# MLCogUP/nspeech

Hardware: AMD Instinct MI355X
Metric: mel-frames/sec Tacotron-2 LJSpeech bs32 train step (higher is better)
Workload: dtype bf16; 1 GPU; Tacotron-2 train step (fwd+bwd+clip+Adam), batch 32/GPU, T_in 160, T_out 1000, r=5; targets = spectrogram features of synthetic speech (SURVEY 8d); global_batch=32, parallelism=dp1, deterministic_gradients=True

## Files before the change

### include/nspeech_hip.h

```cpp
#ifndef NSPEECH_HIP_H
#define NSPEECH_HIP_H
#include <stddef.h>
#include <stdint.h>

#ifdef __cplusplus
extern "C" {
#endif

typedef void* ns_stream_t;

enum { NS_OK = 0, NS_ERR_BAD_ARG = -1, NS_ERR_UNSUPPORTED_SHAPE = -2, NS_ERR_LAUNCH = -3,
       NS_ERR_SHORT_BUFFER = -4  };
enum { NS_F32 = 0, NS_BF16 = 1, NS_F64 = 2  };
enum { NS_ACT_NONE = 0, NS_ACT_RELU = 1, NS_ACT_TANH = 2, NS_ACT_SIGMOID = 3,
       NS_ACT_SOFTSIGN = 4  };

int ns_version(void);
const char* ns_device_arch(void);
const char* ns_last_error(void);

int ns_occupy(int blocks, int threads, int lds_bytes, int heavy, double usec, int* started, ns_stream_t stream);
int ns_wait_counter(const int* counter, int target, double timeout_usec, ns_stream_t stream);

typedef struct {
  int dtype;
  int M, N, K;
  const void* A; int64_t lda; int a_mode;
  const void* B; int64_t ldb; int b_mode;
  int b_seg_len; int64_t b_seg_stride;
  void* C; int64_t ldc; int c_dtype;
  int accumulate;
  const float* bias;
  int act;
  float alpha;
  int row_period, row_lo, row_hi, row_shift;
  float* col_sum; float* col_sumsq;
  int split_k;
  const void* addend; int64_t ld_add;
  const void* gate; int64_t ld_gate;
  int f32_passes;
  int addend_dtype;
  const void* A_lo; const void* B_lo;
  int batch; int64_t batch_stride_a, batch_stride_b, batch_stride_c;
  float* stat_part;
  int stat_slots;
  const void* stat_z; int64_t ld_stat_z; int stat_z_dtype;
  const float* stat_mean; const float* stat_istd;
  float* splitk_work; int* splitk_count;
} ns_gemm_params;
int ns_gemm(const ns_gemm_params* p, ns_stream_t stream);
size_t ns_gemm_stat_part_floats(int M, int N);
size_t ns_gemm_splitk_work_bytes(int M, int N, int split_k);
size_t ns_gemm_splitk_counters(int M, int N);
const char* ns_gemm_last_kernel(void);



typedef struct {
  const void* src; int src_dtype; int64_t src_si, src_sj;
  void* dst; int dst_dtype; int64_t dst_si, dst_sj;
  int I, J, Cc;
  int accumulate;
} ns_copy3d_params;
int ns_copy3d(const ns_copy3d_params* p, ns_stream_t stream);

typedef struct {
  const int* ids;
  const float* table;
  void* out; int out_dtype;
  int N, T, P, padl, D, V;
} ns_embedding_params;
int ns_embedding_fwd(const ns_embedding_params* p, ns_stream_t stream);
typedef struct {
  const int* ids;
  const float* dout;
  float* dtable;
  int N, T, P, padl, D, V;
  float* work;
} ns_embedding_bwd_params;
int ns_embedding_bwd(const ns_embedding_bwd_params* p, ns_stream_t stream);
size_t ns_embedding_bwd_work_floats(int N, int D, int V);

typedef struct {
  const void* z; void* y; int dtype;
  int rows, C;
  const float* col_sum; const float* col_sumsq; float count;
  const float* gamma; const float* beta;
  float* moving_mean; float* moving_var;
  float* mean_out; float* istd_out;
  float eps, momentum;
  int training;
  int row_period, row_lo, row_hi;
  void* y_hi; void* y_lo;
  int64_t ld_y;
} ns_bn_fwd_params;
int ns_bn_fwd(const ns_bn_fwd_params* p, ns_stream_t stream);

typedef struct {
  const float* dy; const void* z; void* dpre; int dtype;
  int rows, C;
  const float* mean; const float* istd; const float* gamma;
  float* dgamma; float* dbeta; float* dbias;
  float* work;
  float count;
  int act;
  int row_period, row_lo, row_hi;
  int dpre_dtype;
  const float* sum_dy; const float* sum_dyxh;
  int64_t ld_dy;
} ns_bn_bwd_params;
int ns_bn_bwd(const ns_bn_bwd_params* p, ns_stream_t stream);

typedef struct {
  const void* x; int dtype; int64_t ld;
  int rows, C;
  float* out;
  float* work;
} ns_colsum_params;
int ns_colsum(const ns_colsum_params* p, ns_stream_t stream);
size_t ns_colsum_work_floats(int C);

typedef struct {
  const float* pred; int64_t ldp;
  const float* target;
  void* dpred; int dpred_dtype; int64_t ldd;
  int N, T, P, padl, F;
  int n_prio; float w_all, w_prio;
  float* loss_acc;
  int vec4;
} ns_l1_loss_params;
int ns_l1_loss(const ns_l1_loss_params* p, ns_stream_t stream);

typedef struct { const float* x; int64_t n; float* out; float* work; } ns_sumsq_params;
int ns_sumsq(const ns_sumsq_params* p, ns_stream_t stream);
typedef struct {
  float* p; const float* g; float* m; float* v; int64_t n;
  const float* gnorm_sq; float clip; float grad_scale;
  float lr_t, beta1, beta2, eps;
  void* shadow_bf16;
  const int* status[12];
  float* skipped;
} ns_adam_params;
int ns_adam(const ns_adam_params* p, ns_stream_t stream);

typedef struct { const float* x; const int64_t* offsets; int nseg; float* out; } ns_segment_stats_params;
int ns_segment_stats(const ns_segment_stats_params* p, ns_stream_t stream);

int ns_zero(void* p, size_t bytes, ns_stream_t stream);
#define NS_ZERO_MANY_MAX 24
int ns_zero_many(void* const* ptrs, const size_t* bytes, int n, ns_stream_t stream);
int ns_streams_concurrent(ns_stream_t a, ns_stream_t b, void* work);

typedef struct { const float* src; void* hi; void* lo; int64_t n; } ns_split_params;
int ns_split_hi_lo(const ns_split_params* p, ns_stream_t stream);

typedef struct {
  const float* src; int rows, cols; int64_t ld_src;
  void* dst; int dst_dtype; int64_t ld_dst;
  int transpose;
  void* dst_hi; void* dst_lo;
} ns_cast2d_params;
int ns_cast2d(const ns_cast2d_params* p, ns_stream_t stream);
int ns_cast2d_batchable(const ns_cast2d_params* p);
int ns_cast2d_batch(const ns_cast2d_params* table_dev, const int* tile_end_dev, int n, int total_tiles, ns_stream_t stream);

typedef struct {
  int dtype;
  int N, T, H, P, padl;
  const float* xg; int64_t ld_xg;
  const void* whT;
  const void* wh;
  const int* lengths;
  int reverse;
  float forget_bias;
  void* h; int64_t ld_h;
  float* c;
  void* gates;
  const float* dh; int64_t ld_dh;
  void* dgates;
  float* work;
  int f32_passes;
  const void* whT_hi; const void* whT_lo; const void* wh_bf16;
  void* dgates_bf16;
  void* h_bf16; int64_t ld_h_bf16;
  uint32_t zoneout_thr_cell, zoneout_thr_output;
  uint32_t zoneout_seed_cell, zoneout_seed_output;
  float cell_clip;
} ns_lstm_seq_params;
int ns_lstm_seq_fwd(const ns_lstm_seq_params* p, ns_stream_t stream);
int ns_lstm_seq_bwd(const ns_lstm_seq_params* p, ns_stream_t stream);
size_t ns_lstm_seq_work_bytes(const ns_lstm_seq_params* p);
int ns_lstm_seq2_fwd(const ns_lstm_seq_params* p0, const ns_lstm_seq_params* p1, ns_stream_t stream);
int ns_lstm_seq2_bwd(const ns_lstm_seq_params* p0, const ns_lstm_seq_params* p1, ns_stream_t stream);


int ns_lstm_cluster_supported(const ns_lstm_seq_params* fw, const ns_lstm_seq_params* bw, int backward);
size_t ns_lstm_cluster_work_bytes(const ns_lstm_seq_params* p);
int ns_lstm_cluster_fwd(const ns_lstm_seq_params* fw, const ns_lstm_seq_params* bw, void* work, ns_stream_t stream);
int ns_lstm_cluster_bwd(const ns_lstm_seq_params* fw, const ns_lstm_seq_params* bw, void* work, ns_stream_t stream);

int ns_lstm_wide_supported(const ns_lstm_seq_params* p, int backward);
size_t ns_lstm_wide_work_bytes(const ns_lstm_seq_params* p);
int ns_lstm_wide_fwd(const ns_lstm_seq_params* p, void* work, ns_stream_t stream);
int ns_lstm_wide_bwd(const ns_lstm_seq_params* p, void* work, ns_stream_t stream);

typedef struct {
  int dtype, N, H, K;
  const void* a; int64_t a_sn;
  const void* wT;
  const float* xg; int64_t xg_sn;
  const float* bias;
  const float* c_prev; int64_t c_sn;
  void* h_out; int64_t h_sn;
  void* h_out2; int64_t h2_sn;
  float* c_out; int64_t co_sn;
  float forget_bias;
  int f32_passes;
  const void* wT_hi; const void* wT_lo;
  float zoneout_cell, zoneout_output;
  const void* h_prev; int64_t hp_sn;
  float cell_clip;
} ns_lstm_step_params;
int ns_lstm_step(const ns_lstm_step_params* p, ns_stream_t stream);

size_t ns_rows32_packed_bytes(int K, int C);
int ns_rows32_pack(const float* w, int64_t ldw, int K, int C, int cell_units, void* packed, ns_stream_t stream);
size_t ns_rows32_rows_bytes(int K);
int ns_rows32_pack_rows(const float* a, int64_t a_sn, int N, int K, void* rows, int rows_K, int col0, ns_stream_t stream);
typedef struct {
  int N, K, C;
  const float* a; int64_t a_sn;
  const void* a_rows; int a_rows_K, a_rows_col;
  const void* packed;
  int f32_passes;
  const float* bias;
  const float* add; int64_t add_sn;
  int act;
  float* out; int64_t out_sn;
  float* out2; int64_t out2_sn;
  void* rows_out; int rows_out_K, rows_out_col;
  void* rows_out2; int rows_out2_K, rows_out2_col;
  int cell_units;
  const float* c_prev; int64_t c_sn;
  float* c_out; int64_t co_sn;
  float forget_bias;
  float zoneout_cell, zoneout_output;
  const float* h_prev; int64_t hp_sn;
  float cell_clip;
} ns_rows32_params;
int ns_rows32(const ns_rows32_params* p, ns_stream_t stream);

typedef struct {
  int dtype, N, Ti, Pi, padl_i, Tia, A, E, kw;
  const int* lengths;
  const float* keys_t;
  const void* values;
  const float* q; int64_t q_sn;
  const float* aprev; float* aout; int64_t al_sn;
  void* ctx_out; int64_t ctx_sn;
  void* ctx_out2; int64_t ctx2_sn;
  const float* wcl; const float* v;
  float* e_raw;
  const void* pv; int E2;
  void* pv_out; int64_t pv_out_sn;
// ... 298 lines not shown
```

### nspeech_amd/csrc/common.h

```cpp
#pragma once
#include <hip/hip_runtime.h>
#include <stdint.h>
#include <stdio.h>
#include <string.h>
#include "../../include/nspeech_hip.h"

typedef __bf16 bf16_t;
typedef __attribute__((ext_vector_type(8))) __bf16 bf16x8;
typedef __attribute__((ext_vector_type(4))) __bf16 bf16x4;
typedef __attribute__((ext_vector_type(4))) float f32x4;
typedef __attribute__((ext_vector_type(16))) float f32x16;

void ns_set_error(const char* fmt, ...);
int ns_zero_async(void* p, size_t bytes, hipStream_t s);
int ns_device_cus();
int ns_stats_finalize(const float* part, int slots, int N, float* s1, float* s2, hipStream_t s);

#define NS_CHECK_ARG(cond, ...)                                   \
  do {                                                            \
    if (!(cond)) {                                                \
      ns_set_error(__VA_ARGS__);                                  \
      return NS_ERR_BAD_ARG;                                      \
    }                                                             \
  } while (0)

#define NS_CHECK_LAUNCH(name)                                     \
  do {                                                            \
    hipError_t e__ = hipGetLastError();                           \
    if (e__ != hipSuccess) {                                      \
      ns_set_error("%s: launch failed: %s", name,                 \
                   hipGetErrorString(e__));                       \
      return NS_ERR_LAUNCH;                                       \
    }                                                             \
  } while (0)

template <typename T> struct dt_of;
template <> struct dt_of<float> { static constexpr int v = NS_F32; };
template <> struct dt_of<bf16_t> { static constexpr int v = NS_BF16; };

__device__ __forceinline__ float ldf(const float* p) { return *p; }
__device__ __forceinline__ float ldf(const bf16_t* p) { return (float)*p; }
__device__ __forceinline__ void stf(float* p, float v) { *p = v; }
__device__ __forceinline__ void stf(bf16_t* p, float v) { *p = (bf16_t)v; }

__device__ __forceinline__ float sigmoidf_(float x) {
  return __builtin_amdgcn_rcpf(1.0f + __builtin_amdgcn_exp2f(-1.4426950408889634f * x));
}
__device__ __forceinline__ float tanhf_(float x) {
  return 1.0f - 2.0f * __builtin_amdgcn_rcpf(__builtin_amdgcn_exp2f(2.8853900817779268f * x) + 1.0f);
}

__device__ __forceinline__ void ns_st_sc1(float* p, float v) { __hip_atomic_store(p, v, __ATOMIC_RELAXED, __HIP_MEMORY_SCOPE_AGENT); }
__device__ __forceinline__ float ns_ld_sc1(const float* p) { return __hip_atomic_load(p, __ATOMIC_RELAXED, __HIP_MEMORY_SCOPE_AGENT); }
__device__ __forceinline__ void ns_st_sc1(float4* p, const float4& v) {
  unsigned long long* q = (unsigned long long*)p;
  __hip_atomic_store(q, ((unsigned long long)__float_as_uint(v.y) << 32) | __float_as_uint(v.x), __ATOMIC_RELAXED, __HIP_MEMORY_SCOPE_AGENT);
  __hip_atomic_store(q + 1, ((unsigned long long)__float_as_uint(v.w) << 32) | __float_as_uint(v.z), __ATOMIC_RELAXED, __HIP_MEMORY_SCOPE_AGENT);
}
__device__ __forceinline__ float4 ns_ld_sc1(const float4* p) {
  const unsigned long long* q = (const unsigned long long*)p;
  const unsigned long long a = __hip_atomic_load(q, __ATOMIC_RELAXED, __HIP_MEMORY_SCOPE_AGENT);
  const unsigned long long b = __hip_atomic_load(q + 1, __ATOMIC_RELAXED, __HIP_MEMORY_SCOPE_AGENT);
  return make_float4(__uint_as_float((unsigned)a), __uint_as_float((unsigned)(a >> 32)), __uint_as_float((unsigned)b),
                     __uint_as_float((unsigned)(b >> 32)));
}
__device__ __forceinline__ void ns_drain_stores() { asm volatile("s_waitcnt vmcnt(0)" ::: "memory"); }

__host__ __device__ __forceinline__ uint32_t ns_fmix32(uint32_t x) {
  x ^= x >> 16; x *= 0x85EBCA6Bu; x ^= x >> 13; x *= 0xC2B2AE35u; x ^= x >> 16;
  return x;
}
__host__ __device__ __forceinline__ bool ns_zone_keep(uint32_t seed, uint32_t t, uint32_t n, uint32_t u, uint32_t thr) {
  uint32_t x = ns_fmix32(seed ^ (t * 0x9E3779B9u));
  x = ns_fmix32(x ^ (n * 0x7FEB352Du));
  x = ns_fmix32(x ^ (u * 0x846CA68Bu));
  return (x >> 8) < thr;
}

__device__ __forceinline__ float ns_cell_clip(float c, float clip) { return clip > 0.f ? fminf(fmaxf(c, -clip), clip) : c; }

__device__ __forceinline__ float apply_act(float v, int act) {
  switch (act) {
    case NS_ACT_RELU: return v > 0.f ? v : 0.f;
    case NS_ACT_TANH: return tanhf_(v);
    case NS_ACT_SIGMOID: return sigmoidf_(v);
    case NS_ACT_SOFTSIGN: return v / (1.0f + fabsf(v));
    default: return v;
  }
}

#define NS_DPP_F(v, ctrl) __builtin_bit_cast(float, __builtin_amdgcn_update_dpp(0, __builtin_bit_cast(int, (v)), (ctrl), 0xF, 0xF, true))
__device__ __forceinline__ float row16_sum(float v) {
  v += NS_DPP_F(v, 0xB1);
  v += NS_DPP_F(v, 0x4E);
  v += NS_DPP_F(v, 0x141);
  v += NS_DPP_F(v, 0x140);
  return v;
}
__device__ __forceinline__ float row16_max(float v) {
  v = fmaxf(v, NS_DPP_F(v, 0xB1));
  v = fmaxf(v, NS_DPP_F(v, 0x4E));
  v = fmaxf(v, NS_DPP_F(v, 0x141));
  v = fmaxf(v, NS_DPP_F(v, 0x140));
  return v;
}
__device__ __forceinline__ float wave_sum(float v) {
  v = row16_sum(v);
  v += __shfl_xor(v, 16, 64);
  v += __shfl_xor(v, 32, 64);
  return v;
}
__device__ __forceinline__ float wave_max(float v) {
  v = row16_max(v);
  v = fmaxf(v, __shfl_xor(v, 16, 64));
  v = fmaxf(v, __shfl_xor(v, 32, 64));
  return v;
}

__device__ __forceinline__ float block_sum(float v, float* red) {
  v = wave_sum(v);
  int w = threadIdx.x >> 6, nw = (blockDim.x + 63) >> 6;
  __syncthreads();
  if ((threadIdx.x & 63) == 0) red[w] = v;
  __syncthreads();
  float s = 0.f;
  for (int i = 0; i < nw; ++i) s += red[i];
  return s;
}
__device__ __forceinline__ float block_max(float v, float* red) {
  v = wave_max(v);
  int w = threadIdx.x >> 6, nw = (blockDim.x + 63) >> 6;
  __syncthreads();
  if ((threadIdx.x & 63) == 0) red[w] = v;
  __syncthreads();
  float s = -INFINITY;
  for (int i = 0; i < nw; ++i) s = fmaxf(s, red[i]);
  return s;
}

__device__ __forceinline__ void ldsplit8(const float* p, bool ok, bf16x8& hi, bf16x8& lo) {
  float4 a = make_float4(0.f, 0.f, 0.f, 0.f), b = a;
  if (ok) { a = *(const float4*)p; b = *(const float4*)(p + 4); }
  const float f[8] = {a.x, a.y, a.z, a.w, b.x, b.y, b.z, b.w};
#pragma unroll
  for (int i = 0; i < 8; ++i) {
    const bf16_t h = (bf16_t)f[i];
    hi[i] = h;
    lo[i] = (bf16_t)(f[i] - (float)h);
  }
}
template <int PASSES>
__device__ __forceinline__ f32x4 mfma_split(const bf16x8& ah, const bf16x8& al, const bf16x8& bh, const bf16x8& bl,
                                            f32x4 acc) {
  if (PASSES > 1) acc = __builtin_amdgcn_mfma_f32_16x16x32_bf16(al, bh, acc, 0, 0, 0);
  if (PASSES > 2) acc = __builtin_amdgcn_mfma_f32_16x16x32_bf16(ah, bl, acc, 0, 0, 0);
  return __builtin_amdgcn_mfma_f32_16x16x32_bf16(ah, bh, acc, 0, 0, 0);
}


__device__ __forceinline__ void ns_rows32_store(bf16_t* base, int nkc, int n, int k, float v) {
  const long i16 = (((long)(n >> 4) * nkc + (k >> 5)) * 64 + ((k >> 3) & 3) * 16 + (n & 15)) * 2;
  const bf16_t h = (bf16_t)v;
  base[i16 * 8 + (k & 7)] = h;
  base[(i16 + 1) * 8 + (k & 7)] = (bf16_t)(v - (float)h);
}

constexpr unsigned NS_SPIN_TICKS = 200000000u;
#define NS_GLOBAL __attribute__((address_space(1)))
template <typename T> __device__ __forceinline__ T ns_lds_peek(const T* p) {
  return *(const volatile __attribute__((address_space(3))) T*)p;
}
template <typename T> __device__ __forceinline__ void ns_lds_poke(T* p, T v) {
  *(volatile __attribute__((address_space(3))) T*)p = v;
}
__device__ __forceinline__ bool ns_spin_timed_out(unsigned& t0) {
  const unsigned now = (unsigned)wall_clock64() | 1u;
  if (t0 == 0u) { t0 = now; return false; }
  return now - t0 > NS_SPIN_TICKS;
}

static inline int ceil_div(long a, long b) { return (int)((a + b - 1) / b); }
```

### nspeech_amd/csrc/core.hip

```cpp
#include "common.h"
#include <stdarg.h>

static thread_local char g_err[512] = "";

void ns_set_error(const char* fmt, ...) {
  va_list ap;
  va_start(ap, fmt);
  vsnprintf(g_err, sizeof(g_err), fmt, ap);
  va_end(ap);
}

int ns_device_cus() {
  static int cached[64] = {0};
  int dev = 0;
  if (hipGetDevice(&dev) != hipSuccess || dev < 0 || dev >= 64) { (void)hipGetLastError(); return 256; }
  if (cached[dev] == 0) {
    int n = 0;
    if (hipDeviceGetAttribute(&n, hipDeviceAttributeMultiprocessorCount, dev) != hipSuccess || n <= 0) { (void)hipGetLastError(); n = 256; }
    cached[dev] = n;
  }
  return cached[dev];
}

extern "C" int ns_version(void) { return 100; }
extern "C" const char* ns_device_arch(void) { return "gfx950"; }
extern "C" const char* ns_last_error(void) { return g_err; }

__global__ void ns_zero_kernel(uint4* p, size_t n16) {
  for (size_t i = (size_t)blockIdx.x * blockDim.x + threadIdx.x; i < n16; i += (size_t)gridDim.x * blockDim.x)
    p[i] = make_uint4(0u, 0u, 0u, 0u);
}
int ns_zero_async(void* p, size_t bytes, hipStream_t s) {
  if (bytes == 0) return NS_OK;
  NS_CHECK_ARG(p && (bytes & 15) == 0 && (((uintptr_t)p) & 15) == 0, "ns_zero_async: 16-byte granularity");
  const size_t n16 = bytes / 16;
  const int grid = (int)((n16 + 255) / 256 < 4096 ? (n16 + 255) / 256 : 4096);
  hipLaunchKernelGGL(ns_zero_kernel, dim3(grid), dim3(256), 0, s, (uint4*)p, n16);
  NS_CHECK_LAUNCH("ns_zero");
  return NS_OK;
}
extern "C" int ns_zero(void* p, size_t bytes, ns_stream_t stream) { return ns_zero_async(p, bytes, (hipStream_t)stream); }

struct ZeroMany { uint4* p[NS_ZERO_MANY_MAX]; size_t n16[NS_ZERO_MANY_MAX]; };
__global__ void ns_zero_many_kernel(ZeroMany z) {
  uint4* p = z.p[blockIdx.y];
  const size_t n16 = z.n16[blockIdx.y];
  for (size_t i = (size_t)blockIdx.x * blockDim.x + threadIdx.x; i < n16; i += (size_t)gridDim.x * blockDim.x)
    p[i] = make_uint4(0u, 0u, 0u, 0u);
}
extern "C" int ns_zero_many(void* const* ptrs, const size_t* bytes, int n, ns_stream_t stream) {
  NS_CHECK_ARG(n >= 0 && (n == 0 || (ptrs && bytes)), "ns_zero_many: null");
  for (int i0 = 0; i0 < n; i0 += NS_ZERO_MANY_MAX) {
    ZeroMany z = {};
    const int m = n - i0 < NS_ZERO_MANY_MAX ? n - i0 : NS_ZERO_MANY_MAX;
    size_t most = 0;
    for (int i = 0; i < m; ++i) {
      NS_CHECK_ARG((bytes[i0 + i] & 15) == 0 && (((uintptr_t)ptrs[i0 + i]) & 15) == 0 && (ptrs[i0 + i] || !bytes[i0 + i]),
                   "ns_zero_many: 16-byte granularity");
      z.p[i] = (uint4*)ptrs[i0 + i];
      z.n16[i] = bytes[i0 + i] / 16;
      most = z.n16[i] > most ? z.n16[i] : most;
    }
    if (most == 0) continue;
    const int gx = (int)((most + 255) / 256 < 256 ? (most + 255) / 256 : 256);
    hipLaunchKernelGGL(ns_zero_many_kernel, dim3(gx, m), dim3(256), 0, (hipStream_t)stream, z);
    NS_CHECK_LAUNCH("ns_zero_many");
  }
  return NS_OK;
}

__global__ void ns_occupy_kernel(unsigned long long ticks, int* started) {
  extern __shared__ char occupy_lds[];
  if (threadIdx.x == 0) {
    occupy_lds[0] = 1;
    if (started) atomicAdd(started, 1);
  }
  const unsigned long long t0 = wall_clock64();
  while (wall_clock64() - t0 < ticks) __builtin_amdgcn_s_sleep(8);
}
__global__ void ns_wait_counter_kernel(const int* counter, int target, unsigned long long ticks) {
  const unsigned long long t0 = wall_clock64();
  while (__hip_atomic_load(counter, __ATOMIC_RELAXED, __HIP_MEMORY_SCOPE_AGENT) < target && wall_clock64() - t0 < ticks)
    __builtin_amdgcn_s_sleep(8);
}
__global__ void ns_occupy_heavy_kernel(unsigned long long ticks, int* started) {
  extern __shared__ char occupy_lds[];
  if (threadIdx.x == 0) {
    occupy_lds[0] = 1;
    if (started) atomicAdd(started, 1);
  }
  asm volatile("v_mov_b32 v127, 0" ::: "v127");
  const unsigned long long t0 = wall_clock64();
  while (wall_clock64() - t0 < ticks) __builtin_amdgcn_s_sleep(8);
}
extern "C" int ns_occupy(int blocks, int threads, int lds_bytes, int heavy, double usec, int* started, ns_stream_t stream) {
  NS_CHECK_ARG(blocks >= 1 && blocks <= 4096 && threads >= 64 && threads <= 1024 && (threads & 63) == 0,
               "ns_occupy: 1..4096 blocks of 64..1024 threads (a multiple of 64)");
  NS_CHECK_ARG(lds_bytes >= 0 && lds_bytes <= 160 * 1024 && usec >= 0 && usec <= 1e6, "ns_occupy: lds <= 160 KB, usec <= 1e6");
  if (lds_bytes > 64 * 1024)
    (void)hipFuncSetAttribute(heavy ? (const void*)ns_occupy_heavy_kernel : (const void*)ns_occupy_kernel,
                              hipFuncAttributeMaxDynamicSharedMemorySize, lds_bytes);
  const size_t lds = (size_t)(lds_bytes < 16 ? 16 : lds_bytes);
  const unsigned long long ticks = (unsigned long long)(usec * 100.0);
  if (heavy) hipLaunchKernelGGL(ns_occupy_heavy_kernel, dim3(blocks), dim3(threads), lds, (hipStream_t)stream, ticks, started);
  else hipLaunchKernelGGL(ns_occupy_kernel, dim3(blocks), dim3(threads), lds, (hipStream_t)stream, ticks, started);
  NS_CHECK_LAUNCH("ns_occupy");
  return NS_OK;
}
extern "C" int ns_wait_counter(const int* counter, int target, double timeout_usec, ns_stream_t stream) {
  NS_CHECK_ARG(counter && timeout_usec >= 0 && timeout_usec <= 1e6, "ns_wait_counter: null counter or timeout > 1 s");
  hipLaunchKernelGGL(ns_wait_counter_kernel, dim3(1), dim3(64), 0, (hipStream_t)stream, counter, target,
                     (unsigned long long)(timeout_usec * 100.0));
  NS_CHECK_LAUNCH("ns_wait_counter");
  return NS_OK;
}

__global__ void ns_probe_wait_kernel(int* w) {
  const long long t0 = wall_clock64();
  int seen = 0;
  while (wall_clock64() - t0 < 20000) {
    if (__hip_atomic_load(w, __ATOMIC_RELAXED, __HIP_MEMORY_SCOPE_AGENT) != 0) { seen = 1; break; }
  }
  w[1] = seen;
}
__global__ void ns_probe_set_kernel(int* w) { __hip_atomic_store(w, 1, __ATOMIC_RELAXED, __HIP_MEMORY_SCOPE_AGENT); }
extern "C" int ns_streams_concurrent(ns_stream_t a_, ns_stream_t b_, void* work) {
  hipStream_t a = (hipStream_t)a_, b = (hipStream_t)b_;
  NS_CHECK_ARG(work && (((uintptr_t)work) & 15) == 0, "ns_streams_concurrent: 16 bytes of device memory");
  if (a == b) return 0;
  int rc = ns_zero_async(work, 16, a);
  if (rc) return rc;
  if (hipStreamSynchronize(a) != hipSuccess || hipStreamSynchronize(b) != hipSuccess) {
    ns_set_error("ns_streams_concurrent: synchronize failed");
    return NS_ERR_LAUNCH;
  }
  hipLaunchKernelGGL(ns_probe_wait_kernel, dim3(1), dim3(1), 0, a, (int*)work);
  hipLaunchKernelGGL(ns_probe_set_kernel, dim3(1), dim3(1), 0, b, (int*)work);
  NS_CHECK_LAUNCH("ns_streams_concurrent");
  int host[2] = {0, 0};
  if (hipStreamSynchronize(a) != hipSuccess || hipStreamSynchronize(b) != hipSuccess ||
      hipMemcpy(host, work, sizeof(host), hipMemcpyDeviceToHost) != hipSuccess) {
    ns_set_error("ns_streams_concurrent: synchronize / copy failed");
    return NS_ERR_LAUNCH;
  }
  return host[1] ? 1 : 0;
}
```

### nspeech_amd/csrc/elementwise.hip

```cpp
#include "common.h"
#include <stdlib.h>

__device__ __forceinline__ float ld_dyn(const void* p, int dtype, long i) {
  return dtype == NS_BF16 ? (float)((const bf16_t*)p)[i] : ((const float*)p)[i];
}
__device__ __forceinline__ void st_dyn(void* p, int dtype, long i, float v) {
  if (dtype == NS_BF16) ((bf16_t*)p)[i] = (bf16_t)v;
  else ((float*)p)[i] = v;
}

__global__ void copy3d_kernel(ns_copy3d_params p) {
  const long total = (long)p.I * p.J * p.Cc;
  for (long idx = (long)blockIdx.x * blockDim.x + threadIdx.x; idx < total; idx += (long)gridDim.x * blockDim.x) {
    const int c = idx % p.Cc;
    const long ij = idx / p.Cc;
    const int j = ij % p.J;
    const int i = ij / p.J;
    const float v = ld_dyn(p.src, p.src_dtype, i * p.src_si + j * p.src_sj + c);
    const long d = i * p.dst_si + j * p.dst_sj + c;
    if (p.accumulate) st_dyn(p.dst, p.dst_dtype, d, ld_dyn(p.dst, p.dst_dtype, d) + v);
    else st_dyn(p.dst, p.dst_dtype, d, v);
  }
}
extern "C" int ns_copy3d(const ns_copy3d_params* p, ns_stream_t s) {
  NS_CHECK_ARG(p && p->src && p->dst, "ns_copy3d: null");
  const long total = (long)p->I * p->J * p->Cc;
  if (total <= 0) return NS_OK;
  int grid = (int)min((long)4096, (total + 255) / 256);
  hipLaunchKernelGGL(copy3d_kernel, dim3(grid), dim3(256), 0, (hipStream_t)s, *p);
  NS_CHECK_LAUNCH("copy3d");
  return NS_OK;
}

__global__ void embedding_fwd_kernel(ns_embedding_params p) {
  const int row = blockIdx.x;
  const int n = row / p.T, t = row % p.T;
  int id = p.ids[row];
  id = id < 0 ? 0 : (id >= p.V ? p.V - 1 : id);
  const float* src = p.table + (long)id * p.D;
  const long dst = ((long)n * p.P + p.padl + t) * p.D;
  for (int d = threadIdx.x; d < p.D; d += blockDim.x) st_dyn(p.out, p.out_dtype, dst + d, src[d]);
}
extern "C" int ns_embedding_fwd(const ns_embedding_params* p, ns_stream_t s) {
  NS_CHECK_ARG(p && p->ids && p->table && p->out, "ns_embedding_fwd: null");
  if (p->N * p->T == 0) return NS_OK;
  hipLaunchKernelGGL(embedding_fwd_kernel, dim3(p->N * p->T), dim3(64), 0, (hipStream_t)s, *p);
  NS_CHECK_LAUNCH("embedding_fwd");
  return NS_OK;
}
constexpr int EMB_CNT = 1024;
__global__ __launch_bounds__(256) void embedding_bwd_kernel(ns_embedding_bwd_params p) {
  __shared__ int list[256];
  __shared__ int wcnt[4];
  __shared__ int last;
  const int v = blockIdx.x, n = blockIdx.y, tid = threadIdx.x, lane = tid & 63, wave = tid >> 6;
  constexpr int MAXD = 4;
  float acc[MAXD] = {0.f, 0.f, 0.f, 0.f};
  const float* rows = p.dout + ((long)n * p.P + p.padl) * p.D;
  for (int base = 0; base < p.T; base += 256) {
    const int t = base + tid;
    bool hit = false;
    if (t < p.T) {
      int id = p.ids[n * p.T + t];
      id = id < 0 ? 0 : (id >= p.V ? p.V - 1 : id);
      hit = id == v;
    }
    const unsigned long long b = __ballot(hit);
    if (lane == 0) wcnt[wave] = __popcll(b);
    __syncthreads();
    int off = __popcll(b & ((1ull << lane) - 1ull));
    for (int w = 0; w < wave; ++w) off += wcnt[w];
    const int total = wcnt[0] + wcnt[1] + wcnt[2] + wcnt[3];
    if (hit) list[off] = t;
    __syncthreads();
    for (int e = 0; e < total; e += 4) {
      float x[4][MAXD];
#pragma unroll
      for (int q = 0; q < 4; ++q) {
        const float* src = rows + (long)list[min(e + q, total - 1)] * p.D;
#pragma unroll
        for (int i = 0; i < MAXD; ++i) x[q][i] = (e + q < total && tid + 256 * i < p.D) ? src[tid + 256 * i] : 0.f;
      }
#pragma unroll
      for (int q = 0; q < 4; ++q)
#pragma unroll
        for (int i = 0; i < MAXD; ++i) acc[i] += x[q][i];
    }
    __syncthreads();
  }
  float* share = p.work + EMB_CNT + ((long)v * p.N + n) * p.D;
#pragma unroll
  for (int i = 0; i < MAXD; ++i)
    if (tid + 256 * i < p.D) ns_st_sc1(share + tid + 256 * i, acc[i]);
  ns_drain_stores();
  __syncthreads();
  int* counter = (int*)p.work + v;
  if (tid == 0) last = atomicAdd(counter, 1) == p.N - 1;
  __syncthreads();
  if (!last) return;
#pragma unroll
  for (int i = 0; i < MAXD; ++i) {
    if (tid + 256 * i < p.D) {
      float a = 0.f;
      for (int m = 0; m < p.N; ++m) a += ns_ld_sc1(p.work + EMB_CNT + ((long)v * p.N + m) * p.D + tid + 256 * i);
      p.dtable[(long)v * p.D + tid + 256 * i] += a;
    }
  }
  if (tid == 0) *counter = 0;
}
extern "C" size_t ns_embedding_bwd_work_floats(int N, int D, int V) {
  return (size_t)EMB_CNT + (size_t)(V > 0 ? V : 0) * (size_t)(N > 0 ? N : 0) * (size_t)(D > 0 ? D : 0);
}
extern "C" int ns_embedding_bwd(const ns_embedding_bwd_params* p, ns_stream_t s) {
  NS_CHECK_ARG(p && p->ids && p->dout && p->dtable && p->work, "ns_embedding_bwd: null (work: ns_embedding_bwd_work_floats)");
  NS_CHECK_ARG(p->D <= 1024 && p->V >= 1 && p->V <= EMB_CNT, "ns_embedding_bwd: D <= 1024, V <= 1024");
  if (p->N * p->T == 0) return NS_OK;
  hipLaunchKernelGGL(embedding_bwd_kernel, dim3(p->V, p->N), dim3(256), 0, (hipStream_t)s, *p);
  NS_CHECK_LAUNCH("embedding_bwd");
  return NS_OK;
}

__global__ void bn_finalize_kernel(ns_bn_fwd_params p) {
  const int c = blockIdx.x * blockDim.x + threadIdx.x;
  if (c >= p.C) return;
  float mean, var;
  if (p.training) {
    mean = p.col_sum[c] / p.count;
    var = p.col_sumsq[c] / p.count - mean * mean;
    var = var < 0.f ? 0.f : var;
    if (p.moving_mean) {
      p.moving_mean[c] = p.moving_mean[c] * p.momentum + mean * (1.f - p.momentum);
      p.moving_var[c] = p.moving_var[c] * p.momentum + var * (1.f - p.momentum);
    }
  } else {
    mean = p.moving_mean[c];
    var = p.moving_var[c];
  }
  p.mean_out[c] = mean;
  p.istd_out[c] = rsqrtf(var + p.eps);
}

template <typename T>
__global__ void bn_apply_kernel(ns_bn_fwd_params p) {
  const T* z = (const T*)p.z;
  T* y = (T*)p.y;
  const long total = (long)p.rows * p.C;
  for (long idx = (long)blockIdx.x * blockDim.x + threadIdx.x; idx < total; idx += (long)gridDim.x * blockDim.x) {
    const int c = idx % p.C;
    const int row = idx / p.C;
    bool valid = true;
    if (p.row_period > 0) {
      const int t = row % p.row_period;
      valid = t >= p.row_lo && t < p.row_hi;
    }
    float v = 0.f;
    if (valid) v = (ldf(z + idx) - p.mean_out[c]) * p.istd_out[c] * p.gamma[c] + p.beta[c];
    stf(y + (p.ld_y ? (long)row * p.ld_y + c : idx), v);
  }
}
__device__ __forceinline__ float4 ld4f(const float* p) { return *(const float4*)p; }
__device__ __forceinline__ float4 ld4f(const bf16_t* p) {
  const bf16x4 v = *(const bf16x4*)p;
  return make_float4((float)v[0], (float)v[1], (float)v[2], (float)v[3]);
}
template <typename T>
__global__ __launch_bounds__(256) void bn_apply4_kernel(ns_bn_fwd_params p) {
  const T* z = (const T*)p.z;
  const int C4 = p.C >> 2;
  const long total4 = (long)p.rows * C4;
  for (long i4 = (long)blockIdx.x * blockDim.x + threadIdx.x; i4 < total4; i4 += (long)gridDim.x * blockDim.x) {
    const int row = (int)(i4 / C4), c = (int)(i4 - (long)row * C4) * 4;
    bool valid = true;
    if (p.row_period > 0) {
      const int t = row % p.row_period;
      valid = t >= p.row_lo && t < p.row_hi;
    }
    float4 v = make_float4(0.f, 0.f, 0.f, 0.f);
    if (valid) {
      const float4 x = ld4f(z + i4 * 4), m = *(const float4*)(p.mean_out + c), is = *(const float4*)(p.istd_out + c);
      const float4 g = *(const float4*)(p.gamma + c), b = *(const float4*)(p.beta + c);
      v.x = (x.x - m.x) * is.x * g.x + b.x; v.y = (x.y - m.y) * is.y * g.y + b.y;
      v.z = (x.z - m.z) * is.z * g.z + b.z; v.w = (x.w - m.w) * is.w * g.w + b.w;
    }
    if (p.y) {
      const long yo = p.ld_y ? (long)row * p.ld_y + c : i4 * 4;
      if constexpr (sizeof(T) == 4) *(float4*)((float*)p.y + yo) = v;
      else {
        bf16x4 o; o[0] = (bf16_t)v.x; o[1] = (bf16_t)v.y; o[2] = (bf16_t)v.z; o[3] = (bf16_t)v.w;
        *(bf16x4*)((bf16_t*)p.y + yo) = o;
      }
    }
    if (p.y_hi) {
      const float f[4] = {v.x, v.y, v.z, v.w};
      bf16x4 hi, lo;
#pragma unroll
      for (int j = 0; j < 4; ++j) { hi[j] = (bf16_t)f[j]; lo[j] = (bf16_t)(f[j] - (float)hi[j]); }
      *(bf16x4*)((bf16_t*)p.y_hi + i4 * 4) = hi;
      *(bf16x4*)((bf16_t*)p.y_lo + i4 * 4) = lo;
    }
  }
}

extern "C" int ns_bn_fwd(const ns_bn_fwd_params* p, ns_stream_t s) {
  NS_CHECK_ARG(p && p->z && (p->y || p->y_hi) && p->gamma && p->beta && p->mean_out && p->istd_out, "ns_bn_fwd: null");
  NS_CHECK_ARG(!p->training || (p->col_sum && p->col_sumsq && p->count > 0), "ns_bn_fwd: training needs stats");
  NS_CHECK_ARG(p->training || (p->moving_mean && p->moving_var), "ns_bn_fwd: inference needs moving stats");
  NS_CHECK_ARG((p->y_hi != nullptr) == (p->y_lo != nullptr), "ns_bn_fwd: y_hi and y_lo come together");
  NS_CHECK_ARG(p->ld_y == 0 || (p->ld_y >= p->C && p->y), "ns_bn_fwd: ld_y < C, or no y");
  hipLaunchKernelGGL(bn_finalize_kernel, dim3(ceil_div(p->C, 256)), dim3(256), 0, (hipStream_t)s, *p);
  const long total = (long)p->rows * p->C;
  auto al = [](const void* q, int b) { return ((uintptr_t)q % b) == 0; };
  const int esz = p->dtype == NS_BF16 ? 2 : 4;
  const bool vec = p->C % 4 == 0 && p->ld_y % 4 == 0 && al(p->z, 4 * esz) && al(p->y, 4 * esz) && al(p->mean_out, 16) && al(p->istd_out, 16) &&
                   al(p->gamma, 16) && al(p->beta, 16) && al(p->y_hi, 8) && al(p->y_lo, 8);
  if (vec) {
    const int grid = (int)min((long)4096, (total / 4 + 255) / 256);
    if (p->dtype == NS_BF16) hipLaunchKernelGGL(bn_apply4_kernel<bf16_t>, dim3(grid), dim3(256), 0, (hipStream_t)s, *p);
    else hipLaunchKernelGGL(bn_apply4_kernel<float>, dim3(grid), dim3(256), 0, (hipStream_t)s, *p);
    NS_CHECK_LAUNCH("bn_fwd");
    return NS_OK;
  }
  NS_CHECK_ARG(p->y && !p->y_hi, "ns_bn_fwd: the pre-split outputs need C %% 4 == 0 and 16-byte aligned operands");
  int grid = (int)min((long)8192, (total + 255) / 256);
  if (p->dtype == NS_BF16) hipLaunchKernelGGL(bn_apply_kernel<bf16_t>, dim3(grid), dim3(256), 0, (hipStream_t)s, *p);
  else hipLaunchKernelGGL(bn_apply_kernel<float>, dim3(grid), dim3(256), 0, (hipStream_t)s, *p);
  NS_CHECK_LAUNCH("bn_fwd");
  return NS_OK;
}

constexpr int BN_MAX_BLOCKS = 32;
constexpr int BN_ROWS_PER_BLOCK = 64;

template <typename T>
__global__ void bn_bwd_reduce_kernel(ns_bn_bwd_params p) {
  const T* z = (const T*)p.z;
  const int rpb = (p.rows + gridDim.x - 1) / gridDim.x;
  const int r0 = blockIdx.x * rpb, r1 = min(p.rows, r0 + rpb);
  for (int c = threadIdx.x; c < p.C; c += blockDim.x) {
    const float mean = p.mean[c], istd = p.istd[c];
    float s1 = 0.f, s2 = 0.f;
    for (int row = r0; row < r1; ++row) {
      if (p.row_period > 0) {
        const int t = row % p.row_period;
        if (t < p.row_lo || t >= p.row_hi) continue;
      }
      const long idx = (long)row * p.C + c;
      const float dy = p.dy[p.ld_dy ? (long)row * p.ld_dy + c : idx];
      const float xh = (ldf(z + idx) - mean) * istd;
      s1 += dy;
      s2 += dy * xh;
    }
    p.work[(long)(2 * blockIdx.x) * p.C + c] = s1;
    p.work[(long)(2 * blockIdx.x + 1) * p.C + c] = s2;
  }
}

template <typename T>
__global__ void bn_bwd_apply_kernel(ns_bn_bwd_params p) {
  const T* z = (const T*)p.z;
  T* dpre = (T*)p.dpre;
  const int rpb = (p.rows + gridDim.x - 1) / gridDim.x;
  const int r0 = blockIdx.x * rpb, r1 = min(p.rows, r0 + rpb);
  const float invM = 1.f / p.count;
  for (int c = threadIdx.x; c < p.C; c += blockDim.x) {
    const float mean = p.mean[c], istd = p.istd[c], g = p.gamma[c];
    float t1 = 0.f, t2 = 0.f;
    for (int b = 0; b < (int)gridDim.x; ++b) { t1 += p.work[(long)(2 * b) * p.C + c]; t2 += p.work[(long)(2 * b + 1) * p.C + c]; }
    const float m1 = t1 * invM, m2 = t2 * invM;
    float sb = 0.f;
    for (int row = r0; row < r1; ++row) {
      const long idx = (long)row * p.C + c;
      bool valid = true;
      if (p.row_period > 0) {
        const int t = row % p.row_period;
        valid = t >= p.row_lo && t < p.row_hi;
      }
      float d = 0.f;
      if (valid) {
        const float zv = ldf(z + idx);
        const float xh = (zv - mean) * istd;
        d = g * istd * (p.dy[p.ld_dy ? (long)row * p.ld_dy + c : idx] - m1 - xh * m2);
        if (p.act == NS_ACT_RELU) d = zv > 0.f ? d : 0.f;
        else if (p.act == NS_ACT_TANH) d *= (1.f - zv * zv);
        else if (p.act == NS_ACT_SIGMOID) d *= zv * (1.f - zv);
        else if (p.act == NS_ACT_SOFTSIGN) d *= (1.f - fabsf(zv)) * (1.f - fabsf(zv));
      }
      if (sizeof(T) == 4 && p.dpre_dtype == NS_BF16) {
        const bf16_t db = (bf16_t)d;
        ((bf16_t*)p.dpre)[idx] = db;
        sb += (float)db;
      } else {
        stf(dpre + idx, d);
        sb += (float)(T)d;
      }
    }
    if (p.dbias) atomicAdd(p.dbias + c, sb);
    if (blockIdx.x == 0) {
      if (p.dgamma) p.dgamma[c] += t2;
      if (p.dbeta) p.dbeta[c] += t1;
    }
  }
}
__device__ __forceinline__ float4 ld4(const float* p) { return *(const float4*)p; }
__device__ __forceinline__ float4 ld4(const bf16_t* p) {
  const bf16x4 v = *(const bf16x4*)p;
  return make_float4((float)v[0], (float)v[1], (float)v[2], (float)v[3]);
}
__device__ __forceinline__ void st4(float* p, float4 v) { *(float4*)p = v; }
__device__ __forceinline__ void st4(bf16_t* p, float4 v) {
  bf16x4 o;
  o[0] = (bf16_t)v.x; o[1] = (bf16_t)v.y; o[2] = (bf16_t)v.z; o[3] = (bf16_t)v.w;
  *(bf16x4*)p = o;
}
constexpr int BN4_QUADS = 16;
constexpr int BN4_LANES = 16;
constexpr int BN4_UNROLL = 4;
constexpr int BN4_MAX_RB = 64;

template <typename T>
__global__ __launch_bounds__(256) void bn_bwd_reduce4_kernel(ns_bn_bwd_params p) {
  __shared__ float red[256][8];
  const T* z = (const T*)p.z;
  const int tid = threadIdx.x, ql = tid % BN4_QUADS, rl = tid / BN4_QUADS;
  const int q = blockIdx.y * BN4_QUADS + ql;
  const bool active = 4 * q < p.C;
  const int rpb = (p.rows + gridDim.x - 1) / gridDim.x;
  const int r0 = blockIdx.x * rpb, r1 = min(p.rows, r0 + rpb);
  float s1[4] = {0.f, 0.f, 0.f, 0.f}, s2[4] = {0.f, 0.f, 0.f, 0.f};
  if (active) {
    const float4 mean = *(const float4*)(p.mean + 4 * q), istd = *(const float4*)(p.istd + 4 * q);
    for (int base = r0 + rl; base < r1; base += BN4_UNROLL * BN4_LANES) {
      float4 d[BN4_UNROLL], zz[BN4_UNROLL];
      bool ok[BN4_UNROLL];
#pragma unroll
      for (int u = 0; u < BN4_UNROLL; ++u) {
        const int row = base + u * BN4_LANES;
        ok[u] = row < r1;
        if (ok[u] && p.row_period > 0) {
          const int t = row % p.row_period;
          ok[u] = t >= p.row_lo && t < p.row_hi;
        }
        if (ok[u]) {
          const long idx = (long)row * p.C + 4 * q;
          d[u] = *(const float4*)(p.dy + (p.ld_dy ? (long)row * p.ld_dy + 4 * q : idx));
          zz[u] = ld4(z + idx);
        }
      }
#pragma unroll
      for (int u = 0; u < BN4_UNROLL; ++u) {
        if (ok[u]) {
          s1[0] += d[u].x; s2[0] = fmaf(d[u].x, (zz[u].x - mean.x) * istd.x, s2[0]);
          s1[1] += d[u].y; s2[1] = fmaf(d[u].y, (zz[u].y - mean.y) * istd.y, s2[1]);
          s1[2] += d[u].z; s2[2] = fmaf(d[u].z, (zz[u].z - mean.z) * istd.z, s2[2]);
          s1[3] += d[u].w; s2[3] = fmaf(d[u].w, (zz[u].w - mean.w) * istd.w, s2[3]);
        }
      }
    }
  }
#pragma unroll
  for (int i = 0; i < 4; ++i) { red[tid][i] = s1[i]; red[tid][4 + i] = s2[i]; }
  __syncthreads();
  if (rl == 0 && active) {
#pragma unroll
    for (int i = 0; i < 4; ++i) {
      float a = 0.f, b = 0.f;
      for (int r = 0; r < BN4_LANES; ++r) { a += red[r * BN4_QUADS + ql][i]; b += red[r * BN4_QUADS + ql][4 + i]; }
      p.work[(long)blockIdx.x * p.C + 4 * q + i] = a;
      p.work[((long)gridDim.x + blockIdx.x) * p.C + 4 * q + i] = b;
    }
  }
}

template <typename T>
__global__ __launch_bounds__(256) void bn_bwd_apply4_kernel(ns_bn_bwd_params p, const float* sum_dy, const float* sum_dyxh,
                                                            float* part) {
  __shared__ float red[256][4];
  const T* z = (const T*)p.z;
  const int tid = threadIdx.x, ql = tid % BN4_QUADS, rl = tid / BN4_QUADS;
  const int q = blockIdx.y * BN4_QUADS + ql;
  const bool active = 4 * q < p.C;
  const int rpb = (p.rows + gridDim.x - 1) / gridDim.x;
  const int r0 = blockIdx.x * rpb, r1 = min(p.rows, r0 + rpb);
  const bool d16 = sizeof(T) == 4 && p.dpre_dtype == NS_BF16;
  const float invM = 1.f / p.count;
  float sb[4] = {0.f, 0.f, 0.f, 0.f};
  if (active) {
    const float4 mean = *(const float4*)(p.mean + 4 * q), istd = *(const float4*)(p.istd + 4 * q);
    const float4 g = *(const float4*)(p.gamma + 4 * q);
    const float4 w1 = *(const float4*)(sum_dy + 4 * q), w2 = *(const float4*)(sum_dyxh + 4 * q);
    const float mu[4] = {mean.x, mean.y, mean.z, mean.w}, is[4] = {istd.x, istd.y, istd.z, istd.w};
    const float gi[4] = {g.x * istd.x, g.y * istd.y, g.z * istd.z, g.w * istd.w};
    const float m1[4] = {w1.x * invM, w1.y * invM, w1.z * invM, w1.w * invM};
    const float m2[4] = {w2.x * invM, w2.y * invM, w2.z * invM, w2.w * invM};
    for (int base = r0 + rl; base < r1; base += BN4_UNROLL * BN4_LANES) {
      float4 d[BN4_UNROLL], zz[BN4_UNROLL];
      bool inr[BN4_UNROLL], ok[BN4_UNROLL];
#pragma unroll
      for (int u = 0; u < BN4_UNROLL; ++u) {
        const int row = base + u * BN4_LANES;
        inr[u] = row < r1;
        ok[u] = inr[u];
        if (ok[u] && p.row_period > 0) {
          const int t = row % p.row_period;
          ok[u] = t >= p.row_lo && t < p.row_hi;
        }
        if (ok[u]) {
          const long idx = (long)row * p.C + 4 * q;
          d[u] = *(const float4*)(p.dy + (p.ld_dy ? (long)row * p.ld_dy + 4 * q : idx));
          zz[u] = ld4(z + idx);
        }
      }
#pragma unroll
      for (int u = 0; u < BN4_UNROLL; ++u) {
        if (!inr[u]) continue;
        const long idx = (long)(base + u * BN4_LANES) * p.C + 4 * q;
        float o[4] = {0.f, 0.f, 0.f, 0.f};
        if (ok[u]) {
          const float dv[4] = {d[u].x, d[u].y, d[u].z, d[u].w}, zv[4] = {zz[u].x, zz[u].y, zz[u].z, zz[u].w};
#pragma unroll
          for (int i = 0; i < 4; ++i) {
            const float xh = (zv[i] - mu[i]) * is[i];
            float v = gi[i] * (dv[i] - m1[i] - xh * m2[i]);
            if (p.act == NS_ACT_RELU) v = zv[i] > 0.f ? v : 0.f;
            else if (p.act == NS_ACT_TANH) v *= (1.f - zv[i] * zv[i]);
            else if (p.act == NS_ACT_SIGMOID) v *= zv[i] * (1.f - zv[i]);
            else if (p.act == NS_ACT_SOFTSIGN) v *= (1.f - fabsf(zv[i])) * (1.f - fabsf(zv[i]));
            o[i] = v;
          }
        }
        const float4 ov = make_float4(o[0], o[1], o[2], o[3]);
        if (d16) {
          st4((bf16_t*)p.dpre + idx, ov);
#pragma unroll
          for (int i = 0; i < 4; ++i) sb[i] += (float)(bf16_t)o[i];
        } else {
          st4((T*)p.dpre + idx, ov);
#pragma unroll
          for (int i = 0; i < 4; ++i) sb[i] += (float)(T)o[i];
        }
      }
    }
  }
#pragma unroll
  for (int i = 0; i < 4; ++i) red[tid][i] = sb[i];
  __syncthreads();
  if (rl == 0 && active) {
#pragma unroll
    for (int i = 0; i < 4; ++i) {
      float a = 0.f;
      for (int r = 0; r < BN4_LANES; ++r) a += red[r * BN4_QUADS + ql][i];
      part[(long)blockIdx.x * p.C + 4 * q + i] = a;
    }
  }
}
__global__ __launch_bounds__(256) void bn_bwd_finalize_kernel(ns_bn_bwd_params p, const float* sum_dy, const float* sum_dyxh,
                                                              const float* part, int nb) {
  __shared__ float red[8][33];
  const int cl = threadIdx.x & 31, q = threadIdx.x >> 5;
  const int c = blockIdx.x * 32 + cl;
  float a = 0.f;
  if (c < p.C && p.dbias)
    for (int b = q; b < nb; b += 8) a += part[(long)b * p.C + c];
  red[q][cl] = a;
  __syncthreads();
  if (q == 0 && c < p.C) {
    if (p.dbias) {
      const float s01 = red[0][cl] + red[1][cl], s23 = red[2][cl] + red[3][cl];
      const float s45 = red[4][cl] + red[5][cl], s67 = red[6][cl] + red[7][cl];
      p.dbias[c] += (s01 + s23) + (s45 + s67);
    }
    if (p.dgamma) p.dgamma[c] += sum_dyxh[c];
    if (p.dbeta) p.dbeta[c] += sum_dy[c];
  }
}

extern "C" int ns_bn_bwd(const ns_bn_bwd_params* p, ns_stream_t s_) {
  hipStream_t s = (hipStream_t)s_;
  NS_CHECK_ARG(p && p->dy && p->z && p->dpre && p->mean && p->istd && p->gamma && p->work, "ns_bn_bwd: null");
  NS_CHECK_ARG(!p->sum_dy == !p->sum_dyxh, "ns_bn_bwd: sum_dy and sum_dyxh come together");
  const bool al16 = ((uintptr_t)p->dy % 16 == 0) && ((uintptr_t)p->z % 8 == 0) && ((uintptr_t)p->dpre % 8 == 0) &&
                    ((uintptr_t)p->mean % 16 == 0) && ((uintptr_t)p->istd % 16 == 0) && ((uintptr_t)p->gamma % 16 == 0) &&
                    ((uintptr_t)p->work % 16 == 0) && (p->dtype == NS_BF16 || ((uintptr_t)p->z % 16 == 0 &&
                    (uintptr_t)p->dpre % (p->dpre_dtype == NS_BF16 ? 8 : 16) == 0)) &&
                    (!p->sum_dy || ((uintptr_t)p->sum_dy % 16 == 0 && (uintptr_t)p->sum_dyxh % 16 == 0));
  NS_CHECK_ARG(p->ld_dy == 0 || p->ld_dy >= p->C, "ns_bn_bwd: ld_dy < C");
  if (p->C % 4 == 0 && p->ld_dy % 4 == 0 && al16) {
    const int rb = max(1, min(BN4_MAX_RB, ceil_div(p->rows, 128)));
    const dim3 grid4(rb, ceil_div(p->C / 4, BN4_QUADS));
    const float* s1 = p->sum_dy;
    const float* s2 = p->sum_dyxh;
    float* part = p->work + 2L * p->C;
    if (!s1) {
      ns_bn_bwd_params q = *p;
      q.work = p->work + (2L + BN4_MAX_RB) * p->C;
      if (p->dtype == NS_BF16) hipLaunchKernelGGL(bn_bwd_reduce4_kernel<bf16_t>, grid4, dim3(256), 0, s, q);
      else hipLaunchKernelGGL(bn_bwd_reduce4_kernel<float>, grid4, dim3(256), 0, s, q);
      NS_CHECK_LAUNCH("bn_bwd_reduce");
      const int rc = ns_stats_finalize(q.work, rb, p->C, p->work, p->work + p->C, s);
      if (rc) return rc;
      s1 = p->work;
      s2 = p->work + p->C;
    }
    if (p->dtype == NS_BF16) hipLaunchKernelGGL(bn_bwd_apply4_kernel<bf16_t>, grid4, dim3(256), 0, s, *p, s1, s2, part);
    else hipLaunchKernelGGL(bn_bwd_apply4_kernel<float>, grid4, dim3(256), 0, s, *p, s1, s2, part);
    hipLaunchKernelGGL(bn_bwd_finalize_kernel, dim3(ceil_div(p->C, 32)), dim3(256), 0, s, *p, s1, s2, part, rb);
    NS_CHECK_LAUNCH("bn_bwd");
    return NS_OK;
  }
  const int grid = max(1, min(BN_MAX_BLOCKS, ceil_div(p->rows, BN_ROWS_PER_BLOCK)));
  if (p->dtype == NS_BF16) {
    hipLaunchKernelGGL(bn_bwd_reduce_kernel<bf16_t>, dim3(grid), dim3(256), 0, s, *p);
    hipLaunchKernelGGL(bn_bwd_apply_kernel<bf16_t>, dim3(grid), dim3(256), 0, s, *p);
  } else {
    hipLaunchKernelGGL(bn_bwd_reduce_kernel<float>, dim3(grid), dim3(256), 0, s, *p);
    hipLaunchKernelGGL(bn_bwd_apply_kernel<float>, dim3(grid), dim3(256), 0, s, *p);
  }
  NS_CHECK_LAUNCH("bn_bwd");
  return NS_OK;
}

constexpr int CS_ROWS = 32;
constexpr int COLSUM_MAX_BLOCKS = 64;
constexpr int COLSUM_CNT = 1024;
__global__ void colsum_kernel(ns_colsum_params p) {
  const int r0 = blockIdx.x * CS_ROWS;
  for (int c = threadIdx.x; c < p.C; c += blockDim.x) {
    float v[CS_ROWS];
#pragma unroll
    for (int j = 0; j < CS_ROWS; ++j) v[j] = (r0 + j < p.rows) ? ld_dyn(p.x, p.dtype, (long)(r0 + j) * p.ld + c) : 0.f;
    float s = 0.f;
#pragma unroll
    for (int j = 0; j < CS_ROWS; ++j) s += v[j];
    atomicAdd(p.out + c, s);
  }
}
template <typename T>
__global__ __launch_bounds__(256) void colsum4_kernel(ns_colsum_params p) {
  __shared__ float red[256][4];
  const T* x = (const T*)p.x;
  const int tid = threadIdx.x, ql = tid % BN4_QUADS, rl = tid / BN4_QUADS;
  const int q = blockIdx.y * BN4_QUADS + ql;
  const bool active = 4 * q < p.C;
  const int rpb = (p.rows + gridDim.x - 1) / gridDim.x;
  const int r0 = blockIdx.x * rpb, r1 = min(p.rows, r0 + rpb);
  float s4[4] = {0.f, 0.f, 0.f, 0.f};
  constexpr int CU = 8;
  if (active) {
    for (int base = r0 + rl; base < r1; base += CU * BN4_LANES) {
      float4 v[CU];
#pragma unroll
      for (int u = 0; u < CU; ++u) {
        const int row = base + u * BN4_LANES;
        v[u] = row < r1 ? ld4(x + (long)row * p.ld + 4 * q) : make_float4(0.f, 0.f, 0.f, 0.f);
      }
#pragma unroll
      for (int u = 0; u < CU; ++u) { s4[0] += v[u].x; s4[1] += v[u].y; s4[2] += v[u].z; s4[3] += v[u].w; }
    }
  }
#pragma unroll
  for (int i = 0; i < 4; ++i) red[tid][i] = s4[i];
  __syncthreads();
  if (rl == 0 && active) {
#pragma unroll
    for (int i = 0; i < 4; ++i) {
      float a = 0.f;
      for (int r = 0; r < BN4_LANES; ++r) a += red[r * BN4_QUADS + ql][i];
      if (4 * q + i < p.C) {
        if (p.work) ns_st_sc1(p.work + COLSUM_CNT + (long)blockIdx.x * p.C + 4 * q + i, a);
        else atomicAdd(p.out + 4 * q + i, a);
      }
    }
  }
  if (!p.work) return;
  __shared__ int last;
  ns_drain_stores();
  __syncthreads();
  int* counter = (int*)p.work + blockIdx.y;
  if (tid == 0) last = atomicAdd(counter, 1) == (int)gridDim.x - 1;
  __syncthreads();
  if (!last) return;
  const int c0 = blockIdx.y * BN4_QUADS * 4;
  constexpr int GB = COLSUM_MAX_BLOCKS / 4;
  const int cc = tid & 63, grp = tid >> 6;
  float pv[GB];
#pragma unroll
  for (int i = 0; i < GB; ++i) {
    const int b = grp * GB + i;
    pv[i] = (b < (int)gridDim.x && c0 + cc < p.C) ? ns_ld_sc1(p.work + COLSUM_CNT + (long)b * p.C + c0 + cc) : 0.f;
  }
  float a = 0.f;
#pragma unroll
  for (int i = 0; i < GB; ++i) a += pv[i];
  red[tid][0] = a;
  __syncthreads();
  if (tid < 64 && c0 + tid < p.C) p.out[c0 + tid] += ((red[tid][0] + red[64 + tid][0]) + red[128 + tid][0]) + red[192 + tid][0];
  if (tid == 0) *counter = 0;
}
extern "C" size_t ns_colsum_work_floats(int C) { return (size_t)COLSUM_CNT + (size_t)COLSUM_MAX_BLOCKS * (size_t)(C > 0 ? C : 0); }

__global__ __launch_bounds__(256) void colsum_det_kernel(ns_colsum_params p) {
  __shared__ int last;
  const int c = blockIdx.y * 256 + threadIdx.x;
  const int rpb = (p.rows + gridDim.x - 1) / gridDim.x;
  const int r0 = blockIdx.x * rpb, r1 = min(p.rows, r0 + rpb);
  if (c < p.C) {
    float a = 0.f;
    for (int r = r0; r < r1; ++r) a += ld_dyn(p.x, p.dtype, (long)r * p.ld + c);
    ns_st_sc1(p.work + COLSUM_CNT + (long)blockIdx.x * p.C + c, a);
  }
  ns_drain_stores();
  __syncthreads();
  int* counter = (int*)p.work + blockIdx.y;
  if (threadIdx.x == 0) last = atomicAdd(counter, 1) == (int)gridDim.x - 1;
  __syncthreads();
  if (!last) return;
  if (c < p.C) {
    float a = 0.f;
    for (int b = 0; b < (int)gridDim.x; ++b) a += ns_ld_sc1(p.work + COLSUM_CNT + (long)b * p.C + c);
    p.out[c] += a;
  }
  if (threadIdx.x == 0) *counter = 0;
}

extern "C" int ns_colsum(const ns_colsum_params* p, ns_stream_t s) {
  NS_CHECK_ARG(p && p->x && p->out, "ns_colsum: null");
  if (p->rows <= 0 || p->C <= 0) return NS_OK;
  const int esz = p->dtype == NS_BF16 ? 2 : 4;
  NS_CHECK_ARG(!p->work || p->C <= 64 * COLSUM_CNT, "ns_colsum: the deterministic form takes C <= 65536");
  if ((p->C + 3) / 4 * 4 <= p->ld && p->ld % 4 == 0 && ((uintptr_t)p->x % (4 * esz)) == 0) {
    const dim3 grid(max(1, min(64, ceil_div(p->rows, 128))), ceil_div((p->C + 3) / 4, BN4_QUADS));
    if (p->dtype == NS_BF16) hipLaunchKernelGGL(colsum4_kernel<bf16_t>, grid, dim3(256), 0, (hipStream_t)s, *p);
    else hipLaunchKernelGGL(colsum4_kernel<float>, grid, dim3(256), 0, (hipStream_t)s, *p);
    NS_CHECK_LAUNCH("colsum");
    return NS_OK;
  }
  if (p->work) {
    ns_colsum_params q = *p;
    hipLaunchKernelGGL(colsum_det_kernel, dim3(COLSUM_MAX_BLOCKS, ceil_div(p->C, 256)), dim3(256), 0, (hipStream_t)s, q);
    NS_CHECK_LAUNCH("colsum");
    return NS_OK;
  }
  hipLaunchKernelGGL(colsum_kernel, dim3(ceil_div(p->rows, CS_ROWS)), dim3(256), 0, (hipStream_t)s, *p);
  NS_CHECK_LAUNCH("colsum");
  return NS_OK;
}

__device__ __forceinline__ void l1_point(const ns_l1_loss_params& p, float pv, float tv, long prow, int f, float& s_all,
                                         float& s_pr) {
  const float d = pv - tv;
  const float ab = fabsf(d);
  s_all += ab;
  const bool pr = f < p.n_prio;
  if (pr) s_pr += ab;
  if (p.dpred) {
    const float sg = d > 0.f ? 1.f : (d < 0.f ? -1.f : 0.f);
    st_dyn(p.dpred, p.dpred_dtype, prow * p.ldd + f, sg * (p.w_all + (pr ? p.w_prio : 0.f)));
  }
}
// ... 525 lines not shown
```

### nspeech_amd/csrc/gemm.hip

```cpp
#include "common.h"

struct Epi {
  void* C; long ldc; int c_dtype; int accumulate;
  const float* bias; int act; float alpha;
  int row_period, row_lo, row_hi, row_shift;
  int M, N;
  const void* addend; long ld_add; int add_bf16;
  const void* gate; long ld_gate; int gate_dtype;
  const void* sz; long ld_sz; int sz_bf16; const float* smean; const float* sistd;
};

__device__ __forceinline__ Epi make_epi(const ns_gemm_params& p) {
  Epi e;
  e.C = p.C; e.ldc = p.ldc; e.c_dtype = p.c_dtype; e.accumulate = p.accumulate;
  e.bias = p.bias; e.act = p.act; e.alpha = p.alpha;
  e.row_period = p.row_period; e.row_lo = p.row_lo; e.row_hi = p.row_hi; e.row_shift = p.row_shift;
  e.M = p.M; e.N = p.N;
  e.addend = p.addend; e.ld_add = p.ld_add; e.add_bf16 = p.addend_dtype == NS_BF16;
  e.gate = p.gate; e.ld_gate = p.ld_gate; e.gate_dtype = p.dtype;
  e.sz = p.stat_z; e.ld_sz = p.ld_stat_z; e.sz_bf16 = p.stat_z_dtype == NS_BF16; e.smean = p.stat_mean; e.sistd = p.stat_istd;
  return e;
}

__device__ __forceinline__ bool row_valid(const Epi& e, int m) {
// ... 54 lines not shown
  __shared__ int sk_last;
  typedef unsigned int u32x4 __attribute__((ext_vector_type(4)));
  constexpr unsigned SLOT_BYTES = 256u * PER * 16u;
  const auto rs = __builtin_amdgcn_make_buffer_rsrc((void*)p.splitk_work, 0, 0x7ffffff0, 0x00020000);
  const unsigned tile0 = (unsigned)tile * (unsigned)p.split_k * SLOT_BYTES + (unsigned)tid * 16u;
  const unsigned mine = tile0 + (unsigned)ksl * SLOT_BYTES;
#pragma unroll
  for (int i = 0; i < PER; ++i) {
    const u32x4 x = {__float_as_uint(v[i].x), __float_as_uint(v[i].y), __float_as_uint(v[i].z), __float_as_uint(v[i].w)};
    __builtin_amdgcn_raw_buffer_store_b128(x, rs, mine + (unsigned)i * 4096u, 0, 16);
  }
  ns_drain_stores();
  __syncthreads();
  if (tid == 0) sk_last = atomicAdd(p.splitk_count + tile, 1) == p.split_k - 1;
  __syncthreads();
  if (!sk_last) return false;
#pragma unroll
  for (int i = 0; i < PER; ++i) v[i] = make_float4(0.f, 0.f, 0.f, 0.f);
  u32x4 cur[PER], nxt[PER];
#pragma unroll
  for (int i = 0; i < PER; ++i) cur[i] = __builtin_amdgcn_raw_buffer_load_b128(rs, tile0 + (unsigned)i * 4096u, 0, 16);
  for (int s = 0; s < p.split_k; ++s) {
    if (s + 1 < p.split_k) {
#pragma unroll
      for (int i = 0; i < PER; ++i)
        nxt[i] = __builtin_amdgcn_raw_buffer_load_b128(rs, tile0 + (unsigned)(s + 1) * SLOT_BYTES + (unsigned)i * 4096u, 0, 16);
    }
#pragma unroll
    for (int i = 0; i < PER; ++i) {
      v[i].x += __uint_as_float(cur[i][0]); v[i].y += __uint_as_float(cur[i][1]);
      v[i].z += __uint_as_float(cur[i][2]); v[i].w += __uint_as_float(cur[i][3]);
    }
#pragma unroll
    for (int i = 0; i < PER; ++i) cur[i] = nxt[i];
  }
  if (tid == 0) p.splitk_count[tile] = 0;
  return true;
}
template <int NJ>
__device__ __forceinline__ bool splitk_gather_acc(const ns_gemm_params& p, f32x4 (&acc)[4][NJ], int tile, int ksl, int tid) {
  float4 v[4 * NJ];
#pragma unroll
  for (int i = 0; i < 4; ++i)
#pragma unroll
    for (int j = 0; j < NJ; ++j) v[i * NJ + j] = make_float4(acc[i][j][0], acc[i][j][1], acc[i][j][2], acc[i][j][3]);
  if (!splitk_gather<4 * NJ>(p, v, tile, ksl, tid)) return false;
#pragma unroll
  for (int i = 0; i < 4; ++i)
#pragma unroll
    for (int j = 0; j < NJ; ++j) acc[i][j] = (f32x4){v[i * NJ + j].x, v[i * NJ + j].y, v[i * NJ + j].z, v[i * NJ + j].w};
  return true;
}

template <typename T>
__device__ __forceinline__ float ld_a(const ns_gemm_params& p, int m, int k) {
  const T* A = (const T*)p.A;
  return p.a_mode == 0 ? ldf(A + (long)m * p.lda + k) : ldf(A + (long)k * p.lda + m);
}
template <typename T>
__device__ __forceinline__ float ld_b(const ns_gemm_params& p, int k, int n) {
  const T* B = (const T*)p.B;
  if (p.b_seg_len > 0) {
    int s = k / p.b_seg_len;
    B += (long)s * p.b_seg_stride;
    k -= s * p.b_seg_len;
  }
  return p.b_mode == 0 ? ldf(B + (long)n * p.ldb + k) : ldf(B + (long)k * p.ldb + n);
}

template <typename T>
__global__ __launch_bounds__(256) void gemm_generic_kernel(ns_gemm_params p) {
  constexpr int BM = 64, BN = 64, BK = 16;
  __shared__ float As[BK][BM + 1];
  __shared__ float Bs[BK][BN + 1];
  const int tid = threadIdx.x;
  const int m0 = blockIdx.y * BM, n0 = blockIdx.x * BN;
  const int tx = tid & 15, ty = tid >> 4;
  const int nk = (p.K + BK - 1) / BK;
  const int per = (nk + p.split_k - 1) / p.split_k;
  const int ksl = blockIdx.z % p.split_k;
  batch_shift(p, blockIdx.z / p.split_k);
  const int kt0 = ksl * per, kt1 = min(nk, kt0 + per);
  float acc[4][4] = {};
  for (int kt = kt0; kt < kt1; ++kt) {
    const int k0 = kt * BK;
    for (int i = tid; i < BK * BM; i += 256) {
      int kk, mm;
      if (p.a_mode == 0) { kk = i % BK; mm = i / BK; } else { mm = i % BM; kk = i / BM; }
      int m = m0 + mm, k = k0 + kk;
      As[kk][mm] = (m < p.M && k < p.K) ? ld_a<T>(p, m, k) : 0.f;
    }
    for (int i = tid; i < BK * BN; i += 256) {
      int kk, nn;
      if (p.b_mode == 0) { kk = i % BK; nn = i / BK; } else { nn = i % BN; kk = i / BN; }
      int n = n0 + nn, k = k0 + kk;
      Bs[kk][nn] = (n < p.N && k < p.K) ? ld_b<T>(p, k, n) : 0.f;
    }
    __syncthreads();
#pragma unroll
    for (int kk = 0; kk < BK; ++kk) {
      float a[4], b[4];
#pragma unroll
      for (int i = 0; i < 4; ++i) a[i] = As[kk][ty * 4 + i];
#pragma unroll
      for (int j = 0; j < 4; ++j) b[j] = Bs[kk][tx * 4 + j];
#pragma unroll
      for (int i = 0; i < 4; ++i)
#pragma unroll
        for (int j = 0; j < 4; ++j) acc[i][j] = fmaf(a[i], b[j], acc[i][j]);
    }
    __syncthreads();
  }
  bool add_bias = (ksl == 0);
  if (p.splitk_work && p.split_k > 1) {
    float4 v[4];
#pragma unroll
    for (int i = 0; i < 4; ++i) v[i] = make_float4(acc[i][0], acc[i][1], acc[i][2], acc[i][3]);
    if (!splitk_gather<4>(p, v, blockIdx.y * gridDim.x + blockIdx.x, ksl, tid)) return;
#pragma unroll
    for (int i = 0; i < 4; ++i) { acc[i][0] = v[i].x; acc[i][1] = v[i].y; acc[i][2] = v[i].z; acc[i][3] = v[i].w; }
    add_bias = true;
  }
  Epi e = make_epi(p);
  float s1[4] = {0.f, 0.f, 0.f, 0.f}, s2[4] = {0.f, 0.f, 0.f, 0.f};
  for (int i = 0; i < 4; ++i) {
    int m = m0 + ty * 4 + i;
    if (m >= p.M) continue;
    bool valid = row_valid(e, m);
    for (int j = 0; j < 4; ++j) {
      int n = n0 + tx * 4 + j;
      if (n >= p.N) continue;
      float v = epi_value(e, m, n, acc[i][j], add_bias, valid);
      const float vs = epi_store(e, m, n, v);
      if (valid) {
        s1[j] += vs;
        s2[j] += stat_second(e, m, n, vs);
      }
    }
  }
  if (p.stat_part) {
#pragma unroll
    for (int j = 0; j < 4; ++j) { As[ty][tx * 4 + j] = s1[j]; Bs[ty][tx * 4 + j] = s2[j]; }
    __syncthreads();
    if (tid < BN && n0 + tid < p.N) {
      float a = 0.f, b = 0.f;
      for (int r = 0; r < 16; ++r) { a += As[r][tid]; b += Bs[r][tid]; }
      p.stat_part[(long)blockIdx.y * p.N + n0 + tid] = a;
      p.stat_part[((long)p.stat_slots + blockIdx.y) * p.N + n0 + tid] = b;
    }
  }
}

__global__ __launch_bounds__(1024) void gemm_stats_finalize_kernel(const float* part, int slots, int N, float* col_sum,
                                                                   float* col_sumsq) {
  __shared__ float red[32][33][2];
  const int c = threadIdx.x & 31, q = threadIdx.x >> 5;
  const int n = blockIdx.x * 32 + c;
  float a = 0.f, b = 0.f;
  if (n < N) {
    for (int s = q; s < slots; s += 32) {
      a += part[(long)s * N + n];
      b += part[((long)slots + s) * N + n];
    }
  }
  red[q][c][0] = a; red[q][c][1] = b;
  __syncthreads();
#pragma unroll
  for (int h = 16; h >= 1; h >>= 1) {
    if (q < h) { red[q][c][0] += red[q + h][c][0]; red[q][c][1] += red[q + h][c][1]; }
    __syncthreads();
  }
  if (q == 0 && n < N) {
    col_sum[n] = red[0][c][0];
    if (col_sumsq) col_sumsq[n] = red[0][c][1];
  }
}

constexpr int GBM = 128, GBN = 128, GBK = 64;

__device__ __forceinline__ int row_img_off(int row, int chunk) {
  return row * 128 + ((chunk ^ ((row >> 1) & 7)) << 4);
}
__device__ __forceinline__ int col_swz(int k) { return (k & 3) | ((k >> 1) & 4); }
__device__ __forceinline__ int col_img_off_chunk(int k, int chunk) {
  return k * 256 + ((chunk ^ (col_swz(k) << 1)) << 4);
}
__device__ __forceinline__ int col_img_off_unit(int k, int unit) {
  return k * 256 + ((unit ^ (col_swz(k) << 2)) << 3);
}

typedef __attribute__((address_space(3))) bf16x4 lds_bf16x4;

__device__ __forceinline__ bf16x8 frag_row(const char* img, int row, int chunk) {
  return *(const bf16x8*)(img + row_img_off(row, chunk));
}
__device__ __forceinline__ bf16x8 frag_col(const char* img, int kbase, int col0, int lane) {
  const int i16 = lane & 15, g = lane >> 4;
  const int q = i16 >> 2, pp = i16 & 3;
  const int k = kbase + 8 * g + q;
  const int unit = (col0 >> 2) + pp;
  bf16x4 t0 = __builtin_amdgcn_ds_read_tr16_b64_v4bf16((lds_bf16x4*)(img + col_img_off_unit(k, unit)));
  bf16x4 t1 = __builtin_amdgcn_ds_read_tr16_b64_v4bf16((lds_bf16x4*)(img + col_img_off_unit(k + 4, unit)));
  return __builtin_shufflevector(t0, t1, 0, 1, 2, 3, 4, 5, 6, 7);
}

struct Stage { uint4 v[4]; };

template <int MODE, int BK = GBK, int ROWS = 128>
__device__ __forceinline__ void stage_load(Stage& s, const bf16_t* base, long ld, int r0, int extent,
                                           int k0, int K, int tid) {
  if (MODE == 0) {
    const int c = tid & 7;
#pragma unroll
    for (int i = 0; i < ROWS / 32; ++i) {
      const int row = (tid >> 3) + 32 * i;
      const int r = r0 + row, k = k0 + c * 8;
      if (r < extent && k < K) s.v[i] = *(const uint4*)(base + (long)r * ld + k);
      else s.v[i] = make_uint4(0, 0, 0, 0);
    }
  } else {
    const int c = tid & 15;
#pragma unroll
    for (int i = 0; i < BK / 16; ++i) {
      const int kr = (tid >> 4) + 16 * i;
      const int k = k0 + kr, r = r0 + c * 8;
      if (k < K && r < extent) s.v[i] = *(const uint4*)(base + (long)k * ld + r);
      else s.v[i] = make_uint4(0, 0, 0, 0);
    }
  }
}
template <int MODE, int BK = GBK, int ROWS = 128>
__device__ __forceinline__ void stage_store(const Stage& s, char* img, int tid) {
  if (MODE == 0) {
    const int c = tid & 7;
#pragma unroll
    for (int i = 0; i < ROWS / 32; ++i) {
      const int row = (tid >> 3) + 32 * i;
      *(uint4*)(img + row_img_off(row, c)) = s.v[i];
    }
  } else {
    const int c = tid & 15;
#pragma unroll
    for (int i = 0; i < BK / 16; ++i) {
      const int kr = (tid >> 4) + 16 * i;
      *(uint4*)(img + col_img_off_chunk(kr, c)) = s.v[i];
    }
  }
}

__device__ __forceinline__ void mfma_epilogue(const ns_gemm_params& p, f32x4 (&acc)[4][4], int m0, int n0, int wm,
                                              int wn, int lane, bool add_bias) {
  Epi e = make_epi(p);
#pragma unroll
  for (int j = 0; j < 4; ++j) {
    const int n = n0 + wn * 64 + j * 16 + (lane & 15);
    float s1 = 0.f, s2 = 0.f;
#pragma unroll
    for (int i = 0; i < 4; ++i) {
#pragma unroll
      for (int r = 0; r < 4; ++r) {
        const int m = m0 + wm * 64 + i * 16 + (lane >> 4) * 4 + r;
        if (m < p.M && n < p.N) {
          const bool valid = row_valid(e, m);
          float v = epi_value(e, m, n, acc[i][j][r], add_bias, valid);
          const float vs = epi_store(e, m, n, v);
          if (valid) {
            s1 += vs;
            s2 += stat_second(e, m, n, vs);
          }
        }
      }
    }
    if (p.stat_part) {
      s1 += __shfl_xor(s1, 16, 64); s1 += __shfl_xor(s1, 32, 64);
      s2 += __shfl_xor(s2, 16, 64); s2 += __shfl_xor(s2, 32, 64);
      if ((lane >> 4) == 0 && n < p.N) {
        const long slot = (m0 >> 6) + wm;
        p.stat_part[slot * p.N + n] = s1;
        p.stat_part[(p.stat_slots + slot) * p.N + n] = s2;
      }
    }
  }
}

__device__ __forceinline__ void xcd_work_item(const ns_gemm_params& p, int nwg, int& tile, int& ksl) {
  if (p.split_k > 1 && p.batch == 1) {
    const int W = nwg * p.split_k;
    const int L = blockIdx.x + gridDim.x * blockIdx.y;
    const int xcd = L & 7, q = W >> 3, r = W & 7;
    const int j = (xcd < r ? xcd * (q + 1) : r * (q + 1) + (xcd - r) * q) + (L >> 3);
    ksl = j / nwg;
    tile = j - ksl * nwg;
  } else {
    const int orig = blockIdx.x, xcd = orig & 7, q = nwg >> 3, r = nwg & 7;
    tile = (xcd < r ? xcd * (q + 1) : r * (q + 1) + (xcd - r) * q) + (orig >> 3);
    ksl = blockIdx.y;
  }
}

__device__ __forceinline__ float4 ldv4(const void* base, bool bf16, long off) {
  if (bf16) {
    const bf16x4 v = *(const bf16x4*)((const bf16_t*)base + off);
    return make_float4((float)v[0], (float)v[1], (float)v[2], (float)v[3]);
  }
  return *(const float4*)((const float*)base + off);
}
template <int NJ>
__device__ __forceinline__ void x256_quadrant(const ns_gemm_params& p, f32x4 (&acc)[4][NJ], int mq, int nq, int lane) {
  const Epi e = make_epi(p);
  const int li = lane & 15, c4 = (lane >> 4) * 4;
  const bool want_stats = p.stat_part != nullptr;
#pragma unroll
  for (int j = 0; j < NJ; ++j) {
    const int n = nq + j * 16 + c4;
    if (n >= p.N) continue;
    float4 bias = make_float4(0.f, 0.f, 0.f, 0.f), smean = bias, sistd = bias;
    if (e.bias) bias = *(const float4*)(e.bias + n);
    if (e.sz) { smean = *(const float4*)(e.smean + n); sistd = *(const float4*)(e.sistd + n); }
    float s1[4] = {0.f, 0.f, 0.f, 0.f}, s2[4] = {0.f, 0.f, 0.f, 0.f};
#pragma unroll
    for (int i = 0; i < 4; ++i) {
      const int m = mq + i * 16 + li;
      if (m >= p.M) continue;
      const bool valid = row_valid(e, m);
      float v[4] = {acc[i][j][0], acc[i][j][1], acc[i][j][2], acc[i][j][3]};
      const float bb[4] = {bias.x, bias.y, bias.z, bias.w};
      float4 ad = make_float4(0.f, 0.f, 0.f, 0.f);
// ... 517 lines not shown
      int kin;
      const float* bb = b_tile_base((kt + 1) * FBK, kin);
      stagef_load<AMODE, TM>(sa, A, p.lda, m0, p.M, (kt + 1) * FBK, p.K, tid);
      stagef_load<BMODE>(sb, bb, p.ldb, n0, p.N, kin, KB, tid);
    }
    bf16x8 ah[4], al[4], bh[NJ], bl[NJ];
#pragma unroll
    for (int i = 0; i < 4; ++i) {
      if (AMODE == 0) {
        const int off = row32_img_off(wm * 64 + i * 16 + (lane & 15), lane >> 4);
        ah[i] = *(const bf16x8*)(iAh + off);
        if (PASSES > 1) al[i] = *(const bf16x8*)(iAl + off);
      } else {
        ah[i] = frag_col(iAh, 0, wm * 64 + i * 16, lane);
        if (PASSES > 1) al[i] = frag_col(iAl, 0, wm * 64 + i * 16, lane);
      }
    }
#pragma unroll
    for (int j = 0; j < NJ; ++j) {
      if (BMODE == 0) {
        const int off = row32_img_off(wn * (NJ * 16) + j * 16 + (lane & 15), lane >> 4);
        bh[j] = *(const bf16x8*)(iBh + off);
        if (PASSES > 1) bl[j] = *(const bf16x8*)(iBl + off);
      } else {
        bh[j] = frag_col(iBh, 0, wn * (NJ * 16) + j * 16, lane);
        if (PASSES > 1) bl[j] = frag_col(iBl, 0, wn * (NJ * 16) + j * 16, lane);
      }
    }
#pragma unroll
    for (int i = 0; i < 4; ++i)
#pragma unroll
      for (int j = 0; j < NJ; ++j) {
        if (VEC) {
          if (PASSES > 1) {
            acc[i][j] = __builtin_amdgcn_mfma_f32_16x16x32_bf16(bh[j], al[i], acc[i][j], 0, 0, 0);
            acc[i][j] = __builtin_amdgcn_mfma_f32_16x16x32_bf16(bl[j], ah[i], acc[i][j], 0, 0, 0);
          }
          acc[i][j] = __builtin_amdgcn_mfma_f32_16x16x32_bf16(bh[j], ah[i], acc[i][j], 0, 0, 0);
        } else {
          if (PASSES > 1) {
            acc[i][j] = __builtin_amdgcn_mfma_f32_16x16x32_bf16(al[i], bh[j], acc[i][j], 0, 0, 0);
            acc[i][j] = __builtin_amdgcn_mfma_f32_16x16x32_bf16(ah[i], bl[j], acc[i][j], 0, 0, 0);
          }
          acc[i][j] = __builtin_amdgcn_mfma_f32_16x16x32_bf16(ah[i], bh[j], acc[i][j], 0, 0, 0);
        }
      }
    if (more) {
      char* nb = smem + (cur ^ 1) * 32768;
      stagef_store<AMODE, PASSES, TM>(sa, nb, nb + 8192, tid);
      stagef_store<BMODE, PASSES>(sb, nb + 16384, nb + 24576, tid);
    }
    __syncthreads();
  }
  bool add_bias = ksl == 0;
  if (p.splitk_work && p.split_k > 1) {
    if (!splitk_gather_acc<NJ>(p, acc, wgid, ksl, tid)) return;
    add_bias = true;
  }
  if constexpr (VEC) x256_quadrant(p, acc, m0 + wm * 64, n0 + wn * (NJ * 16), lane);
  else mfma_epilogue(p, acc, m0, n0, wm, wn, lane, add_bias);
}

template <int PASSES, int MT, int NC>
__global__ __launch_bounds__(SKW * 64) void gemm_skinny_f32_kernel(ns_gemm_params p) {
  __shared__ float red[SKW][16 * MT][20];
  const int tid = threadIdx.x, lane = tid & 63, wave = tid >> 6;
  const int n0 = blockIdx.x * NC;
  const int m0 = blockIdx.y * 16 * MT;
  const float* A = (const float*)p.A;
  const float* B = (const float*)p.B;
  const int r16 = lane & 15, g = lane >> 4;
  f32x4 acc[MT];
#pragma unroll
  for (int i = 0; i < MT; ++i) acc[i] = (f32x4){0.f, 0.f, 0.f, 0.f};
  const int nkc = (p.K + 31) / 32;
  const bool ok0 = m0 + r16 < p.M, ok1 = MT > 1 && m0 + 16 + r16 < p.M, okn = r16 < NC && n0 + r16 < p.N;
  for (int kc0 = wave; kc0 < nkc; kc0 += SKW * 2) {
    bf16x8 ah[2][MT], al[2][MT], bh[2], bl[2];
#pragma unroll
    for (int q = 0; q < 2; ++q) {
      const int k = (kc0 + q * SKW) * 32 + g * 8;
      const bool okk = k < p.K;
      ldsplit8(A + (long)(m0 + r16) * p.lda + k, ok0 && okk, ah[q][0], al[q][0]);
      if (MT > 1) ldsplit8(A + (long)(m0 + 16 + r16) * p.lda + k, ok1 && okk, ah[q][MT - 1], al[q][MT - 1]);
      ldsplit8(B + (long)(n0 + r16) * p.ldb + k, okn && okk, bh[q], bl[q]);
    }
#pragma unroll
    for (int q = 0; q < 2; ++q)
#pragma unroll
      for (int i = 0; i < MT; ++i) acc[i] = mfma_split<PASSES>(ah[q][i], al[q][i], bh[q], bl[q], acc[i]);
  }
#pragma unroll
  for (int i = 0; i < MT; ++i)
#pragma unroll
    for (int r = 0; r < 4; ++r) red[wave][i * 16 + g * 4 + r][r16] = acc[i][r];
  __syncthreads();
  Epi e = make_epi(p);
  for (int idx = tid; idx < 16 * MT * NC; idx += SKW * 64) {
    const int mm = idx / NC, nn = idx % NC;
    const int m = m0 + mm, n = n0 + nn;
    if (m >= p.M || n >= p.N) continue;
    float v = 0.f;
#pragma unroll
    for (int w = 0; w < SKW; ++w) v += red[w][mm][nn];
    const bool valid = row_valid(e, m);
    v = epi_value(e, m, n, v, true, valid);
    epi_store(e, m, n, v);
  }
}

static bool aligned16(const void* p) { return (((uintptr_t)p) & 15) == 0; }

static thread_local const char* g_last_kernel = "";
extern "C" const char* ns_gemm_last_kernel(void) { return g_last_kernel; }

static bool vec_epilogue_ok(const ns_gemm_params& p) {
  auto al = [](const void* q, long ld, bool bf16) { return !q || ((((uintptr_t)q) & (bf16 ? 7 : 15)) == 0 && ld % 4 == 0); };
  if (p.accumulate == 2 || p.split_k != 1 || p.N % 4 != 0) return false;
  if (p.batch > 1 && p.batch_stride_c % 4 != 0) return false;
  return al(p.C, p.ldc, p.c_dtype == NS_BF16) && al(p.addend, p.ld_add, p.addend_dtype == NS_BF16) &&
         al(p.gate, p.ld_gate, p.dtype == NS_BF16) && al(p.stat_z, p.ld_stat_z, p.stat_z_dtype == NS_BF16) &&
         al(p.bias, 4, false) && al(p.stat_mean, 4, false) && al(p.stat_istd, 4, false) && al(p.stat_part, 4, false);
}
static bool half_tiles_wanted(const ns_gemm_params& p, int tiles128) {
  static const int env = [] { const char* e = getenv("NS_GEMM_HALF"); return e ? atoi(e) : -1; }();
  if (env == 0 || env == 1) return env != 0;
  return tiles128 * p.batch <= (env > 1 ? env : 256) && p.M > 64;
}
static bool x256_ok(const ns_gemm_params& p) {
  if (p.dtype != NS_BF16 || p.a_mode != 0 || p.b_mode != 0 || p.split_k != 1) return false;
  if (p.b_seg_len != 0 && (p.b_seg_len % 64 != 0 || p.b_seg_stride % 8 != 0)) return false;
  if (p.K % 64 != 0 || p.K < 128 || p.M < 1024 || p.N % 128 != 0) return false;
  if ((p.A_lo != nullptr) != (p.B_lo != nullptr)) return false;
  if (p.A_lo && (!aligned16(p.A_lo) || !aligned16(p.B_lo))) return false;
  {
    auto al = [](const void* q, long ld, bool bf16) { return !q || ((((uintptr_t)q) & (bf16 ? 7 : 15)) == 0 && ld % 4 == 0); };
    if (!al(p.C, p.ldc, p.c_dtype == NS_BF16) || !al(p.addend, p.ld_add, p.addend_dtype == NS_BF16) ||
        !al(p.gate, p.ld_gate, true) || !al(p.stat_z, p.ld_stat_z, p.stat_z_dtype == NS_BF16) || !al(p.bias, 4, false) ||
        !al(p.stat_mean, 4, false) || !al(p.stat_istd, 4, false) || !al(p.stat_part, 4, false)) return false;
  }
  if ((double)p.M * (double)p.lda * 2.0 >= 4.0e9 || (double)p.N * (double)p.ldb * 2.0 >= 4.0e9) return false;
  if (getenv("NS_GEMM_NO256")) return false;
  return ceil_div(p.M, 256) * ceil_div(p.N, 256) >= 96;
}

extern "C" size_t ns_gemm_stat_part_floats(int M, int N) {
  if (M <= 0 || N <= 0) return 0;
  return (size_t)2 * 4 * ceil_div(M, 256) * (size_t)N;
}

static int gemm_dispatch(ns_gemm_params& p, hipStream_t stream);

int ns_stats_finalize(const float* part, int slots, int N, float* s1, float* s2, hipStream_t stream) {
  hipLaunchKernelGGL(gemm_stats_finalize_kernel, dim3(ceil_div(N, 32)), dim3(1024), 0, stream, part, slots, N, s1, s2);
  NS_CHECK_LAUNCH("gemm_stats_finalize");
  return NS_OK;
}

extern "C" size_t ns_gemm_splitk_work_bytes(int M, int N, int split_k) {
  if (split_k <= 1) return 0;
  return (size_t)split_k * ((size_t)ceil_div(M, 128) * 128) * ((size_t)ceil_div(N, 128) * 128) * sizeof(float);
}
extern "C" size_t ns_gemm_splitk_counters(int M, int N) { return (size_t)ceil_div(M, 64) * ceil_div(N, 64); }

extern "C" int ns_gemm(const ns_gemm_params* pp, ns_stream_t stream_) {
  hipStream_t stream = (hipStream_t)stream_;
  NS_CHECK_ARG(pp != nullptr, "ns_gemm: null params");
  ns_gemm_params p = *pp;
  NS_CHECK_ARG(!p.col_sumsq || p.col_sum, "ns_gemm: col_sumsq needs col_sum");
  NS_CHECK_ARG(!p.col_sum || p.stat_part, "ns_gemm: col_sum needs the stat_part scratch (ns_gemm_stat_part_floats)");
  NS_CHECK_ARG(!p.stat_z || (p.col_sum && p.col_sumsq && p.stat_mean && p.stat_istd && p.accumulate != 2 && p.split_k <= 1),
               "ns_gemm: stat_z needs col_sum, col_sumsq, stat_mean, stat_istd and a non-atomic store");
  if (!p.col_sum) p.stat_part = nullptr;
  p.stat_slots = 0;
  int rc = gemm_dispatch(p, stream);
  if (rc || !p.stat_part || p.M == 0 || p.N == 0) return rc;
  hipLaunchKernelGGL(gemm_stats_finalize_kernel, dim3(ceil_div(p.N, 32)), dim3(1024), 0, stream, p.stat_part, p.stat_slots,
                     p.N, p.col_sum, p.col_sumsq);
  NS_CHECK_LAUNCH("gemm_stats_finalize");
  return NS_OK;
}

static int gemm_dispatch(ns_gemm_params& p, hipStream_t stream) {
  NS_CHECK_ARG(p.M >= 0 && p.N >= 0 && p.K >= 0, "ns_gemm: negative dims");
  if (p.M == 0 || p.N == 0) return NS_OK;
  NS_CHECK_ARG(p.A && p.B && p.C, "ns_gemm: null operand");
  NS_CHECK_ARG(p.dtype == NS_F32 || p.dtype == NS_BF16, "ns_gemm: bad dtype %d", p.dtype);
  NS_CHECK_ARG(p.c_dtype == NS_F32 || p.c_dtype == NS_BF16, "ns_gemm: bad c_dtype %d", p.c_dtype);
  if (p.split_k < 1) p.split_k = 1;
  NS_CHECK_ARG((p.splitk_work != nullptr) == (p.splitk_count != nullptr), "ns_gemm: splitk_work and splitk_count come together");
  NS_CHECK_ARG(!p.splitk_work || p.split_k == 1 || p.batch <= 1, "ns_gemm: deterministic split-K takes no batch");
  NS_CHECK_ARG(!p.splitk_work || ns_gemm_splitk_work_bytes(p.M, p.N, p.split_k) < 0x7ffffff0ull,
               "ns_gemm: deterministic split-K scratch beyond 2 GB (32-bit buffer offsets): lower split_k");
  NS_CHECK_ARG(p.accumulate >= 0 && p.accumulate <= 2, "ns_gemm: bad accumulate");
  NS_CHECK_ARG(p.accumulate == 0 || p.c_dtype == NS_F32, "ns_gemm: accumulate needs fp32 C");
  NS_CHECK_ARG(p.split_k == 1 || (p.accumulate == 2 && p.act == NS_ACT_NONE && !p.col_sum),
               "ns_gemm: split_k>1 needs atomic accumulate, no activation, no stats");
  NS_CHECK_ARG(p.b_seg_len == 0 || (p.b_seg_len > 0 && p.K % p.b_seg_len == 0),
               "ns_gemm: K must be a multiple of b_seg_len");
  if (p.alpha == 0.f) p.alpha = 1.f;
  if (p.batch < 1) p.batch = 1;
  NS_CHECK_ARG(p.batch == 1 || (!p.col_sum && !p.bias && !p.addend && !p.gate && !p.A_lo && p.batch <= 65535),
               "ns_gemm: batched calls take no bias / addend / gate / statistics / pre-split operands");

  bool fast = (p.dtype == NS_BF16) && aligned16(p.A) && aligned16(p.B) && (p.lda % 8 == 0) &&
              (p.ldb % 8 == 0) && (p.b_seg_stride % 8 == 0) && (p.batch_stride_a % 8 == 0) &&
              (p.batch_stride_b % 8 == 0);
  if (fast) {
    if (p.a_mode == 0) fast = fast && (p.K % 8 == 0); else fast = fast && (p.M % 8 == 0);
    if (p.b_mode == 0) fast = fast && (p.K % 8 == 0); else fast = fast && (p.N % 8 == 0);
    if (p.b_seg_len > 0) fast = fast && (p.b_seg_len % GBK == 0);
  }
  if (fast && p.M <= 32 && p.a_mode == 0 && p.b_mode == 0 && p.b_seg_len == 0 && p.split_k == 1 &&
      !p.col_sum && p.batch == 1) {
    g_last_kernel = "gemm_skinny_kernel";
    if (p.N >= 32 * 128) hipLaunchKernelGGL(gemm_skinny_kernel<2>, dim3(ceil_div(p.N, 32)), dim3(SKW * 64), 0, stream, p);
    else hipLaunchKernelGGL(gemm_skinny_kernel<1>, dim3(ceil_div(p.N, 16)), dim3(SKW * 64), 0, stream, p);
    NS_CHECK_LAUNCH("gemm_skinny");
    return NS_OK;
  }
  if (fast && p.batch == 1 && x256_ok(p)) {
    const int tiles = ceil_div(p.M, 256) * ceil_div(p.N, 256);
    const size_t lds = 2 * XBUF;
    static bool attr_set = false;
    if (!attr_set) {
      (void)hipFuncSetAttribute((const void*)gemm_x256_kernel<1>, hipFuncAttributeMaxDynamicSharedMemorySize, (int)lds);
      (void)hipFuncSetAttribute((const void*)gemm_x256_kernel<3>, hipFuncAttributeMaxDynamicSharedMemorySize, (int)lds);
      (void)hipFuncSetAttribute((const void*)gemm_x256_kernel<2>, hipFuncAttributeMaxDynamicSharedMemorySize, (int)lds);
      attr_set = true;
    }
    p.stat_slots = 4 * ceil_div(p.M, 256);
    const bool two = p.A_lo && p.f32_passes == 2;
    g_last_kernel = p.A_lo ? (two ? "gemm_x256_kernel<2>" : "gemm_x256_kernel<3>") : "gemm_x256_kernel<1>";
    if (two) hipLaunchKernelGGL(gemm_x256_kernel<2>, dim3(tiles), dim3(512), lds, stream, p);
    else if (p.A_lo) hipLaunchKernelGGL(gemm_x256_kernel<3>, dim3(tiles), dim3(512), lds, stream, p);
    else hipLaunchKernelGGL(gemm_x256_kernel<1>, dim3(tiles), dim3(512), lds, stream, p);
    NS_CHECK_LAUNCH("gemm_x256");
    return NS_OK;
  }
  NS_CHECK_ARG(!p.A_lo && !p.B_lo, "ns_gemm: pre-split operands (A_lo / B_lo) need the 256-tile path "
               "(bf16, a_mode 0, b_mode 0, K %% 64 == 0, M >= 1024, N %% 128 == 0, >= 96 tiles, no split_k)");
  if (fast) {
    const int tiles = ceil_div(p.M, GBM) * ceil_div(p.N, GBN);
    dim3 grid(tiles, p.split_k, p.batch);
    const size_t lds = 65536;
    p.stat_slots = 2 * ceil_div(p.M, GBM);
    const bool vec = vec_epilogue_ok(p);
    const bool half = vec && p.a_mode == 0 && half_tiles_wanted(p, tiles);
    if (half) {
      grid.x = ceil_div(p.M, 64) * ceil_div(p.N, GBN);
      p.stat_slots = ceil_div(p.M, 64);
    }
#define LAUNCH_MFMA(AM, BM_)                                                                      \
  do {                                                                                            \
    static bool attr_set = false;                                                                 \
    if (!attr_set) {                                                                              \
      (void)hipFuncSetAttribute((const void*)gemm_mfma_kernel<AM, BM_, false>,                        \
                          hipFuncAttributeMaxDynamicSharedMemorySize, (int)lds);                  \
      (void)hipFuncSetAttribute((const void*)gemm_mfma_kernel<AM, BM_, true>,                         \
                          hipFuncAttributeMaxDynamicSharedMemorySize, (int)lds);                  \
      attr_set = true;                                                                            \
    }                                                                                             \
    g_last_kernel = vec ? "gemm_mfma_kernel<" #AM ", " #BM_ ", true, 64, 128>" : "gemm_mfma_kernel<" #AM ", " #BM_ ", false, 64, 128>";  \
    if (vec) hipLaunchKernelGGL((gemm_mfma_kernel<AM, BM_, true>), grid, dim3(256), lds, stream, p);  \
    else hipLaunchKernelGGL((gemm_mfma_kernel<AM, BM_, false>), grid, dim3(256), lds, stream, p);     \
  } while (0)
#define LAUNCH_MFMA_HALF(BM_)                                                                     \
  do {                                                                                            \
    static bool attr_set = false;                                                                 \
    if (!attr_set) {                                                                              \
      (void)hipFuncSetAttribute((const void*)gemm_mfma_kernel<0, BM_, true, 64, 64>,                  \
                          hipFuncAttributeMaxDynamicSharedMemorySize, (int)lds);                  \
      attr_set = true;                                                                            \
    }                                                                                             \
    g_last_kernel = "gemm_mfma_kernel<0, " #BM_ ", true, 64, 64>";                                \
    hipLaunchKernelGGL((gemm_mfma_kernel<0, BM_, true, 64, 64>), grid, dim3(256), lds, stream, p);    \
  } while (0)
    static const int bk32_env = [] { const char* e = getenv("NS_GEMM_BK32"); return e ? atoi(e) : -1; }();
    const bool bk32 = bk32_env >= 0 ? bk32_env != 0 : (long)tiles * p.split_k * p.batch >= 600;
    if (half) {
      if (p.b_mode == 0) LAUNCH_MFMA_HALF(0); else LAUNCH_MFMA_HALF(1);
    } else if (p.a_mode == 1 && p.b_mode == 1 && bk32 && (p.b_seg_len == 0 || p.b_seg_len % 32 == 0)) {
      g_last_kernel = vec ? "gemm_mfma_kernel<1, 1, true, 32, 128>" : "gemm_mfma_kernel<1, 1, false, 32, 128>";
      if (vec) hipLaunchKernelGGL((gemm_mfma_kernel<1, 1, true, 32>), grid, dim3(256), 32768, stream, p);
      else hipLaunchKernelGGL((gemm_mfma_kernel<1, 1, false, 32>), grid, dim3(256), 32768, stream, p);
    } else if (p.a_mode == 0 && p.b_mode == 0) LAUNCH_MFMA(0, 0);
    else if (p.a_mode == 0 && p.b_mode == 1) LAUNCH_MFMA(0, 1);
    else if (p.a_mode == 1 && p.b_mode == 0) LAUNCH_MFMA(1, 0);
    else LAUNCH_MFMA(1, 1);
#undef LAUNCH_MFMA_HALF
#undef LAUNCH_MFMA
    NS_CHECK_LAUNCH("gemm_mfma");
    return NS_OK;
  }
  if (p.dtype == NS_F32 && p.f32_passes > 0) {
    bool ok = aligned16(p.A) && aligned16(p.B) && (p.lda % 4 == 0) && (p.ldb % 4 == 0) && (p.b_seg_stride % 4 == 0) &&
              (p.batch_stride_a % 4 == 0) && (p.batch_stride_b % 4 == 0);
    if (p.a_mode == 0) ok = ok && (p.K % 4 == 0); else ok = ok && (p.M % 4 == 0);
    if (p.b_mode == 0) ok = ok && (p.K % 4 == 0); else ok = ok && (p.N % 4 == 0);
    if (p.b_seg_len > 0) ok = ok && (p.b_seg_len % FBK == 0);
    const bool three = p.f32_passes >= 3;
    if (ok && p.M <= 32 && p.a_mode == 0 && p.b_mode == 0 && p.b_seg_len == 0 && p.split_k == 1 && !p.col_sum &&
        p.K % 8 == 0 && p.lda % 4 == 0 && p.batch == 1) {
      g_last_kernel = "gemm_skinny_f32_kernel";
      if (ceil_div(p.N, 16) <= 64) {
        const dim3 grid(ceil_div(p.N, 8), ceil_div(p.M, 16));
        if (three) hipLaunchKernelGGL((gemm_skinny_f32_kernel<3, 1, 8>), grid, dim3(SKW * 64), 0, stream, p);
        else hipLaunchKernelGGL((gemm_skinny_f32_kernel<1, 1, 8>), grid, dim3(SKW * 64), 0, stream, p);
      } else {
        if (three) hipLaunchKernelGGL((gemm_skinny_f32_kernel<3, 2, 16>), dim3(ceil_div(p.N, 16)), dim3(SKW * 64), 0, stream, p);
        else hipLaunchKernelGGL((gemm_skinny_f32_kernel<1, 2, 16>), dim3(ceil_div(p.N, 16)), dim3(SKW * 64), 0, stream, p);
      }
      NS_CHECK_LAUNCH("gemm_skinny_f32");
      return NS_OK;
    }
    if (ok) {
      const int tiles = ceil_div(p.M, GBM) * ceil_div(p.N, GBN);
      dim3 grid(tiles, p.split_k, p.batch);
      const size_t lds = 65536;
      p.stat_slots = 2 * ceil_div(p.M, GBM);
      const bool vec = vec_epilogue_ok(p);
      const bool half = vec && p.a_mode == 0 && half_tiles_wanted(p, tiles);
      if (half) {
        grid.x = ceil_div(p.M, 64) * ceil_div(p.N, GBN);
        p.stat_slots = ceil_div(p.M, 64);
      }
#define LAUNCH_F32(AM, BM_, PS)                                                                     \
  do {                                                                                              \
    static bool attr_set = false;                                                                   \
    if (!attr_set) {                                                                                \
      (void)hipFuncSetAttribute((const void*)gemm_mfma_f32_kernel<AM, BM_, PS, false>,              \
// ... 47 lines not shown
```

### nspeech_amd/models/tacotron2.py

```python
import math
import os

import numpy as np
import torch

from .. import ops
from .._lib import ACT_NONE, ACT_RELU, ACT_SOFTSIGN, ACT_TANH
from ..utils.text.symbols import symbols
from . import params as P_

PADL = 2
PADR = 2


def _round_up(x, m):
    return (x + m - 1) // m * m


class _LazyAudio(object):

    def __init__(self, model):
        self._m = model

    def __len__(self):
# ... 100 lines not shown
        return {k: host[o:o + int(np.prod(s))].reshape(s).copy() for k, (o, s) in self.layout.entries.items()}

    def numpy_grads(self):
        host = self.flat_g.cpu().numpy()
        return {k: host[o:o + int(np.prod(s))].reshape(s).copy() for k, (o, s) in self.layout.entries.items()}

    def numpy_stats(self):
        host = self.flat_stats.cpu().numpy()
        return {k: host[o:o + int(np.prod(s))].reshape(s).copy() for k, (o, s) in self.stat_layout.entries.items()}

    def state_dict(self):
        d = {"model/inference/" + k: torch.from_numpy(v) for k, v in self.numpy_params().items()}
        d.update({"model/inference/" + k: torch.from_numpy(v) for k, v in self.numpy_stats().items()})
        d["optimizer/adam_m"] = self.flat_m.cpu()
        d["optimizer/adam_v"] = self.flat_v.cpu()
        d["global_step"] = torch.tensor(self.global_step)
        return d

    def load_state_dict(self, d):
        pv = {k: d["model/inference/" + k].numpy() for k in self.layout.entries}
        sv = {k: d["model/inference/" + k].numpy() for k in self.stat_layout.entries}
        self.load_numpy(pv, sv)
        if "optimizer/adam_m" in d:
            self.flat_m.copy_(d["optimizer/adam_m"])
            self.flat_v.copy_(d["optimizer/adam_v"])
        self.global_step = int(d.get("global_step", 0))

    def _o(self, name):
        return self.layout.off(name)

    def _bf16_w(self, D):
        if D == torch.float32 and self.passes_bwd == 1 and self.flat_s is not self.flat_p:
            return self.flat_s
        return None

    def _dgb(self, name, numel, D):
        if self._bf16_w(D) is None:
            return None
        return self._buf(name, numel, torch.bfloat16)

    def _W(self, D):
        return self.flat_p if D == torch.float32 else self.flat_s

    use_cast_batch = os.environ.get("NS_CAST_BATCH", "1") != "0"

    def refresh_shadows(self, full=False):
        if full or not self.use_cast_batch or self.device.type != "cuda":
            return self._refresh_shadows(full)
        batch = getattr(self, "_cast_batch", None)
        if batch is None:
            batch = self._cast_batch = ops.CastBatch(self.device).record(lambda: self._refresh_shadows(False))
        else:
            ops.CAST_RECORD = dropped = []
            try:
                self._refresh_shadows(False)
            finally:
                ops.CAST_RECORD = None
            if len(dropped) != batch.n:
                batch = self._cast_batch = ops.CastBatch(self.device).record(lambda: self._refresh_shadows(False))
        batch.run()

    def _refresh_shadows(self, full=False):
        hp = self._hparams
        T = self.T
        dev = self.device
        if full and self.flat_s is not self.flat_p:
            ops.cast2d(self.flat_p, 1, self.layout.size, self.layout.size, self.flat_s, self.layout.size, False)
        if not hasattr(self, "tsh"):
            self.tsh = {}

        split = self.passes_fwd > 0

        def tr(key, name, r0, rows, cols, D=None, pair_only=False):
            D = D or T
            want_pair = split and D == torch.float32
            if want_pair and key + "_hi" not in self.tsh:
                self.tsh[key + "_hi"] = torch.zeros(cols * rows, dtype=torch.bfloat16, device=dev)
                self.tsh[key + "_lo"] = torch.zeros(cols * rows, dtype=torch.bfloat16, device=dev)
            dst = None
            if not (pair_only and want_pair):
                if key not in self.tsh:
                    self.tsh[key] = torch.zeros(cols * rows, dtype=D, device=dev)
                dst = self.tsh[key]
            ops.cast2d(self.flat_p, rows, cols, cols, dst, rows, True, src_off=self._o(name) + r0 * cols,
                       dst_hi=self.tsh[key + "_hi"] if want_pair else None,
                       dst_lo=self.tsh[key + "_lo"] if want_pair else None)

        M, E, A, D = hp.num_mels, 2 * hp.encoder_lstm_units, hp.attention_dim, hp.decoder_lstm_units
        He, Hx = hp.encoder_lstm_units, hp.expand_lstm_units
        C = hp.encoder_conv_channels
        Cx = hp.expand_conv_channels
        for d in ("fw", "bw"):
            tr("enc_%s_whT" % d, "encoder/encoder_lstm/%s/lstm_cell/kernel" % d, C, He, 4 * He)
            tr("exp_%s_whT" % d, "expand/encoder_lstm/%s/lstm_cell/kernel" % d, Cx, Hx, 4 * Hx, self.Tx)
        tr("l1_whT", "decoder/lstm_1/kernel", A + E, D, 4 * D)
        tr("l2_whT", "decoder/lstm_2/kernel", D, D, 4 * D)
        if self.mode == "mixed" and (A + E) % 64 == 0 and D % 64 == 0 and (4 * D) % 128 == 0:
            tr("l1_xT", "decoder/lstm_1/kernel", 0, A + E, 4 * D, torch.float32, pair_only=True)
            tr("l2_xT", "decoder/lstm_2/kernel", 0, D, 4 * D, torch.float32, pair_only=True)
        if self.Tx == torch.bfloat16 and Cx % 64 == 0 and (4 * Hx) % 128 == 0:
            for d in ("fw", "bw"):
                tr("exp_%s_xT" % d, "expand/encoder_lstm/%s/lstm_cell/kernel" % d, 0, Cx, 4 * Hx, self.Tx)
        tr("w1cT", "decoder/decoder_prenet/dense_1/kernel", M, E, 256)
        tr("w2T", "decoder/decoder_prenet/dense_2/kernel", 0, 256, 128)
        tr("wattT", "decoder/attention_lstm/kernel", 0, 128 + self.Dsp + A, 4 * A)
        tr("wqT", "decoder/attention/query_layer/kernel", 0, A, A)
        if self.Tx == torch.bfloat16:
            kx = hp.expand_conv_width
            for i in range(1, hp.expand_conv_layers):
                if (kx * Cx) % 64 == 0 and Cx % 128 == 0:
                    tr("expT_%d" % i, "expand/conv_%d/conv1d/kernel" % i, 0, kx * Cx, Cx, self.Tx)
        if self.mode == "mixed":
            kp, Cp = hp.postnet_conv_width, hp.postnet_conv_channels
            for i in range(1, hp.postnet_conv_layers):
                if (kp * Cp) % 64 == 0 and Cp % 128 == 0:
                    tr("postT_%d" % i, "decoder_postnet/postnet_conv_%d/conv1d/kernel" % i, 0, kp * Cp, Cp, torch.float32,
                       pair_only=True)
        if "wcl" not in self.tsh:
            self.tsh["wcl"] = torch.zeros(7 * A, dtype=torch.float32, device=dev)
        ops.gemm(self.flat_p, self.flat_p, self.tsh["wcl"], 7, A, 20, 20, A, A, b_mode=1,
                 a_off=self._o("decoder/attention/location_conv/kernel"),
                 b_off=self._o("decoder/attention/location_layer/kernel"))
        F = hp.num_freq
        Fp = self._lin_pad(F)
        if "wl_pad" not in self.tsh:
            self.tsh["wl_pad"] = torch.zeros(2 * Hx * Fp, dtype=self.Tx, device=dev)
            self.tsh["bl_pad"] = torch.zeros(Fp, dtype=torch.float32, device=dev)
            if self.Tx == torch.bfloat16 and Fp % 128 == 0 and (2 * Hx) % 64 == 0:
                self.tsh["wl_padT"] = torch.zeros(Fp * 2 * Hx, dtype=self.Tx, device=dev)
        ops.cast2d(self.flat_p, 2 * Hx, F, F, self.tsh["wl_pad"], Fp, False, src_off=self._o("dense/kernel"))
        ops.cast2d(self.flat_p, 1, F, F, self.tsh["bl_pad"], Fp, False, src_off=self._o("dense/bias"))
        if "wl_padT" in self.tsh:
            ops.cast2d(self.flat_p, 2 * Hx, F, F, self.tsh["wl_padT"], 2 * Hx, True, src_off=self._o("dense/kernel"))

    def _lin_pad(self, F):
        return _round_up(F, 128) if (self.Tx == torch.bfloat16 and F >= 512) else _round_up(F, 16)

    def _buf(self, name, numel, dtype, zero=True):
        key = name
        if name.startswith("dpre_") or name.startswith("lstm_work"):
            key = "%s_%s" % (name, str(dtype))
        b = self._bufs.get(key)
        if b is None or b.numel() < numel or b.dtype != dtype:
            b = torch.empty(_round_up(numel, 8), dtype=dtype, device=self.device)
            ops.zero(b)
            self._bufs[key] = b
        return b

    _BUCKET_AFTER = {"expand_conv_bwd": "head", "attn_rnn_bwd": "postnet", "attn_wgrad": "decoder",
                     "encoder_bwd": "encoder"}

    overlap_wgrads = os.environ.get("NS_OVERLAP_WGRADS", "1") != "0"
    _queue_env = os.environ.get("NS_WGRAD_QUEUE")

    @property
    def queue_groups(self):
        if self._queue_env is not None:
            return tuple(g for g in self._queue_env.split(",") if g)
        return ("postnet",) if self.reducer is not None else ("postnet", "head")

    def _side_stream(self):
        if self._side is None:
            self._side = ops.concurrent_stream(self.device)
        ev = torch.cuda.Event()
        ev.record(torch.cuda.current_stream(self.device))
        self._side.wait_event(ev)
        self._side_busy = True
        return self._side

    def _defer(self, group, fn, eager=False):
        if not (self.overlap_wgrads and self.device.type == "cuda"):
            fn()
        elif eager and group not in self.queue_groups:
            self._side_groups.add(group)
            with torch.cuda.stream(self._side_stream()):
                fn()
        else:
            self._deferred.append((group, fn))

    def _flush_deferred(self):
        if not self._deferred:
            return
        calls, self._deferred = self._deferred, []
        self._side_groups.update(grp for grp, _ in calls)
        with torch.cuda.stream(self._side_stream()):
            for _, fn in calls:
                fn()

    def _join_deferred(self):
        self._flush_deferred()
        if self._side_busy:
            ev = torch.cuda.Event()
            ev.record(self._side)
            torch.cuda.current_stream(self.device).wait_event(ev)
            self._side_busy = False
        self._side_groups = set()

    def _tick(self, label):
        if self.reducer is not None and label in self._BUCKET_AFTER:
            name = self._BUCKET_AFTER[label]
            if any(grp == name for grp, _ in self._deferred):
                self._deferred.append((name, lambda: self.reducer.bucket_ready(name)))
            elif name in self._side_groups:
                with torch.cuda.stream(self._side_stream()):
                    self.reducer.bucket_ready(name)
            else:
                self.reducer.bucket_ready(name)
        if self.timing is not None:
            ev = torch.cuda.Event(enable_timing=True)
            ev.record()
            self.timing.append((label, ev))

    def _set_inputs(self, text_inputs, input_lengths, speaker_ids):
        dev = self.device
        self.inputs = torch.as_tensor(np.asarray(text_inputs) if not torch.is_tensor(text_inputs) else text_inputs
                                      ).to(dev, torch.int32).contiguous()
        self.input_lengths = torch.as_tensor(
            np.asarray(input_lengths) if not torch.is_tensor(input_lengths) else input_lengths
        ).to(dev, torch.int32).contiguous()
        self._host_lengths = (input_lengths.cpu().numpy() if torch.is_tensor(input_lengths) else np.asarray(input_lengths)
                              ).reshape(-1).astype(np.int64)
        self.speaker_ids = None
        if self.Dsp:
            if speaker_ids is None:
                raise ValueError("num_speakers = %d: speaker_ids are required" % self.n_speakers)
            ids = speaker_ids.cpu().numpy() if torch.is_tensor(speaker_ids) else np.asarray(speaker_ids)
            ids = ids.reshape(-1).astype(np.int64)
            if ids.shape[0] != self.inputs.shape[0] or ids.min() < 0 or ids.max() >= self.n_speakers:
                raise ValueError("speaker_ids must hold one id in [0, %d) per utterance" % self.n_speakers)
            self.speaker_ids = torch.from_numpy(ids.astype(np.int32)).to(dev)

    def initialize(self, text_inputs, input_lengths, speaker_ids=None, mel_targets=None, linear_targets=None):
        dev = self.device
        self._set_inputs(text_inputs, input_lengths, speaker_ids)
        self.is_training = linear_targets is not None
        self.is_training_pass = self.is_training
        if self.is_training:
            self.mel_targets = torch.as_tensor(mel_targets).to(dev, torch.float32).contiguous()
            self.linear_targets = torch.as_tensor(linear_targets).to(dev, torch.float32).contiguous()
            self.forward_train()
        else:
            self.mel_targets = self.linear_targets = None
            from .tacotron2_infer import forward_infer
            forward_infer(self)
        return self

    def add_loss(self):
        return self

    def learning_rate_at(self, step):
        hp = self._hparams
        return hp.initial_learning_rate * 0.5 ** (step / hp.learning_rate_decay_halflife)

    def add_optimizer(self, global_step=0, gradient_clip=1.0):
        self.global_step = int(global_step)
        self.gradient_clip = float(gradient_clip)
        self.optimize = self.step
        return self

    def add_stats(self):
        self.stats = self.summary
        return self

    def summary(self):
        ent = list(self.layout.entries.items())
        pairs = []
        for _, (o, sh) in ent:
            pairs += [o, o + int(np.prod(sh))]
        nvar = len(ent)
        goff = torch.tensor(pairs + [pairs[-1]], dtype=torch.int64, device=self.device)
        gout = self._buf("sum_gout", 4 * (2 * nvar), torch.float32)
        ops.segment_stats(self.flat_g, goff, 2 * nvar, gout)
        vals = {}
        one = self._buf("sum_vout", 16, torch.float32)
        for name in ("mel_outputs", "linear_outputs", "mel_targets", "linear_targets"):
            buf = getattr(self, name).float().contiguous()
            n = buf.numel()
            o2 = torch.tensor([0, n], dtype=torch.int64, device=self.device)
            ops.segment_stats(buf, o2, 1, one)
            sm, sq, mn, mx = [float(x) for x in one[:4].cpu().numpy()]
            mean = sm / n
            vals[name] = dict(min=mn, max=mx, mean=mean, std=math.sqrt(max(sq / n - mean * mean, 0.0)))
        g = gout[:8 * nvar].cpu().numpy().reshape(2 * nvar, 4)[0::2]
        norms = np.sqrt(np.maximum(g[:, 1], 0.0)) / self.world_size
        out = dict(loss=self.loss, loss_mel=self.mel_loss, loss_linear=self.linear_loss, learning_rate=self.learning_rate,
                   max_gradient_norm=float(norms.max()), gradient_norm={k: float(v) for (k, _), v in zip(ent, norms)},
                   histograms=vals)
        return out

    def _stats_buf(self, tag, cout):
        m = self._bufs.setdefault("st_map", {})
        arena = self._buf("st_arena", 1 << 16, torch.float32)
        if tag not in m:
            off = self._bufs.get("st_used", 0)
            assert off + 4 * cout <= arena.numel(), "BatchNorm statistics arena too small"
            m[tag] = arena[off:off + 4 * cout]
            self._bufs["st_used"] = off + ((4 * cout + 63) // 64) * 64
        return m[tag]

    def _bwd_stats_buf(self, tag, cout):
        m = self._bufs.setdefault("bst_map", {})
        if tag not in m:
            m[tag] = self._buf("bst_" + tag, 2 * cout, torch.float32)
        return m[tag]

    def _dy_stats_kw(self, stats_for, row0=0):
        if not stats_for or not self.fuse_bn_bwd_stats:
            return {}
        z = self._bufs[stats_for + "_z"]
        st = self._bufs["st_map"][stats_for]
        c = st.numel() // 4
        bs = self._bwd_stats_buf(stats_for, c)
        self._bwd_sums[stats_for] = (bs, bs[c:])
        return dict(col_sum=bs, col_sumsq=bs[c:], stat_z=z, ld_stat_z=c, stat_z_off=row0 * c, stat_mean=st[2 * c:],
                    stat_istd=st[3 * c:])

    fuse_bn_bwd_stats = True
    postnet_passes = int(os.environ.get("NS_POSTNET_PASSES", "3"))

    def _x256_split_ok(self, tag, rows, cin, cout, k):
        return (self.mode == "mixed" and ("postT_" + tag[4:] + "_hi") in self.tsh and tag.startswith("post")
                and (k * cin) % 64 == 0 and cout % 128 == 0 and rows >= 1024
                and ((rows + 255) // 256) * ((cout + 255) // 256) >= 96)

    def _conv_fwd(self, scope, xin, cin, cout, k, act, N, T, Pp, tag, training=True, D=None, xsplit=None,
                  emit_split=False, y_out=None):
        kl = (k - 1) // 2
        rows = N * Pp
        a_rows = self.padl - kl
        Mg = rows - (k - 1) - a_rows
        D = D or self.T
        z = self._buf(tag + "_z", rows * cout, D)
        st = self._stats_buf(tag, cout)
        wT = self.tsh.get("expT_" + tag[3:]) if tag.startswith("exp") and D == torch.bfloat16 else None
        common = dict(a_off=a_rows * cin, c_off=self.padl * cout, bias=self.flat_p, bias_off=self._o(scope + "/conv1d/bias"),
                      act=act, row_mask=(Pp, self.padl, self.padl + T, self.padl),
                      col_sum=st if training else None, col_sumsq=st[cout:] if training else None)
        if xsplit is not None:
            key = "postT_" + tag[4:]
            ops.gemm(xsplit[0], self.tsh[key + "_hi"], z, Mg, cout, k * cin, cin, k * cin, cout, a_mode=0, b_mode=0,
                     a_lo=xsplit[1], b_lo=self.tsh[key + "_lo"], f32_passes=self.postnet_passes, **common)
        elif wT is not None:
            ops.gemm(xin, wT, z, Mg, cout, k * cin, cin, k * cin, cout, a_mode=0, b_mode=0, **common)
        else:
            ops.gemm(xin, self._W(D), z, Mg, cout, k * cin, cin, cout, cout, a_mode=0, b_mode=1,
                     b_off=self._o(scope + "/conv1d/kernel"), **common)
        y = yh = yl = None
        ykw = {}
        if emit_split:
            yh = self._buf(tag + "_yhi", rows * cout, torch.bfloat16)
            yl = self._buf(tag + "_ylo", rows * cout, torch.bfloat16)
        elif y_out is not None:
            y = y_out[0]
            ykw = dict(y_off=y_out[1], ld_y=y_out[2])
        else:
            y = self._buf(tag + "_y", rows * cout, D)
        ops.bn_fwd(z, y, rows, cout, st, st[cout:], N * T, self.flat_p, self.flat_p, self.flat_stats,
                   self.flat_stats, st[2 * cout:], st[3 * cout:], training, row_mask=(Pp, self.padl, self.padl + T),
                   gamma_off=self._o(scope + "/batch_normalization/gamma"),
                   beta_off=self._o(scope + "/batch_normalization/beta"),
                   mm_off=self.stat_layout.off(scope + "/batch_normalization/moving_mean"),
                   mv_off=self.stat_layout.off(scope + "/batch_normalization/moving_variance"), y_hi=yh, y_lo=yl, **ykw)
        return (yh, yl) if emit_split else y

    def _conv_bwd(self, scope, xin, dy, cin, cout, k, act, N, T, Pp, tag, dx, need_dx=True, dx_accumulate=False,
                  D=None, defer=None, stats_for=None):
        kl = (k - 1) // 2
        kr = k - 1 - kl
        rows = N * Pp
        z = self._bufs[tag + "_z"]
        st = self._bufs["st_map"][tag]
        D = D or self.T
        w16 = self._bf16_w(D)
        Dg = torch.bfloat16 if w16 is not None else D
        own = "_" + tag if (defer and self.overlap_wgrads) else ""
        dpre = self._buf("dpre_%d%s" % (cout, own), rows * cout, Dg)
        if isinstance(xin, tuple):
            assert w16 is not None
            xin = xin[0]
        elif w16 is not None:
            cache, key = getattr(self, "_x16_cache", None), (xin.data_ptr(), rows, cin)
            x16 = cache.get(key) if cache is not None else None
            if x16 is None:
                x16 = self._buf("xin16_%d%s" % (cin, own), rows * cin, torch.bfloat16)
                ops.cast2d(xin, rows, cin, cin, x16, cin, False)
                if cache is not None:
                    cache[key] = x16
            xin = x16
        work = self._buf("bn_work", 200 * max(1024, cout), torch.float32)
        g = self.flat_g
        dykw = {}
        if isinstance(dy, tuple):
            dy, dykw = dy[0], dict(dy_off=dy[1], ld_dy=dy[2])
        ops.bn_bwd(dy, z, dpre, rows, cout, st[2 * cout:], st[3 * cout:], self.flat_p, g, g, g, work, N * T, act,
                   sums=self._bwd_sums.pop(tag, None), row_mask=(Pp, self.padl, self.padl + T), **dykw,
                   gamma_off=self._o(scope + "/batch_normalization/gamma"),
                   dgamma_off=self._o(scope + "/batch_normalization/gamma"),
                   dbeta_off=self._o(scope + "/batch_normalization/beta"),
                   dbias_off=self._o(scope + "/conv1d/bias"))
        a_rows = self.padl - kl
        Mg = rows - (k - 1) - a_rows
        def wgrad():
            ops.gemm(xin, dpre, g, k * cin, cout, Mg, cin, cout, cout, a_mode=1, b_mode=1,
                     a_off=a_rows * cin, b_off=self.padl * cout, c_off=self._o(scope + "/conv1d/kernel"),
                     accumulate=2, split_k=self._splitk(Mg, k * cin, cout))
        if defer:
            self._defer(defer, wgrad, eager=True)
        else:
            wgrad()
        if need_dx:
            a2 = self.padl - kr
            Mg2 = rows - (k - 1) - a2
            ops.gemm(dpre, w16 if w16 is not None else self._W(D), dx, Mg2, cin, k * cout, cout, cout, cin, a_mode=0, b_mode=0,
                     a_off=a2 * cout, b_off=self._o(scope + "/conv1d/kernel") + (k - 1) * cin * cout,
                     b_seg=(cout, -cin * cout), c_off=self.padl * cin, accumulate=1 if dx_accumulate else 0,
                     row_mask=(Pp, self.padl, self.padl + T, self.padl), **self._dy_stats_kw(stats_for, self.padl))

    @staticmethod
    def _splitk(K, M, N):
        tiles = ((M + 127) // 128) * ((N + 127) // 128)
        sk = max(1, min(32, 512 // max(tiles, 1)))
        return max(1, min(sk, K // (256 if tiles <= 16 else 512)))

    def _x256_fits(self, rows, cout):
        return rows >= 1024 and ((rows + 255) // 256) * ((cout + 255) // 256) >= 96

    def _xg_gemm(self, x, xg, rows, cin, cout, key, woff, boff, D=None):
        D = D or self.T
        sh = self.tsh.get(key)
        if self._x256_fits(rows, cout) and D == torch.float32 and key + "_hi" in self.tsh:
            xh = self._buf("xgs_hi_" + key, rows * cin, torch.bfloat16)
            xl = self._buf("xgs_lo_" + key, rows * cin, torch.bfloat16)
            ops.split_hi_lo(x, xh, xl, rows * cin)
            ops.gemm(xh, self.tsh[key + "_hi"], xg, rows, cout, cin, cin, cin, cout, a_mode=0, b_mode=0, a_lo=xl,
                     b_lo=self.tsh[key + "_lo"], bias=self.flat_p, bias_off=boff)
        elif sh is not None and self._x256_fits(rows, cout) and D == torch.bfloat16 and sh.dtype == torch.bfloat16:
            ops.gemm(x, sh, xg, rows, cout, cin, cin, cin, cout, a_mode=0, b_mode=0, bias=self.flat_p, bias_off=boff)
        else:
            ops.gemm(x, self._W(D), xg, rows, cout, cin, cin, cout, cout, b_mode=1, b_off=woff, bias=self.flat_p, bias_off=boff)

    def _bilstm_fwd(self, scope, x, cin, H, N, T, Pp, lengths, tag, key, D=None):
        rows = N * Pp
        D = D or self.T
        out = self._buf(tag + "_h", rows * 2 * H, D)
        f32c = (D == torch.float32 and self.passes_fwd == 3 and self.use_cluster and H % 64 == 0 and H <= 256 and T >= 2
                and (self.passes_bwd == 1 or not self.is_training_pass))
        hb = self._buf(tag + "_h16", rows * 2 * H, torch.bfloat16) if f32c else None
        pair = []
        for di, d in enumerate(("fw", "bw")):
            kname = "%s/%s/lstm_cell/kernel" % (scope, d)
            xg = self._buf("%s_xg_%s" % (tag, d), rows * 4 * H, torch.float32)
            self._xg_gemm(x, xg, rows, cin, 4 * H, "%s_%s_xT" % (key, d), self._o(kname),
                          self._o("%s/%s/lstm_cell/bias" % (scope, d)), D)
            c = self._buf("%s_c_%s" % (tag, d), rows * H, torch.float32)
            gt = self._buf("%s_g%s_%s" % (tag, "16" if f32c else "", d), rows * 4 * H, torch.bfloat16 if f32c else D)
            wk = "%s_%s_whT" % (key, d)
            pair.append(ops.lstm_seq_params(N, T, H, Pp, self.padl, xg, 4 * H, self.tsh[wk], None,
                                            lengths, d == "bw", out, 2 * H, c, gt, h_off=di * H,
                                            whT_hi=self.tsh.get(wk + "_hi") if D == torch.float32 else None,
                                            whT_lo=self.tsh.get(wk + "_lo") if D == torch.float32 else None,
                                            h_bf16=hb, h_bf16_off=di * H, ld_h_bf16=2 * H))
        if f32c and not ops.lstm_cluster_supported(pair[0], pair[1], False):
            raise RuntimeError("BiLSTM %s: the fp32-state cluster kernel refused a shape its pre-check accepted" % tag)
        self._bilstm_f32c = getattr(self, "_bilstm_f32c", {})
        self._bilstm_f32c[tag] = f32c
        self._run_bilstm("fwd", pair, tag)
        return out

    use_wide = True

    def zoneout_args(self, layer):
        if self.zoneout_rate <= 0.0:
            return None
        thr = ops.zoneout_threshold(self.zoneout_rate)
        base = self.zoneout_base_seed
        if torch.distributed.is_available() and torch.distributed.is_initialized():
            base ^= (torch.distributed.get_rank() * 0x9E3779B9) & 0xFFFFFFFF
        return (thr, thr, ops.zoneout_seed(base, self.global_step, 2 * layer),
                ops.zoneout_seed(base, self.global_step, 2 * layer + 1))

    def _run_lstm(self, direction, tag, *a, **kw):
        p = ops.lstm_seq_params(*a, **kw)
        if self.use_wide and ops.lstm_wide_supported(p, direction == "bwd"):
            w = self._buf("lstm_wide_work_%s_%s" % (tag, direction), ops.lstm_wide_work_floats(p), torch.float32)
            ops.lstm_wide(direction, p, w)
            self._status_words[(tag, direction)] = w
            self.last_paths["%s:%s" % (tag, direction)] = "wide"
        else:
            ops.lstm_seq_call(direction, p)
            self.last_paths["%s:%s" % (tag, direction)] = "step"

    use_cluster = True
    use_attn_cluster = True

    def _run_bilstm(self, direction, pair, tag):
        from .._lib import NS_BF16
        ok = pair[0].dtype == NS_BF16 or getattr(self, "_bilstm_f32c", {}).get(tag, False)
        if self.use_cluster and ok and ops.lstm_cluster_supported(pair[0], pair[1], direction == "bwd"):
            work = self._buf("lstm_cluster_work_%s_%s" % (tag, direction), ops.lstm_cluster_work_floats(pair[0]),
                             torch.float32)
            ops.lstm_cluster(direction, pair[0], pair[1], work)
            self._status_words[(tag, direction)] = work
            self.last_paths["%s:%s" % (tag, direction)] = "cluster"
        else:
            ops.lstm_seq2(direction, pair[0], pair[1])
            self.last_paths["%s:%s" % (tag, direction)] = "step"

    def check_status(self):
        for key, w in self._status_words.items():
            v = int(w[:1].view(torch.int32).item())
            if v != 0:
                raise RuntimeError("persistent LSTM kernel %s timed out (status %d)" % (key, v))

    def _bilstm_bwd(self, scope, x, dout, cin, H, N, T, Pp, lengths, tag, dx, D=None, defer=None, stats_for=None):
        rows = N * Pp
        D = D or self.T
        g = self.flat_g
        hbuf = self._bufs[tag + "_h"]
        f32c = getattr(self, "_bilstm_f32c", {}).get(tag, False)
        if f32c:
            hbuf = self._bufs[tag + "_h16"]
            x16 = self._buf("%s_x16" % tag, rows * cin, torch.bfloat16)
            ops.cast2d(x, rows, cin, cin, x16, cin, False)
            x = x16
            D = torch.bfloat16
        pair = []
        for di, d in enumerate(("fw", "bw")):
            kname = "%s/%s/lstm_cell/kernel" % (scope, d)
            ko = self._o(kname)
            c = self._bufs["%s_c_%s" % (tag, d)]
            gt = self._bufs["%s_g%s_%s" % (tag, "16" if f32c else "", d)]
            dg = self._buf("%s_dg%s_%s" % (tag, "16" if f32c else "", d), rows * 4 * H, D)
            work = self._buf("lstm_work_%s" % d, N * H + 64, torch.float32)
            pair.append(ops.lstm_seq_params(N, T, H, Pp, self.padl, self._bufs["%s_xg_%s" % (tag, d)], 4 * H, None,
                                            self._W(D), lengths, d == "bw", hbuf, 2 * H, c, gt, dh=dout,
                                            ld_dh=2 * H, dgates=dg, work=work, wh_off=ko + cin * 4 * H,
                                            h_off=di * H, dh_off=di * H,
                                            wh_bf16=self._bf16_w(D), wh_bf16_off=ko + cin * 4 * H,
                                            dgates_bf16=self._dgb("%s_dgb_%s" % (tag, d), rows * 4 * H, D)))
        self._run_bilstm("bwd", pair, tag)
        for di, d in enumerate(("fw", "bw")):
            kname = "%s/%s/lstm_cell/kernel" % (scope, d)
            ko = self._o(kname)
            dg = self._bufs["%s_dg%s_%s" % (tag, "16" if f32c else "", d)]

            def wgrads(d=d, di=di, ko=ko, dg=dg):
                ops.gemm(x, dg, g, cin, 4 * H, rows, cin, 4 * H, 4 * H, a_mode=1, b_mode=1, c_off=ko, accumulate=2,
                         split_k=self._splitk(rows, cin, 4 * H))
                if d == "fw":
                    ops.gemm(hbuf, dg, g, H, 4 * H, rows - 1, 2 * H, 4 * H, 4 * H, a_mode=1, b_mode=1,
                             a_off=di * H, b_off=4 * H, c_off=ko + cin * 4 * H, accumulate=2,
                             split_k=self._splitk(rows, H, 4 * H))
                else:
                    ops.gemm(hbuf, dg, g, H, 4 * H, rows - 1, 2 * H, 4 * H, 4 * H, a_mode=1, b_mode=1,
                             a_off=2 * H + di * H, b_off=0, c_off=ko + cin * 4 * H, accumulate=2,
                             split_k=self._splitk(rows, H, 4 * H))
                ops.colsum(dg, 4 * H, rows, 4 * H, g, out_off=self._o("%s/%s/lstm_cell/bias" % (scope, d)))
            if defer:
                self._defer(defer, wgrads, eager=True)
            else:
                wgrads()
            ops.gemm(dg, self._W(D), dx, rows, cin, 4 * H, 4 * H, 4 * H, cin, a_mode=0, b_mode=0, b_off=ko,
                     accumulate=0 if di == 0 else 1, row_mask=(Pp, self.padl, self.padl + T, 0),
                     **(self._dy_stats_kw(stats_for) if di == 1 else {}))

    def _speaker_fwd(self, N):
        hp = self._hparams
        sd, Dsp = hp.speaker_embed_dim, self.Dsp
        se = self._buf("spk_e", N * sd, self.T)
        ops.embedding_fwd(self.speaker_ids, self.flat_p, se, N, 1, 1, 0, sd, self.n_speakers,
                          table_off=self._o("speaker/speaker_embed"))
        s1 = self._buf("spk_s", N * Dsp, self.T)
        ops.gemm(se, self._W(self.T), s1, N, Dsp, sd, sd, Dsp, Dsp, b_mode=1, b_off=self._o("decoder/dense/kernel"),
                 bias=self.flat_p, bias_off=self._o("decoder/dense/bias"), act=ACT_SOFTSIGN)
        return s1

    def _speaker_bwd(self, dga, N, S1):
        hp = self._hparams
        sd, Dsp, A = hp.speaker_embed_dim, self.Dsp, hp.attention_dim
        T_, g, rows = self.T, self.flat_g, N * S1
        sel = self._bufs.get("spk_sel")
        if sel is None or sel.numel() != N * rows:
            sel = torch.zeros(N, rows, dtype=T_, device=self.device)
            for n in range(N):
                sel[n, n * S1:(n + 1) * S1] = 1
            sel = self._bufs["spk_sel"] = sel.reshape(-1)
        dgs = self._buf("spk_dgs", N * 4 * A, T_)
        ops.gemm(sel, dga, dgs, N, 4 * A, rows, rows, 4 * A, 4 * A, a_mode=0, b_mode=1)
        ds1 = self._buf("spk_ds", N * Dsp, torch.float32)
        wa = self._o("decoder/attention_lstm/kernel")
        ops.gemm(dgs, self._W(T_), ds1, N, Dsp, 4 * A, 4 * A, 4 * A, Dsp, a_mode=0, b_mode=0, b_off=wa + 128 * 4 * A)
        dpre = self._buf("spk_dpre", N * Dsp, T_)
        ops.act_bwd(ds1, self._bufs["spk_s"], dpre, N, Dsp, ACT_SOFTSIGN)
        se = self._bufs["spk_e"]
        kd = self._o("decoder/dense/kernel")
        ops.gemm(se, dpre, g, sd, Dsp, N, sd, Dsp, Dsp, a_mode=1, b_mode=1, c_off=kd, accumulate=2)
        ops.colsum(dpre, Dsp, N, Dsp, g, out_off=self._o("decoder/dense/bias"))
        dse = self._buf("spk_de", N * sd, torch.float32)
        ops.gemm(dpre, self._W(T_), dse, N, sd, Dsp, Dsp, Dsp, sd, a_mode=0, b_mode=0, b_off=kd)
        ops.embedding_bwd(self.speaker_ids, dse, g, N, 1, 1, 0, sd, self.n_speakers,
                          dtable_off=self._o("speaker/speaker_embed"))

    def forward_train(self):
        hp = self._hparams
        T_ = self.T
        N, Ti = self.inputs.shape
        To = self.mel_targets.shape[1]
        r = hp.outputs_per_step
        assert To % r == 0, "T_out must be a multiple of outputs_per_step (datafeeder pads to it)"
        S = To // r
        assert S <= hp.max_iters, "targets longer than max_iters*outputs_per_step"
        M, F = hp.num_mels, hp.num_freq
        Fp = self._lin_pad(F)
        E, A, D = 2 * hp.encoder_lstm_units, hp.attention_dim, hp.decoder_lstm_units
        Pi, Po = Ti + self.padl + self.padr, To + self.padl + self.padr
        S1 = S + 1
        self.dims = dict(N=N, Ti=Ti, To=To, S=S, Pi=Pi, Po=Po, Fp=Fp)
        sig = ("train", N, Ti, To)
        if sig != self._sig:
            self._bufs.clear()
            self._sig = sig
        self._tick("start")
        ops.F32_PASSES = self.passes_fwd
        ops.CELL_CLIP = self.cell_clip
        Tx = self.Tx

        emb = hp.embedding_dim
        x = self._buf("enc_x0", N * Pi * emb, T_)
        ops.embedding_fwd(self.inputs, self.flat_p, x, N, Ti, Pi, self.padl, emb, self.vocab,
                          table_off=self._o("embedding/embedding"))
        cin = emb
        self._enc_in = [x]
        for i in range(hp.encoder_conv_layers):
            act = ACT_RELU if i < hp.encoder_conv_layers - 1 else ACT_NONE
            x = self._conv_fwd("encoder/conv_%d" % i, x, cin, hp.encoder_conv_channels, hp.encoder_conv_width, act,
                               N, Ti, Pi, "enc%d" % i)
            cin = hp.encoder_conv_channels
            self._enc_in.append(x)
        enc = self._bilstm_fwd("encoder/encoder_lstm", x, cin, hp.encoder_lstm_units, N, Ti, Pi, self.input_lengths,
                               "encl", "enc")
        self._tick("encoder")
        keys = self._buf("keys", N * Pi * A, torch.float32)
        ops.gemm(enc, self._W(self.T), keys, N * Pi, A, E, E, A, A, b_mode=1,
                 b_off=self._o("attention_decoder/memory_layer/kernel"))

        fr = self._buf("dec_fr", N * S1 * M, T_)
        if S > 1:
            ops.copy3d(self.mel_targets, fr, N, S - 1, M, (To * M, r * M), (S1 * M, M), src_off=(r - 1) * M,
                       dst_off=2 * M)
        f1 = self._buf("dec_f1", N * S1 * 256, torch.float32)
        w1 = self._o("decoder/decoder_prenet/dense_1/kernel")
        ops.gemm(fr, self._W(self.T), f1, N * S1, 256, M, M, 256, 256, b_mode=1, b_off=w1, bias=self.flat_p,
                 bias_off=self._o("decoder/decoder_prenet/dense_1/bias"))
        Tia = _round_up(Ti, 8)
        p1 = self._buf("dec_p1", N * S1 * 256, T_)
        Dsp = self.Dsp
        xa = self._buf("dec_xa", N * S1 * (128 + Dsp + A), T_)
        if Dsp:
            ops.copy3d(self._speaker_fwd(N), xa, N, S1, Dsp, (Dsp, 0), (S1 * (128 + Dsp + A), 128 + Dsp + A), dst_off=128)
        hc = self._buf("dec_hc", N * S1 * (A + E), T_)
        ca = self._buf("dec_ca", N * S1 * A, torch.float32)
        ga = self._buf("dec_ga", N * S1 * 4 * A, T_)
        q = self._buf("dec_q", N * S1 * A, torch.float32)
        al = self._buf("dec_al", N * S1 * Tia, torch.float32)
        pv = None
        if self.use_pv:
            pv = self._buf("dec_pv", N * Pi * 256, T_)
            ops.gemm(enc, self._W(self.T), pv, N * Pi, 256, E, E, 256, 256, b_mode=1, b_off=w1 + M * 256)
        self._attn_args = dict(
            pv=pv, Dsp=Dsp,
            dtype=ops.dt(hc), N=N, S=S, Ti=Ti, Pi=Pi, padl_i=self.padl, Tia=Tia, A=A, E=E, D1=256, D2=128, kw=7,
            lengths=self.input_lengths, keys=keys, values=enc, f1=f1,
            w1cT=self.tsh["w1cT"], w2T=self.tsh["w2T"], wattT=self.tsh["wattT"], wqT=self.tsh["wqT"],
            b2=(self.flat_p, self._o("decoder/decoder_prenet/dense_2/bias")),
            batt=(self.flat_p, self._o("decoder/attention_lstm/bias")),
            wcl=self.tsh["wcl"], v=(self.flat_p, self._o("decoder/attention/attention_v")),
            p1=p1, xa=xa, hc=hc, ca=ca, ga=ga, q=q, align=al,
            keys_t=self._buf("dec_keys_t", N * A * Tia, torch.float32),
            work=self._buf("attn_work", N * (E + 9 * Tia + 2 * A + A * Tia) + 64, torch.float32),
            wattT_hi=self.tsh.get("wattT_hi"), wattT_lo=self.tsh.get("wattT_lo"),
            align_t=self._buf("dec_al_t", N * S1 * Tia, T_))
        w2 = self._o("decoder/decoder_prenet/dense_2/kernel")
        wa = self._o("decoder/attention_lstm/kernel")
        wq = self._o("decoder/attention/query_layer/kernel")
        self._attn_args.update(w1c=(self._W(self.T), w1 + M * 256), w2=(self._W(self.T), w2),
                               watt=(self._W(self.T), wa), wq=(self._W(self.T), wq))
        self._attn_cluster_fwd = self.use_attn_cluster and ops.taco2_attn_cluster_supported(**self._attn_args)
        if self._attn_cluster_fwd:
            cw = self._buf("attn_cluster_work", ops.taco2_attn_cluster_work_floats(**self._attn_args), torch.float32)
            ops.taco2_attn_cluster("fwd", cw, **self._attn_args)
            self._status_words[("attn", "fwd")] = cw
        else:
            ops.taco2_attn("fwd", **self._attn_args)
        self.last_paths["attn:fwd"] = "cluster" if self._attn_cluster_fwd else "step"
        self._tick("attn_rnn")

        rows = N * S1
        k1, k2 = self._o("decoder/lstm_1/kernel"), self._o("decoder/lstm_2/kernel")
        xg1 = self._buf("dec_xg1", rows * 4 * D, torch.float32)
        self._xg_gemm(hc, xg1, rows, A + E, 4 * D, "l1_xT", k1, self._o("decoder/lstm_1/bias"))
        h1 = self._buf("dec_h1", rows * D, T_)
        c1 = self._buf("dec_c1", rows * D, torch.float32)
        g1 = self._buf("dec_g1", rows * 4 * D, T_)
        self._tick("dec_lstm:xg1")
        self._run_lstm("fwd", "dec1", N, S, D, S1, 1, xg1, 4 * D, self.tsh["l1_whT"], None, None, False, h1, D, c1, g1,
                       whT_hi=self.tsh.get("l1_whT_hi"), whT_lo=self.tsh.get("l1_whT_lo"), zoneout=self.zoneout_args(1))
        self._tick("dec_lstm:loop1")
        xg2 = self._buf("dec_xg2", rows * 4 * D, torch.float32)
        self._xg_gemm(h1, xg2, rows, D, 4 * D, "l2_xT", k2, self._o("decoder/lstm_2/bias"))
        h2 = self._buf("dec_h2", rows * D, T_)
        c2 = self._buf("dec_c2", rows * D, torch.float32)
        g2 = self._buf("dec_g2", rows * 4 * D, T_)
        self._tick("dec_lstm:xg2")
        self._run_lstm("fwd", "dec2", N, S, D, S1, 1, xg2, 4 * D, self.tsh["l2_whT"], None, None, False, h2, D, c2, g2,
                       whT_hi=self.tsh.get("l2_whT_hi"), whT_lo=self.tsh.get("l2_whT_lo"), zoneout=self.zoneout_args(2))
        self._tick("dec_lstm:loop2")
        dec = self._buf("dec_out", rows * M * r, torch.float32)
        ops.gemm(h2, self._W(self.T), dec, rows, M * r, D, D, M * r, M * r, b_mode=1,
                 b_off=self._o("decoder/output_projection/kernel"), bias=self.flat_p,
                 bias_off=self._o("decoder/output_projection/bias"))
        self._tick("dec_lstm")

        decp = self._buf("decp", N * Po * M, torch.float32)
        pin = self._buf("post_in", N * Po * M, T_)
        ops.copy3d(dec, decp, N, To, M, (S1 * M * r, M), (Po * M, M), src_off=M * r, dst_off=self.padl * M)
        ops.copy3d(dec, pin, N, To, M, (S1 * M * r, M), (Po * M, M), src_off=M * r, dst_off=self.padl * M)
        x = pin
        cin = M
        self._post_in = [x]
        Cp = hp.postnet_conv_channels
        for i in range(hp.postnet_conv_layers):
            act = ACT_TANH if i < hp.postnet_conv_layers - 1 else ACT_NONE
            nxt = i + 1 < hp.postnet_conv_layers and self._x256_split_ok("post%d" % (i + 1), N * Po, Cp, Cp, hp.postnet_conv_width)
            split_in = isinstance(x, tuple)
            x = self._conv_fwd("decoder_postnet/postnet_conv_%d" % i, None if split_in else x, cin, Cp,
                               hp.postnet_conv_width, act, N, To, Po, "post%d" % i, xsplit=x if split_in else None,
                               emit_split=nxt)
            cin = Cp
            self._post_in.append(x)
        mel = self._buf("mel_out", N * Po * M, torch.float32)
        ops.gemm(x, self._W(self.T), mel, N * Po, M, Cp, Cp, M, M, b_mode=1,
                 b_off=self._o("decoder_postnet/dense/kernel"), bias=self.flat_p,
                 bias_off=self._o("decoder_postnet/dense/bias"), row_mask=(Po, self.padl, self.padl + To, 0))
        ops.copy3d(decp, mel, N, Po, M, (Po * M, M), (Po * M, M), accumulate=1)
        self._tick("postnet")

        ein = self._buf("exp_in", N * Po * M, Tx)
        ops.copy3d(mel, ein, N, Po, M, (Po * M, M), (Po * M, M))
        x = ein
        cin = M
        self._exp_in = [x]
        Cx = hp.expand_conv_channels
        for i in range(hp.expand_conv_layers):
            act = ACT_RELU if i < hp.expand_conv_layers - 1 else ACT_NONE
            x = self._conv_fwd("expand/conv_%d" % i, x, cin, Cx, hp.expand_conv_width, act, N, To, Po, "exp%d" % i,
                               D=Tx)
            cin = Cx
            self._exp_in.append(x)
        self._tick("expand_conv")
        Hx = hp.expand_lstm_units
        ex = self._bilstm_fwd("expand/encoder_lstm", x, cin, Hx, N, To, Po, None, "expl", "exp", D=Tx)
        self._tick("expand_lstm")
        lin = self._buf("lin_out", N * Po * Fp, torch.float32)
        if "wl_padT" in self.tsh:
            ops.gemm(ex, self.tsh["wl_padT"], lin, N * Po, Fp, 2 * Hx, 2 * Hx, 2 * Hx, Fp, b_mode=0, bias=self.tsh["bl_pad"])
        else:
            ops.gemm(ex, self.tsh["wl_pad"], lin, N * Po, Fp, 2 * Hx, 2 * Hx, Fp, Fp, b_mode=1, bias=self.tsh["bl_pad"])
        self._tick("linear")

        self.mel_outputs = mel[:N * Po * M].view(N, Po, M)[:, self.padl:self.padl + To]
        self.linear_outputs = lin[:N * Po * Fp].view(N, Po, Fp)[:, self.padl:self.padl + To, :F]
        self.decoder_outputs = dec[:rows * M * r].view(N, S1, M * r)[:, 1:].reshape(N, To, M)
        self.alignments = al[:N * S1 * Tia].view(N, S1, Tia)[:, 1:, :Ti].permute(0, 2, 1)
        self.audio = _LazyAudio(self)
        return self

    def backward(self):
        hp = self._hparams
        T_ = self.T
        d = self.dims
        N, Ti, To, S, Pi, Po, Fp = d["N"], d["Ti"], d["To"], d["S"], d["Pi"], d["Po"], d["Fp"]
        r, M, F = hp.outputs_per_step, hp.num_mels, hp.num_freq
        E, A, D = 2 * hp.encoder_lstm_units, hp.attention_dim, hp.decoder_lstm_units
        S1 = S + 1
        g = self.flat_g
        ops.DETERMINISTIC_SPLITK = self.deterministic
        ops.zero_many((g, self.scal))
        self._deferred = []
        self._bwd_sums = {}
        B = self._bufs
        ops.F32_PASSES = self.passes_bwd
        Tx = self.Tx

        n_prio = int(2000 / (hp.sample_rate * 0.5) * F)
        dmel = self._buf("d_mel", N * Po * M, torch.float32)
        dlin = self._buf("d_lin", N * Po * Fp, Tx)
        ops.l1_loss(B["mel_out"], M, self.mel_targets, dmel, M, N, To, Po, self.padl, M, 0, 1.0 / (N * To * M), 0.0,
                    self.scal, acc_off=0)
        ops.l1_loss(B["lin_out"], Fp, self.linear_targets, dlin, Fp, N, To, Po, self.padl, F, n_prio,
                    0.5 / (N * To * F), 0.5 / (N * To * n_prio), self.scal, acc_off=2)
        self._n_prio = n_prio
        self._tick("loss")

        Hx = hp.expand_lstm_units
        ex = B["expl_h"]
        rows_o = N * Po
        dwl = self._buf("d_wl_pad", 2 * Hx * Fp, torch.float32)
        ops.zero(dwl)
        ops.gemm(ex, dlin, dwl, 2 * Hx, Fp, rows_o, 2 * Hx, Fp, Fp, a_mode=1, b_mode=1, accumulate=2,
                 split_k=self._splitk(rows_o, 2 * Hx, Fp))
        ops.copy3d(dwl, g, 1, 2 * Hx, F, (0, Fp), (0, F), dst_off=self._o("dense/kernel"), accumulate=1)
        ops.colsum(dlin, Fp, rows_o, F, g, out_off=self._o("dense/bias"))
        dex = self._buf("d_exp_h", rows_o * 2 * Hx, torch.float32)
        ops.gemm(dlin, self.tsh["wl_pad"], dex, rows_o, 2 * Hx, Fp, Fp, Fp, 2 * Hx, a_mode=0, b_mode=0)
        self._tick("linear_bwd")
        Cx = hp.expand_conv_channels
        dx = self._buf("d_act_a", rows_o * 512, torch.float32)
        dx2 = self._buf("d_act_b", rows_o * 512, torch.float32)
        self._bilstm_bwd("expand/encoder_lstm", self._exp_in[-1], dex, Cx, Hx, N, To, Po, None, "expl", dx, D=Tx,
                         defer="head", stats_for="exp%d" % (hp.expand_conv_layers - 1))
        self._tick("expand_lstm_bwd")
        cur, nxt = dx, dx2
        for i in range(hp.expand_conv_layers - 1, -1, -1):
            act = ACT_RELU if i < hp.expand_conv_layers - 1 else ACT_NONE
            cin = M if i == 0 else Cx
            if i == 0:
                self._conv_bwd("expand/conv_0", self._exp_in[0], cur, cin, Cx, hp.expand_conv_width, act, N, To, Po,
                               "exp0", dmel, dx_accumulate=True, D=Tx, defer="head")
            else:
                self._conv_bwd("expand/conv_%d" % i, self._exp_in[i], cur, cin, Cx, hp.expand_conv_width, act, N, To,
                               Po, "exp%d" % i, nxt, D=Tx, defer="head", stats_for="exp%d" % (i - 1))
                cur, nxt = nxt, cur
        self._tick("expand_conv_bwd")
        Cp = hp.postnet_conv_channels
        dmel_t = self._buf("d_mel_t", rows_o * M, T_)
        ops.copy3d(dmel, dmel_t, 1, rows_o, M, (0, M), (0, M))
        ko = self._o("decoder_postnet/dense/kernel")
        ops.gemm(self._post_in[-1], dmel_t, g, Cp, M, rows_o, Cp, M, M, a_mode=1, b_mode=1, c_off=ko, accumulate=2,
                 split_k=self._splitk(rows_o, Cp, M))
        ops.colsum(dmel_t, M, rows_o, M, g, out_off=self._o("decoder_postnet/dense/bias"))
        cur, nxt = dx, dx2
        ops.gemm(dmel_t, self._W(self.T), cur, rows_o, Cp, M, M, M, Cp, a_mode=0, b_mode=0, b_off=ko,
                 row_mask=(Po, self.padl, self.padl + To, 0), **self._dy_stats_kw("post%d" % (hp.postnet_conv_layers - 1)))
        for i in range(hp.postnet_conv_layers - 1, -1, -1):
            act = ACT_TANH if i < hp.postnet_conv_layers - 1 else ACT_NONE
            cin = M if i == 0 else Cp
            if i == 0:
                self._conv_bwd("decoder_postnet/postnet_conv_0", self._post_in[0], cur, cin, Cp,
                               hp.postnet_conv_width, act, N, To, Po, "post0", dmel, dx_accumulate=True,
                               defer="postnet")
            else:
                self._conv_bwd("decoder_postnet/postnet_conv_%d" % i, self._post_in[i], cur, cin, Cp,
                               hp.postnet_conv_width, act, N, To, Po, "post%d" % i, nxt, defer="postnet",
                               stats_for="post%d" % (i - 1))
                cur, nxt = nxt, cur
        self._tick("postnet_bwd")
        rows = N * S1
        ddec = self._buf("d_dec", rows * M * r, T_)
        ops.copy3d(dmel, ddec, N, To, M, (Po * M, M), (S1 * M * r, M), src_off=self.padl * M, dst_off=M * r)
        h2, h1, hc = B["dec_h2"], B["dec_h1"], B["dec_hc"]
        kp = self._o("decoder/output_projection/kernel")
        def proj_wgrad():
            ops.gemm(h2, ddec, g, D, M * r, rows, D, M * r, M * r, a_mode=1, b_mode=1, c_off=kp, accumulate=2,
                     split_k=self._splitk(rows, D, M * r))
            ops.colsum(ddec, M * r, rows, M * r, g, out_off=self._o("decoder/output_projection/bias"))
        self._defer("decoder", proj_wgrad)
        dh2 = self._buf("d_h2", rows * D, torch.float32)
        ops.gemm(ddec, self._W(self.T), dh2, rows, D, M * r, M * r, M * r, D, a_mode=0, b_mode=0, b_off=kp)
        work = self._buf("lstm_work_d", 2 * N * D + 64, torch.float32)
        k1, k2 = self._o("decoder/lstm_1/kernel"), self._o("decoder/lstm_2/kernel")
        dg2 = self._buf("d_g2", rows * 4 * D, T_)
        self._dgb("d_g2b", rows * 4 * D, T_)
        self._tick("dec_lstm_bwd:proj")
        if self.queue_groups:
            self._flush_deferred()
        self._run_lstm("bwd", "dec2", N, S, D, S1, 1, B["dec_xg2"], 4 * D, None, self._W(self.T), None, False, h2, D,
                       B["dec_c2"], B["dec_g2"], dh=dh2, ld_dh=D, dgates=dg2, work=work, wh_off=k2 + D * 4 * D,
                       wh_bf16=self._bf16_w(T_), wh_bf16_off=k2 + D * 4 * D,
                       dgates_bf16=self._dgb("d_g2b", rows * 4 * D, T_), zoneout=self.zoneout_args(2))
        self._tick("dec_lstm_bwd:loop2")
        w16 = self._bf16_w(T_)
        dg2b = self._bufs.get("d_g2b") if w16 is not None else None

        def b16(name, src, cols):
            return src if dg2b is None else self._buf(name, rows * cols, torch.bfloat16)

        def cast16(dst, src, cols):
            if dst is not src:
                ops.cast2d(src, rows, cols, cols, dst, cols, False)
        h1b, h2b = b16("dec_h1_16", h1, D), b16("dec_h2_16", h2, D)

        def lstm2_wgrads():
            cast16(h1b, h1, D)
            cast16(h2b, h2, D)
            self._lstm_wgrads(h1b, D, h2b, D, dg2b if dg2b is not None else dg2, rows, k2, "decoder/lstm_2/bias")
        self._defer("decoder", lstm2_wgrads)
        if "decoder2" in self.queue_groups:
            self._flush_deferred()
        dh1 = self._buf("d_h1", rows * D, torch.float32)
        if dg2b is not None:
            ops.gemm(dg2b, w16, dh1, rows, D, 4 * D, 4 * D, 4 * D, D, a_mode=0, b_mode=0, b_off=k2)
        else:
            ops.gemm(dg2, self._W(self.T), dh1, rows, D, 4 * D, 4 * D, 4 * D, D, a_mode=0, b_mode=0, b_off=k2)
        dg1 = self._buf("d_g1", rows * 4 * D, T_)
        self._dgb("d_g1b", rows * 4 * D, T_)
        self._tick("dec_lstm_bwd:wgrad2")
        self._run_lstm("bwd", "dec1", N, S, D, S1, 1, B["dec_xg1"], 4 * D, None, self._W(self.T), None, False, h1, D,
                       B["dec_c1"], B["dec_g1"], dh=dh1, ld_dh=D, dgates=dg1, work=work, wh_off=k1 + (A + E) * 4 * D,
                       wh_bf16=self._bf16_w(T_), wh_bf16_off=k1 + (A + E) * 4 * D,
                       dgates_bf16=self._dgb("d_g1b", rows * 4 * D, T_), zoneout=self.zoneout_args(1))
        self._tick("dec_lstm_bwd:loop1")
        dg1b = self._bufs.get("d_g1b") if w16 is not None else None
        hcb = b16("dec_hc_16", hc, A + E)

        def lstm1_wgrads():
            cast16(hcb, hc, A + E)
            self._lstm_wgrads(hcb, A + E, h1b, D, dg1b if dg1b is not None else dg1, rows, k1, "decoder/lstm_1/bias")
        self._defer("decoder", lstm1_wgrads)
        dhc = self._buf("d_hc", rows * (A + E), torch.float32)
        if dg1b is not None:
            ops.gemm(dg1b, w16, dhc, rows, A + E, 4 * D, 4 * D, 4 * D, A + E, a_mode=0, b_mode=0, b_off=k1)
        else:
            ops.gemm(dg1, self._W(self.T), dhc, rows, A + E, 4 * D, 4 * D, 4 * D, A + E, a_mode=0, b_mode=0, b_off=k1)
        self._tick("dec_lstm_bwd")
        df1 = self._buf("d_f1", (rows + 1) * 256, T_)
        dp2 = self._buf("d_p2", rows * 128, T_)
        dga = self._buf("d_ga", rows * 4 * A, T_)
        dq = self._buf("d_q", rows * A, T_)
        dkeys = self._buf("d_keys", N * Pi * A, torch.float32)
        dvalues = self._buf("d_values", N * Pi * E, torch.float32)
        ops.zero_many((dkeys, dvalues))
        dwcl = self._buf("d_wcl", _round_up(7 * A, 4), torch.float32)
        ops.zero(dwcl)
        Tia = _round_up(Ti, 8)
        awork = self._buf("attn_work", N * (E + 9 * Tia + 2 * A + A * Tia) + 64, torch.float32)
        w1 = self._o("decoder/decoder_prenet/dense_1/kernel")
        w2 = self._o("decoder/decoder_prenet/dense_2/kernel")
        wa = self._o("decoder/attention_lstm/kernel")
        wq = self._o("decoder/attention/query_layer/kernel")
        args = dict(self._attn_args)
        if args.get("pv") is not None:
            da0 = self._buf("d_a0", rows * Tia, torch.float32)
            enc = args["values"]
            if T_ == torch.float32:
                src, lda, a0 = dhc, A + E, A
            else:
                src, lda, a0 = self._buf("d_hc_ctx", rows * E, T_), E, 0
                ops.copy3d(dhc, src, 1, rows, E, (0, A + E), (0, E), src_off=A)
            ops.gemm(src, enc, da0, S1, Ti, E, lda, E, Tia, b_mode=0, a_off=a0, b_off=self.padl * E, batch=N,
                     batch_strides=(S1 * lda, Pi * E, S1 * Tia))
            args["da0"] = da0
        args.update(w1c=(self._W(self.T), w1 + M * 256), w2=(self._W(self.T), w2), watt=(self._W(self.T), wa),
                    wq=(self._W(self.T), wq), dhc=dhc, df1=df1, dp2=dp2, dga=dga, dq=dq, dkeys=dkeys, dvalues=dvalues,
                    dv=(g, self._o("decoder/attention/attention_v")), dwcl=dwcl, work=awork,
                    watt_bf16=(self._bf16_w(T_), wa) if self._bf16_w(T_) is not None else None,
                    dga_bf16=self._dgb("d_gab", rows * 4 * A, T_),
                    de=self._buf("d_energy", rows * Tia, torch.float32),
                    dctx_t=self._buf("d_ctx_t", rows * E, T_),
                    post_part=ops.attention_post_part(self.device, N, Tia, A))
        if self._attn_cluster_fwd:
            cw = self._buf("attn_cluster_work_b", ops.taco2_attn_cluster_work_floats(**args), torch.float32)
            ops.taco2_attn_cluster("bwd", cw, **args)
            self._status_words[("attn", "bwd")] = cw
        else:
            ops.taco2_attn("bwd", **args)
        self.last_paths["attn:bwd"] = "cluster" if self._attn_cluster_fwd else "step"
        self._tick("attn_rnn_bwd")
        p1, xa, fr = B["dec_p1"], B["dec_xa"], B["dec_fr"]
        sk = self._splitk
        XA = 128 + self.Dsp + A

        def attn_wgrads():
            ops.gemm(fr, df1, g, M, 256, rows, M, 256, 256, a_mode=1, b_mode=1, c_off=w1, accumulate=2,
                     split_k=sk(rows, M, 256))
            ops.gemm(hc, df1, g, E, 256, rows - 1, A + E, 256, 256, a_mode=1, b_mode=1, a_off=A, b_off=256,
                     c_off=w1 + M * 256, accumulate=2, split_k=sk(rows, E, 256))
            ops.colsum(df1, 256, rows, 256, g, out_off=self._o("decoder/decoder_prenet/dense_1/bias"))
            ops.gemm(p1, dp2, g, 256, 128, rows, 256, 128, 128, a_mode=1, b_mode=1, c_off=w2, accumulate=2,
                     split_k=sk(rows, 256, 128))
            ops.colsum(dp2, 128, rows, 128, g, out_off=self._o("decoder/decoder_prenet/dense_2/bias"))
            ops.gemm(xa, dga, g, XA, 4 * A, rows, XA, 4 * A, 4 * A, a_mode=1, b_mode=1, c_off=wa, accumulate=2,
                     split_k=sk(rows, XA, 4 * A))
            ops.colsum(dga, 4 * A, rows, 4 * A, g, out_off=self._o("decoder/attention_lstm/bias"))
            ops.gemm(hc, dq, g, A, A, rows, A + E, A, A, a_mode=1, b_mode=1, c_off=wq, accumulate=2,
                     split_k=sk(rows, A, A))
        self._defer("decoder", attn_wgrads)
        if self.Dsp:
            self._speaker_bwd(dga, N, S1)
        oc = self._o("decoder/attention/location_conv/kernel")
        ol = self._o("decoder/attention/location_layer/kernel")
        ops.gemm(dwcl, self.flat_p, g, 7, 20, A, A, A, 20, a_mode=0, b_mode=0, b_off=ol, c_off=oc, accumulate=1)
        ops.gemm(self.flat_p, dwcl, g, 20, A, 7, 20, A, A, a_mode=1, b_mode=1, a_off=oc, c_off=ol, accumulate=1)
        enc = B["encl_h"]
# ... 119 lines not shown
```

### nspeech_amd/ops.py

```python
import ctypes as C
import ctypes as C_

import torch

from . import _lib as L
from ._lib import NS_BF16, NS_F32


F32_PASSES = 0
CELL_CLIP = 0.0


def stream():
    return torch.cuda.current_stream().cuda_stream


def dt(t):
    if t.dtype == torch.float32:
        return NS_F32
    if t.dtype == torch.bfloat16:
        return NS_BF16
    raise TypeError("unsupported dtype %s" % t.dtype)


def ptr(t, off=0):
    if t is None:
        return None
    assert t.is_cuda, "hot-path tensors must live on the GPU"
    return t.data_ptr() + off * t.element_size()


def gemm(A, B, Cm, M, N, K, lda, ldb, ldc, a_mode=0, b_mode=0, a_off=0, b_off=0, c_off=0,
         bias=None, bias_off=0, act=0, alpha=1.0, accumulate=0, row_mask=None, col_sum=None,
         col_sumsq=None, split_k=1, b_seg=None, addend=None, addend_off=0, ld_add=0, f32_passes=None,
         gate=None, gate_off=0, ld_gate=0, a_lo=None, b_lo=None, batch=1, batch_strides=(0, 0, 0),
         stat_z=None, ld_stat_z=0, stat_mean=None, stat_istd=None, stat_z_off=0):
    assert A.dtype == B.dtype
    p = L.GemmParams()
    p.dtype = dt(A)
    p.M, p.N, p.K = M, N, K
    p.A, p.lda, p.a_mode = ptr(A, a_off), lda, a_mode
    p.B, p.ldb, p.b_mode = ptr(B, b_off), ldb, b_mode
    if b_seg is not None:
        p.b_seg_len, p.b_seg_stride = b_seg
    p.C, p.ldc, p.c_dtype = ptr(Cm, c_off), ldc, dt(Cm)
    p.accumulate = accumulate
    p.bias = ptr(bias, bias_off)
    p.act = act
    p.alpha = alpha
    if row_mask is not None:
        p.row_period, p.row_lo, p.row_hi, p.row_shift = row_mask
    p.col_sum = ptr(col_sum)
    p.col_sumsq = ptr(col_sumsq)
    if col_sum is not None:
        p.stat_part = ptr(_stat_part(col_sum.device, M, N))
    if stat_z is not None:
        p.stat_z, p.ld_stat_z, p.stat_z_dtype = ptr(stat_z, stat_z_off), ld_stat_z, dt(stat_z)
        p.stat_mean, p.stat_istd = ptr(stat_mean), ptr(stat_istd)
    p.split_k = split_k
    if addend is not None:
        p.addend, p.ld_add, p.addend_dtype = ptr(addend, addend_off), ld_add, dt(addend)
    if gate is not None:
        p.gate, p.ld_gate = ptr(gate, gate_off), ld_gate
    p.f32_passes = F32_PASSES if f32_passes is None else f32_passes
    if batch > 1:
        p.batch = batch
        p.batch_stride_a, p.batch_stride_b, p.batch_stride_c = batch_strides
    if a_lo is not None:
        p.A_lo, p.B_lo = ptr(a_lo, a_off), ptr(b_lo, b_off)
    if split_k > 1 and batch == 1 and DETERMINISTIC_SPLITK:
        work, count = _splitk_scratch(Cm.device, M, N, split_k)
        p.splitk_work, p.splitk_count = ptr(work), ptr(count)
    L.call("ns_gemm", p, stream())


DETERMINISTIC_SPLITK = __import__("os").environ.get("NS_DETERMINISTIC", "0") == "1"
_SPLITK = {}


def _splitk_scratch(device, M, N, split_k):
    lib = L.lib()
    fb, fc = lib.ns_gemm_splitk_work_bytes, lib.ns_gemm_splitk_counters
    fb.restype = fc.restype = L.C.c_size_t
    need, cnt = int(fb(int(M), int(N), int(split_k))), int(fc(int(M), int(N)))
    key = (device, stream())
    cur = _SPLITK.get(key)
    if cur is None or cur[0].numel() * 4 < need or cur[1].numel() < cnt:
        w = torch.empty(max(need // 4, cur[0].numel() if cur else 0), dtype=torch.float32, device=device)
        c = torch.zeros(max(cnt, cur[1].numel() if cur else 0, 4096), dtype=torch.int32, device=device)
        cur = _SPLITK[key] = (w, c)
    return cur


_STAT_PART = {}


def _stat_part(device, M, N):
    fn = L.lib().ns_gemm_stat_part_floats
    fn.restype = L.C.c_size_t
    need = int(fn(int(M), int(N)))
    key = (device, stream())
    buf = _STAT_PART.get(key)
    if buf is None or buf.numel() < need:
        buf = _STAT_PART[key] = torch.empty(need, dtype=torch.float32, device=device)
    return buf


def _fill(_st, **kw):
    for k, v in kw.items():
        setattr(_st, k, v)
    return _st


def copy3d(src, dst, I, J, Cc, src_strides, dst_strides, src_off=0, dst_off=0, accumulate=0):
    p = L.struct("ns_copy3d_params")
    _fill(p, src=ptr(src, src_off), src_dtype=dt(src), src_si=src_strides[0], src_sj=src_strides[1],
          dst=ptr(dst, dst_off), dst_dtype=dt(dst), dst_si=dst_strides[0], dst_sj=dst_strides[1],
          I=I, J=J, Cc=Cc, accumulate=accumulate)
    L.call("ns_copy3d", p, stream())


def embedding_fwd(ids, table, out, N, T, P, padl, D, V, table_off=0):
    p = L.struct("ns_embedding_params")
    _fill(p, ids=ptr(ids), table=ptr(table, table_off), out=ptr(out), out_dtype=dt(out), N=N, T=T, P=P,
          padl=padl, D=D, V=V)
    L.call("ns_embedding_fwd", p, stream())


_EMB_WORK = {}


def embedding_bwd(ids, dout, dtable, N, T, P, padl, D, V, dtable_off=0):
    p = L.struct("ns_embedding_bwd_params")
    fn = L.lib().ns_embedding_bwd_work_floats
    fn.restype = C.c_size_t
    work = _scratch(_EMB_WORK, dout.device, int(fn(int(N), int(D), int(V))))
    _fill(p, ids=ptr(ids), dout=ptr(dout), dtable=ptr(dtable, dtable_off), N=N, T=T, P=P, padl=padl, D=D, V=V, work=ptr(work))
    L.call("ns_embedding_bwd", p, stream())


def bn_fwd(z, y, rows, C, col_sum, col_sumsq, count, gamma, beta, moving_mean, moving_var, mean_out, istd_out,
           training, row_mask=None, eps=1e-3, momentum=0.99, gamma_off=0, beta_off=0, mm_off=0, mv_off=0,
           y_hi=None, y_lo=None, y_off=0, ld_y=0):
    p = L.struct("ns_bn_fwd_params")
    if y_hi is not None:
        p.y_hi, p.y_lo = ptr(y_hi), ptr(y_lo)
    p.ld_y = ld_y
    _fill(p, z=ptr(z), y=ptr(y, y_off), dtype=dt(z), rows=rows, C=C, col_sum=ptr(col_sum), col_sumsq=ptr(col_sumsq),
          count=float(count), gamma=ptr(gamma, gamma_off), beta=ptr(beta, beta_off),
          moving_mean=ptr(moving_mean, mm_off), moving_var=ptr(moving_var, mv_off),
          mean_out=ptr(mean_out), istd_out=ptr(istd_out), eps=eps, momentum=momentum, training=int(training))
    if row_mask is not None:
        p.row_period, p.row_lo, p.row_hi = row_mask
    L.call("ns_bn_fwd", p, stream())


def bn_bwd(dy, z, dpre, rows, C, mean, istd, gamma, dgamma, dbeta, dbias, work, count, act, row_mask=None,
           gamma_off=0, dgamma_off=0, dbeta_off=0, dbias_off=0, sums=None, dy_off=0, ld_dy=0):
    p = L.struct("ns_bn_bwd_params")
    p.ld_dy = ld_dy
    if sums is not None:
        p.sum_dy, p.sum_dyxh = ptr(sums[0]), ptr(sums[1])
    assert work.numel() >= 200 * C, "ns_bn_bwd: work needs 200 * C floats"
    _fill(p, dy=ptr(dy, dy_off), z=ptr(z), dpre=ptr(dpre), dtype=dt(z), rows=rows, C=C, mean=ptr(mean), istd=ptr(istd),
          gamma=ptr(gamma, gamma_off), dgamma=ptr(dgamma, dgamma_off), dbeta=ptr(dbeta, dbeta_off),
          dbias=ptr(dbias, dbias_off), work=ptr(work), count=float(count), act=act)
    if dpre.dtype != z.dtype:
        p.dpre_dtype = dt(dpre)
    if row_mask is not None:
        p.row_period, p.row_lo, p.row_hi = row_mask
    L.call("ns_bn_bwd", p, stream())


_COLSUM_WORK = {}


def _scratch(store, key_extra, floats, zero_head=0):
    key = (key_extra, stream())
    buf = store.get(key)
    if buf is None or buf.numel() < floats:
        buf = store[key] = torch.zeros(int(floats), dtype=torch.float32, device=key_extra)
    return buf


def colsum(x, ld, rows, C, out, x_off=0, out_off=0):
    p = L.struct("ns_colsum_params")
    fn = L.lib().ns_colsum_work_floats
    fn.restype = C_.c_size_t
    work = _scratch(_COLSUM_WORK, x.device, int(fn(int(C))))
    _fill(p, x=ptr(x, x_off), dtype=dt(x), ld=ld, rows=rows, C=C, out=ptr(out, out_off), work=ptr(work))
    L.call("ns_colsum", p, stream())


def l1_loss(pred, ldp, target, dpred, ldd, N, T, P, padl, F, n_prio, w_all, w_prio, loss_acc, acc_off=0):
    p = L.struct("ns_l1_loss_params")
    _fill(p, pred=ptr(pred), ldp=ldp, target=ptr(target), dpred=ptr(dpred),
          dpred_dtype=dt(dpred) if dpred is not None else 0, ldd=ldd, N=N, T=T, P=P, padl=padl, F=F,
          n_prio=n_prio, w_all=w_all, w_prio=w_prio, loss_acc=ptr(loss_acc, acc_off))
    L.call("ns_l1_loss", p, stream())


def sumsq(x, n, out, out_off=0, work=None):
    p = L.struct("ns_sumsq_params")
    _fill(p, x=ptr(x), n=n, out=ptr(out, out_off), work=ptr(work))
    L.call("ns_sumsq", p, stream())


def segment_stats(x, offsets, nseg, out):
    p = L.struct("ns_segment_stats_params")
    _fill(p, x=ptr(x), offsets=ptr(offsets), nseg=nseg, out=ptr(out))
    L.call("ns_segment_stats", p, stream())


def adam(pw, g, m, v, n, gnorm_sq, clip, grad_scale, lr_t, beta1, beta2, eps, shadow=None, status=(), skipped=None):
    p = L.struct("ns_adam_params")
    _fill(p, p=ptr(pw), g=ptr(g), m=ptr(m), v=ptr(v), n=n, gnorm_sq=ptr(gnorm_sq), clip=clip,
          grad_scale=grad_scale, lr_t=lr_t, beta1=beta1, beta2=beta2, eps=eps, shadow_bf16=ptr(shadow), skipped=ptr(skipped))
    assert len(status) <= 12
    for i, w in enumerate(status):
        p.status[i] = ptr(w)
    L.call("ns_adam", p, stream())


def zero(t):
    nbytes = t.numel() * t.element_size()
    assert nbytes % 16 == 0 and t.data_ptr() % 16 == 0, "ops.zero: 16-byte granularity"
    L.check(L.lib().ns_zero(C.c_void_p(ptr(t)), C.c_size_t(nbytes), C.c_void_p(stream())), "ns_zero")


def streams_concurrent(a, b):
    work = torch.zeros(4, dtype=torch.int32, device=a.device)
    rc = L.lib().ns_streams_concurrent(C.c_void_p(a.cuda_stream), C.c_void_p(b.cuda_stream), C.c_void_p(ptr(work)))
    if rc < 0:
        L.check(rc, "ns_streams_concurrent")
    return rc == 1


def concurrent_streams(device, n=1, tries=16):
    cur = torch.cuda.current_stream(device)
    chosen, rejected = [], []
    for _ in range(tries):
        if len(chosen) == n:
            break
        s = torch.cuda.Stream(device=device)
        if streams_concurrent(cur, s) and all(streams_concurrent(c, s) for c in chosen):
            chosen.append(s)
        else:
            rejected.append(s)
    while len(chosen) < n:
        chosen.append(rejected.pop() if rejected else torch.cuda.Stream(device=device))
    return chosen


def concurrent_stream(device, tries=8):
    return concurrent_streams(device, 1, tries)[0]


def zero_many(tensors):
    ts = [t for t in tensors if t is not None and t.numel()]
    if not ts:
        return
    for t in ts:
        assert (t.numel() * t.element_size()) % 16 == 0 and t.data_ptr() % 16 == 0, "ops.zero_many: 16-byte granularity"
    n = len(ts)
    ptrs = (C.c_void_p * n)(*[ptr(t) for t in ts])
    nbytes = (C.c_size_t * n)(*[t.numel() * t.element_size() for t in ts])
    L.check(L.lib().ns_zero_many(ptrs, nbytes, n, C.c_void_p(stream())), "ns_zero_many")


CAST_RECORD = None


def cast2d(src, rows, cols, ld_src, dst, ld_dst, transpose, src_off=0, dst_off=0, dst_hi=None, dst_lo=None):
    p = L.struct("ns_cast2d_params")
    _fill(p, src=ptr(src, src_off), rows=rows, cols=cols, ld_src=ld_src, dst=ptr(dst, dst_off) if dst is not None else None,
          dst_dtype=dt(dst) if dst is not None else NS_F32, ld_dst=ld_dst, transpose=int(transpose))
    if dst_hi is not None:
        p.dst_hi, p.dst_lo = ptr(dst_hi, dst_off), ptr(dst_lo, dst_off)
    if CAST_RECORD is not None and L.lib().ns_cast2d_batchable(C.byref(p)) > 0:
        CAST_RECORD.append(p)
        return
    L.call("ns_cast2d", p, stream())


class CastBatch(object):

    def __init__(self, device):
        self.device = device
        self.table = self.ends = None
        self.n = self.total = 0

    def record(self, fn):
        global CAST_RECORD
        CAST_RECORD = rec = []
        try:
            fn()
        finally:
            CAST_RECORD = None
        if not rec:
            return self
        lib = L.lib()
        ends, tot = [], 0
        for p in rec:
            tot += int(lib.ns_cast2d_batchable(C.byref(p)))
            ends.append(tot)
        raw = b"".join(bytes(p) for p in rec)
        self.table = torch.frombuffer(bytearray(raw), dtype=torch.uint8).to(self.device)
        self.ends = torch.tensor(ends, dtype=torch.int32, device=self.device)
        self.n, self.total = len(rec), tot
        return self

    def run(self):
        if self.n:
            L.check(L.lib().ns_cast2d_batch(C.c_void_p(self.table.data_ptr()), C.c_void_p(self.ends.data_ptr()), self.n,
                                            self.total, C.c_void_p(stream())), "ns_cast2d_batch")


def lstm_seq_params(N, T, H, P, padl, xg, ld_xg, whT, wh, lengths, reverse, h, ld_h, c, gates,
                    dh=None, ld_dh=0, dgates=None, work=None, xg_off=0, whT_off=0, wh_off=0, h_off=0, dh_off=0,
                    forget_bias=1.0, whT_hi=None, whT_lo=None, wh_bf16=None, wh_bf16_off=0, dgates_bf16=None,
                    h_bf16=None, h_bf16_off=0, ld_h_bf16=0, dtype=None, zoneout=None):
    p = L.struct("ns_lstm_seq_params")
    if zoneout is not None:
        p.zoneout_thr_cell, p.zoneout_thr_output, p.zoneout_seed_cell, p.zoneout_seed_output = [int(x) for x in zoneout]
# ... 356 lines not shown
```

Baseline: 1.670 million mel-frames/s.

## Fold BN finalize into GEMM stats kernel and defer wgrad work to side stream

Fuses the batchnorm forward finalize (mean/istd and moving-stat update) into the GEMM column-stats finalize kernel, removing one launch per conv layer. In backward, the BN-bwd finalize, bf16 input casts, the linear-head weight gradient and the postnet dense weight gradient move into deferred closures that run on the side wgrad stream, overlapping with main-stream dgrad work. Adds per-tag work buffers so deferred finalize does not race, plus env overrides to keep items on the main stream. Risks extra stream synchronisation and more scratch memory.

Result: faster. 1.689 million mel-frames/s, median of 6 (+1.2%).

```diff
diff --git a/include/nspeech_hip.h b/include/nspeech_hip.h
--- a/include/nspeech_hip.h
+++ b/include/nspeech_hip.h
@@ -22,6 +22,12 @@
 int ns_occupy(int blocks, int threads, int lds_bytes, int heavy, double usec, int* started, ns_stream_t stream);
 int ns_wait_counter(const int* counter, int target, double timeout_usec, ns_stream_t stream);
 
+typedef struct {
+  float count, eps, momentum;
+  int training;
+  float* moving_mean; float* moving_var;
+  float* mean_out; float* istd_out;
+} ns_gemm_bn_params;
 typedef struct {
   int dtype;
   int M, N, K;
@@ -47,6 +53,7 @@
   const void* stat_z; int64_t ld_stat_z; int stat_z_dtype;
   const float* stat_mean; const float* stat_istd;
   float* splitk_work; int* splitk_count;
+  ns_gemm_bn_params bn;
 } ns_gemm_params;
 int ns_gemm(const ns_gemm_params* p, ns_stream_t stream);
 size_t ns_gemm_stat_part_floats(int M, int N);
@@ -93,6 +100,7 @@
   int row_period, row_lo, row_hi;
   void* y_hi; void* y_lo;
   int64_t ld_y;
+  int stats_final;
 } ns_bn_fwd_params;
 int ns_bn_fwd(const ns_bn_fwd_params* p, ns_stream_t stream);
 
@@ -108,8 +116,10 @@
   int dpre_dtype;
   const float* sum_dy; const float* sum_dyxh;
   int64_t ld_dy;
+  int no_finalize;
 } ns_bn_bwd_params;
 int ns_bn_bwd(const ns_bn_bwd_params* p, ns_stream_t stream);
+int ns_bn_bwd_finalize(const ns_bn_bwd_params* p, ns_stream_t stream);
 
 typedef struct {
   const void* x; int dtype; int64_t ld;
diff --git a/nspeech_amd/csrc/common.h b/nspeech_amd/csrc/common.h
--- a/nspeech_amd/csrc/common.h
+++ b/nspeech_amd/csrc/common.h
@@ -37,6 +37,26 @@
 template <typename T> struct dt_of;
 template <> struct dt_of<float> { static constexpr int v = NS_F32; };
 template <> struct dt_of<bf16_t> { static constexpr int v = NS_BF16; };
+
+__device__ __forceinline__ void bn_finalize_column(int c, float sum, float sumsq, float count, float eps, float momentum,
+                                                   int training, float* moving_mean, float* moving_var, float* mean_out,
+                                                   float* istd_out) {
+  float mean, var;
+  if (training) {
+    mean = sum / count;
+    var = sumsq / count - mean * mean;
+    var = var < 0.f ? 0.f : var;
+    if (moving_mean) {
+      moving_mean[c] = moving_mean[c] * momentum + mean * (1.f - momentum);
+      moving_var[c] = moving_var[c] * momentum + var * (1.f - momentum);
+    }
+  } else {
+    mean = moving_mean[c];
+    var = moving_var[c];
+  }
+  mean_out[c] = mean;
+  istd_out[c] = rsqrtf(var + eps);
+}
 
 __device__ __forceinline__ float ldf(const float* p) { return *p; }
 __device__ __forceinline__ float ldf(const bf16_t* p) { return (float)*p; }
diff --git a/nspeech_amd/csrc/core.hip b/nspeech_amd/csrc/core.hip
--- a/nspeech_amd/csrc/core.hip
+++ b/nspeech_amd/csrc/core.hip
@@ -22,7 +22,7 @@
   return cached[dev];
 }
 
-extern "C" int ns_version(void) { return 100; }
+extern "C" int ns_version(void) { return 101; }
 extern "C" const char* ns_device_arch(void) { return "gfx950"; }
 extern "C" const char* ns_last_error(void) { return g_err; }
 
diff --git a/nspeech_amd/csrc/elementwise.hip b/nspeech_amd/csrc/elementwise.hip
--- a/nspeech_amd/csrc/elementwise.hip
+++ b/nspeech_amd/csrc/elementwise.hip
@@ -123,21 +123,8 @@
 __global__ void bn_finalize_kernel(ns_bn_fwd_params p) {
   const int c = blockIdx.x * blockDim.x + threadIdx.x;
   if (c >= p.C) return;
-  float mean, var;
-  if (p.training) {
-    mean = p.col_sum[c] / p.count;
-    var = p.col_sumsq[c] / p.count - mean * mean;
-    var = var < 0.f ? 0.f : var;
-    if (p.moving_mean) {
-      p.moving_mean[c] = p.moving_mean[c] * p.momentum + mean * (1.f - p.momentum);
-      p.moving_var[c] = p.moving_var[c] * p.momentum + var * (1.f - p.momentum);
-    }
-  } else {
-    mean = p.moving_mean[c];
-    var = p.moving_var[c];
-  }
-  p.mean_out[c] = mean;
-  p.istd_out[c] = rsqrtf(var + p.eps);
+  bn_finalize_column(c, p.training ? p.col_sum[c] : 0.f, p.training ? p.col_sumsq[c] : 0.f, p.count, p.eps, p.momentum,
+                     p.training, p.moving_mean, p.moving_var, p.mean_out, p.istd_out);
 }
 
 template <typename T>
@@ -203,11 +190,11 @@
 
 extern "C" int ns_bn_fwd(const ns_bn_fwd_params* p, ns_stream_t s) {
   NS_CHECK_ARG(p && p->z && (p->y || p->y_hi) && p->gamma && p->beta && p->mean_out && p->istd_out, "ns_bn_fwd: null");
-  NS_CHECK_ARG(!p->training || (p->col_sum && p->col_sumsq && p->count > 0), "ns_bn_fwd: training needs stats");
-  NS_CHECK_ARG(p->training || (p->moving_mean && p->moving_var), "ns_bn_fwd: inference needs moving stats");
+  NS_CHECK_ARG(p->stats_final || !p->training || (p->col_sum && p->col_sumsq && p->count > 0), "ns_bn_fwd: training needs stats");
+  NS_CHECK_ARG(p->stats_final || p->training || (p->moving_mean && p->moving_var), "ns_bn_fwd: inference needs moving stats");
   NS_CHECK_ARG((p->y_hi != nullptr) == (p->y_lo != nullptr), "ns_bn_fwd: y_hi and y_lo come together");
   NS_CHECK_ARG(p->ld_y == 0 || (p->ld_y >= p->C && p->y), "ns_bn_fwd: ld_y < C, or no y");
-  hipLaunchKernelGGL(bn_finalize_kernel, dim3(ceil_div(p->C, 256)), dim3(256), 0, (hipStream_t)s, *p);
+  if (!p->stats_final) hipLaunchKernelGGL(bn_finalize_kernel, dim3(ceil_div(p->C, 256)), dim3(256), 0, (hipStream_t)s, *p);
   const long total = (long)p->rows * p->C;
   auto al = [](const void* q, int b) { return ((uintptr_t)q % b) == 0; };
   const int esz = p->dtype == NS_BF16 ? 2 : 4;
@@ -474,18 +461,35 @@
   }
 }
 
-extern "C" int ns_bn_bwd(const ns_bn_bwd_params* p, ns_stream_t s_) {
-  hipStream_t s = (hipStream_t)s_;
-  NS_CHECK_ARG(p && p->dy && p->z && p->dpre && p->mean && p->istd && p->gamma && p->work, "ns_bn_bwd: null");
-  NS_CHECK_ARG(!p->sum_dy == !p->sum_dyxh, "ns_bn_bwd: sum_dy and sum_dyxh come together");
+static int bn_bwd_row_blocks(int rows) { return max(1, min(BN4_MAX_RB, ceil_div(rows, 128))); }
+static bool bn_bwd_vector_form(const ns_bn_bwd_params* p) {
   const bool al16 = ((uintptr_t)p->dy % 16 == 0) && ((uintptr_t)p->z % 8 == 0) && ((uintptr_t)p->dpre % 8 == 0) &&
                     ((uintptr_t)p->mean % 16 == 0) && ((uintptr_t)p->istd % 16 == 0) && ((uintptr_t)p->gamma % 16 == 0) &&
                     ((uintptr_t)p->work % 16 == 0) && (p->dtype == NS_BF16 || ((uintptr_t)p->z % 16 == 0 &&
                     (uintptr_t)p->dpre % (p->dpre_dtype == NS_BF16 ? 8 : 16) == 0)) &&
                     (!p->sum_dy || ((uintptr_t)p->sum_dy % 16 == 0 && (uintptr_t)p->sum_dyxh % 16 == 0));
+  return p->C % 4 == 0 && p->ld_dy % 4 == 0 && al16;
+}
+
+extern "C" int ns_bn_bwd_finalize(const ns_bn_bwd_params* p, ns_stream_t s_) {
+  NS_CHECK_ARG(p && p->dy && p->z && p->dpre && p->mean && p->istd && p->gamma && p->work, "ns_bn_bwd_finalize: null");
+  NS_CHECK_ARG(p->sum_dy && p->sum_dyxh && bn_bwd_vector_form(p),
+               "ns_bn_bwd_finalize: needs sum_dy / sum_dyxh, C %% 4 == 0 and 16-byte aligned operands");
+  hipLaunchKernelGGL(bn_bwd_finalize_kernel, dim3(ceil_div(p->C, 32)), dim3(256), 0, (hipStream_t)s_, *p, p->sum_dy,
+                     p->sum_dyxh, p->work + 2L * p->C, bn_bwd_row_blocks(p->rows));
+  NS_CHECK_LAUNCH("bn_bwd_finalize");
+  return NS_OK;
+}
+
+extern "C" int ns_bn_bwd(const ns_bn_bwd_params* p, ns_stream_t s_) {
+  hipStream_t s = (hipStream_t)s_;
+  NS_CHECK_ARG(p && p->dy && p->z && p->dpre && p->mean && p->istd && p->gamma && p->work, "ns_bn_bwd: null");
+  NS_CHECK_ARG(!p->sum_dy == !p->sum_dyxh, "ns_bn_bwd: sum_dy and sum_dyxh come together");
   NS_CHECK_ARG(p->ld_dy == 0 || p->ld_dy >= p->C, "ns_bn_bwd: ld_dy < C");
-  if (p->C % 4 == 0 && p->ld_dy % 4 == 0 && al16) {
-    const int rb = max(1, min(BN4_MAX_RB, ceil_div(p->rows, 128)));
+  NS_CHECK_ARG(!p->no_finalize || (p->sum_dy && bn_bwd_vector_form(p)),
+               "ns_bn_bwd: no_finalize needs sum_dy / sum_dyxh, C %% 4 == 0 and 16-byte aligned operands");
+  if (bn_bwd_vector_form(p)) {
+    const int rb = bn_bwd_row_blocks(p->rows);
     const dim3 grid4(rb, ceil_div(p->C / 4, BN4_QUADS));
     const float* s1 = p->sum_dy;
     const float* s2 = p->sum_dyxh;
@@ -503,7 +507,8 @@
     }
     if (p->dtype == NS_BF16) hipLaunchKernelGGL(bn_bwd_apply4_kernel<bf16_t>, grid4, dim3(256), 0, s, *p, s1, s2, part);
     else hipLaunchKernelGGL(bn_bwd_apply4_kernel<float>, grid4, dim3(256), 0, s, *p, s1, s2, part);
-    hipLaunchKernelGGL(bn_bwd_finalize_kernel, dim3(ceil_div(p->C, 32)), dim3(256), 0, s, *p, s1, s2, part, rb);
+    if (!p->no_finalize)
+      hipLaunchKernelGGL(bn_bwd_finalize_kernel, dim3(ceil_div(p->C, 32)), dim3(256), 0, s, *p, s1, s2, part, rb);
     NS_CHECK_LAUNCH("bn_bwd");
     return NS_OK;
   }
diff --git a/nspeech_amd/csrc/gemm.hip b/nspeech_amd/csrc/gemm.hip
--- a/nspeech_amd/csrc/gemm.hip
+++ b/nspeech_amd/csrc/gemm.hip
@@ -230,7 +230,7 @@
 }
 
 __global__ __launch_bounds__(1024) void gemm_stats_finalize_kernel(const float* part, int slots, int N, float* col_sum,
-                                                                   float* col_sumsq) {
+                                                                   float* col_sumsq, ns_gemm_bn_params bn) {
   __shared__ float red[32][33][2];
   const int c = threadIdx.x & 31, q = threadIdx.x >> 5;
   const int n = blockIdx.x * 32 + c;
@@ -251,6 +251,9 @@
   if (q == 0 && n < N) {
     col_sum[n] = red[0][c][0];
     if (col_sumsq) col_sumsq[n] = red[0][c][1];
+    if (bn.mean_out)
+      bn_finalize_column(n, red[0][c][0], red[0][c][1], bn.count, bn.eps, bn.momentum, bn.training, bn.moving_mean,
+                         bn.moving_var, bn.mean_out, bn.istd_out);
   }
 }
 
@@ -1074,7 +1077,8 @@
 static int gemm_dispatch(ns_gemm_params& p, hipStream_t stream);
 
 int ns_stats_finalize(const float* part, int slots, int N, float* s1, float* s2, hipStream_t stream) {
-  hipLaunchKernelGGL(gemm_stats_finalize_kernel, dim3(ceil_div(N, 32)), dim3(1024), 0, stream, part, slots, N, s1, s2);
+  hipLaunchKernelGGL(gemm_stats_finalize_kernel, dim3(ceil_div(N, 32)), dim3(1024), 0, stream, part, slots, N, s1, s2,
+                     ns_gemm_bn_params{});
   NS_CHECK_LAUNCH("gemm_stats_finalize");
   return NS_OK;
 }
@@ -1093,12 +1097,21 @@
   NS_CHECK_ARG(!p.col_sum || p.stat_part, "ns_gemm: col_sum needs the stat_part scratch (ns_gemm_stat_part_floats)");
   NS_CHECK_ARG(!p.stat_z || (p.col_sum && p.col_sumsq && p.stat_mean && p.stat_istd && p.accumulate != 2 && p.split_k <= 1),
                "ns_gemm: stat_z needs col_sum, col_sumsq, stat_mean, stat_istd and a non-atomic store");
+  const ns_gemm_bn_params bn = p.bn;
+  if (bn.mean_out) {
+    NS_CHECK_ARG(p.col_sum && p.col_sumsq && !p.stat_z, "ns_gemm: bn needs col_sum and col_sumsq, and no stat_z");
+    NS_CHECK_ARG(bn.istd_out && (bn.training ? bn.count > 0 && !bn.moving_mean == !bn.moving_var
+                                             : bn.moving_mean && bn.moving_var),
+                 "ns_gemm: bn needs istd_out and, in training, count > 0 / otherwise the moving statistics");
+    NS_CHECK_ARG(p.M > 0 && p.N > 0, "ns_gemm: bn on an empty product");
+  }
+  p.bn = ns_gemm_bn_params{};
   if (!p.col_sum) p.stat_part = nullptr;
   p.stat_slots = 0;
   int rc = gemm_dispatch(p, stream);
   if (rc || !p.stat_part || p.M == 0 || p.N == 0) return rc;
   hipLaunchKernelGGL(gemm_stats_finalize_kernel, dim3(ceil_div(p.N, 32)), dim3(1024), 0, stream, p.stat_part, p.stat_slots,
-                     p.N, p.col_sum, p.col_sumsq);
+                     p.N, p.col_sum, p.col_sumsq, bn);
   NS_CHECK_LAUNCH("gemm_stats_finalize");
   return NS_OK;
 }
diff --git a/nspeech_amd/models/tacotron2.py b/nspeech_amd/models/tacotron2.py
--- a/nspeech_amd/models/tacotron2.py
+++ b/nspeech_amd/models/tacotron2.py
@@ -276,6 +276,13 @@
 
     overlap_wgrads = os.environ.get("NS_OVERLAP_WGRADS", "1") != "0"
     _queue_env = os.environ.get("NS_WGRAD_QUEUE")
+    main_stream_items = tuple(i for i in os.environ.get("NS_MAIN_STREAM", "").split(",") if i)
+    _LATE_GROUPS = ("head", "postnet")
+
+    def _on_main(self, item, group=None):
+        if group is not None and (group not in self._LATE_GROUPS or "%s:%s" % (item, group) in self.main_stream_items):
+            return True
+        return item in self.main_stream_items
 
     @property
     def queue_groups(self):
@@ -292,10 +299,10 @@
         self._side_busy = True
         return self._side
 
-    def _defer(self, group, fn, eager=False):
+    def _defer(self, group, fn, eager=False, now=False):
         if not (self.overlap_wgrads and self.device.type == "cuda"):
             fn()
-        elif eager and group not in self.queue_groups:
+        elif now or (eager and group not in self.queue_groups):
             self._side_groups.add(group)
             with torch.cuda.stream(self._side_stream()):
                 fn()
@@ -457,9 +464,15 @@
         z = self._buf(tag + "_z", rows * cout, D)
         st = self._stats_buf(tag, cout)
         wT = self.tsh.get("expT_" + tag[3:]) if tag.startswith("exp") and D == torch.bfloat16 else None
+        mm_off = self.stat_layout.off(scope + "/batch_normalization/moving_mean")
+        mv_off = self.stat_layout.off(scope + "/batch_normalization/moving_variance")
         common = dict(a_off=a_rows * cin, c_off=self.padl * cout, bias=self.flat_p, bias_off=self._o(scope + "/conv1d/bias"),
                       act=act, row_mask=(Pp, self.padl, self.padl + T, self.padl),
                       col_sum=st if training else None, col_sumsq=st[cout:] if training else None)
+        fold = training and not self._on_main("fold")
+        if fold:
+            common["bn"] = dict(count=N * T, training=True, moving_mean=self.flat_stats, mm_off=mm_off,
+                                moving_var=self.flat_stats, mv_off=mv_off, mean_out=st[2 * cout:], istd_out=st[3 * cout:])
         if xsplit is not None:
             key = "postT_" + tag[4:]
             ops.gemm(xsplit[0], self.tsh[key + "_hi"], z, Mg, cout, k * cin, cin, k * cin, cout, a_mode=0, b_mode=0,
@@ -483,8 +496,7 @@
                    self.flat_stats, st[2 * cout:], st[3 * cout:], training, row_mask=(Pp, self.padl, self.padl + T),
                    gamma_off=self._o(scope + "/batch_normalization/gamma"),
                    beta_off=self._o(scope + "/batch_normalization/beta"),
-                   mm_off=self.stat_layout.off(scope + "/batch_normalization/moving_mean"),
-                   mv_off=self.stat_layout.off(scope + "/batch_normalization/moving_variance"), y_hi=yh, y_lo=yl, **ykw)
+                   mm_off=mm_off, mv_off=mv_off, y_hi=yh, y_lo=yl, stats_final=fold, **ykw)
         return (yh, yl) if emit_split else y
 
     def _conv_bwd(self, scope, xin, dy, cin, cout, k, act, N, T, Pp, tag, dx, need_dx=True, dx_accumulate=False,
@@ -499,6 +511,7 @@
         Dg = torch.bfloat16 if w16 is not None else D
         own = "_" + tag if (defer and self.overlap_wgrads) else ""
         dpre = self._buf("dpre_%d%s" % (cout, own), rows * cout, Dg)
+        cast = None
         if isinstance(xin, tuple):
             assert w16 is not None
             xin = xin[0]
@@ -507,24 +520,35 @@
             x16 = cache.get(key) if cache is not None else None
             if x16 is None:
                 x16 = self._buf("xin16_%d%s" % (cin, own), rows * cin, torch.bfloat16)
-                ops.cast2d(xin, rows, cin, cin, x16, cin, False)
+                cast = (x16, xin)
                 if cache is not None:
+                    for stale in [k_ for k_, v_ in cache.items() if v_ is x16]:
+                        del cache[stale]
                     cache[key] = x16
             xin = x16
-        work = self._buf("bn_work", 200 * max(1024, cout), torch.float32)
         g = self.flat_g
         dykw = {}
         if isinstance(dy, tuple):
             dy, dykw = dy[0], dict(dy_off=dy[1], ld_dy=dy[2])
-        ops.bn_bwd(dy, z, dpre, rows, cout, st[2 * cout:], st[3 * cout:], self.flat_p, g, g, g, work, N * T, act,
-                   sums=self._bwd_sums.pop(tag, None), row_mask=(Pp, self.padl, self.padl + T), **dykw,
-                   gamma_off=self._o(scope + "/batch_normalization/gamma"),
-                   dgamma_off=self._o(scope + "/batch_normalization/gamma"),
-                   dbeta_off=self._o(scope + "/batch_normalization/beta"),
-                   dbias_off=self._o(scope + "/conv1d/bias"))
+        sums = self._bwd_sums.pop(tag, None)
+        late = bool(own) and sums is not None and cout % 4 == 0 and not self._on_main("bn_final", defer)
+        work = self._buf("bn_work" + (own if late else ""), 200 * max(1024, cout), torch.float32)
+        fin = ops.bn_bwd(dy, z, dpre, rows, cout, st[2 * cout:], st[3 * cout:], self.flat_p, g, g, g, work, N * T, act,
+                         sums=sums, row_mask=(Pp, self.padl, self.padl + T), **dykw,
+                         gamma_off=self._o(scope + "/batch_normalization/gamma"),
+                         dgamma_off=self._o(scope + "/batch_normalization/gamma"),
+                         dbeta_off=self._o(scope + "/batch_normalization/beta"),
+                         dbias_off=self._o(scope + "/conv1d/bias"), no_finalize=late)
         a_rows = self.padl - kl
         Mg = rows - (k - 1) - a_rows
+        if cast is not None and (not own or self._on_main("cast", defer)):
+            ops.cast2d(cast[1], rows, cin, cin, cast[0], cin, False)
+            cast = None
         def wgrad():
+            if fin is not None:
+                ops.bn_bwd_finalize(fin)
+            if cast is not None:
+                ops.cast2d(cast[1], rows, cin, cin, cast[0], cin, False)
             ops.gemm(xin, dpre, g, k * cin, cout, Mg, cin, cout, cout, a_mode=1, b_mode=1,
                      a_off=a_rows * cin, b_off=self.padl * cout, c_off=self._o(scope + "/conv1d/kernel"),
                      accumulate=2, split_k=self._splitk(Mg, k * cin, cout))
@@ -642,10 +666,14 @@
         g = self.flat_g
         hbuf = self._bufs[tag + "_h"]
         f32c = getattr(self, "_bilstm_f32c", {}).get(tag, False)
+        cast = None
         if f32c:
             hbuf = self._bufs[tag + "_h16"]
             x16 = self._buf("%s_x16" % tag, rows * cin, torch.bfloat16)
-            ops.cast2d(x, rows, cin, cin, x16, cin, False)
+            cast = (x16, x)
+            if not defer or self._on_main("cast", defer):
+                ops.cast2d(x, rows, cin, cin, x16, cin, False)
+                cast = None
             x = x16
             D = torch.bfloat16
         pair = []
@@ -669,6 +697,8 @@
             dg = self._bufs["%s_dg%s_%s" % (tag, "16" if f32c else "", d)]
 
             def wgrads(d=d, di=di, ko=ko, dg=dg):
+                if cast is not None and di == 0:
+                    ops.cast2d(cast[1], rows, cin, cin, cast[0], cin, False)
                 ops.gemm(x, dg, g, cin, 4 * H, rows, cin, 4 * H, 4 * H, a_mode=1, b_mode=1, c_off=ko, accumulate=2,
                          split_k=self._splitk(rows, cin, 4 * H))
                 if d == "fw":
@@ -930,13 +960,20 @@
         ex = B["expl_h"]
         rows_o = N * Po
         dwl = self._buf("d_wl_pad", 2 * Hx * Fp, torch.float32)
-        ops.zero(dwl)
-        ops.gemm(ex, dlin, dwl, 2 * Hx, Fp, rows_o, 2 * Hx, Fp, Fp, a_mode=1, b_mode=1, accumulate=2,
-                 split_k=self._splitk(rows_o, 2 * Hx, Fp))
-        ops.copy3d(dwl, g, 1, 2 * Hx, F, (0, Fp), (0, F), dst_off=self._o("dense/kernel"), accumulate=1)
-        ops.colsum(dlin, Fp, rows_o, F, g, out_off=self._o("dense/bias"))
+
+        def head_wgrad():
+            ops.zero(dwl)
+            ops.gemm(ex, dlin, dwl, 2 * Hx, Fp, rows_o, 2 * Hx, Fp, Fp, a_mode=1, b_mode=1, accumulate=2,
+                     split_k=self._splitk(rows_o, 2 * Hx, Fp))
+            ops.copy3d(dwl, g, 1, 2 * Hx, F, (0, Fp), (0, F), dst_off=self._o("dense/kernel"), accumulate=1)
+            ops.colsum(dlin, Fp, rows_o, F, g, out_off=self._o("dense/bias"))
+        head_late = not self._on_main("head")
+        if not head_late:
+            head_wgrad()
         dex = self._buf("d_exp_h", rows_o * 2 * Hx, torch.float32)
         ops.gemm(dlin, self.tsh["wl_pad"], dex, rows_o, 2 * Hx, Fp, Fp, Fp, 2 * Hx, a_mode=0, b_mode=0)
+        if head_late:
+            self._defer("head", head_wgrad, now=True)
         self._tick("linear_bwd")
         Cx = hp.expand_conv_channels
         dx = self._buf("d_act_a", rows_o * 512, torch.float32)
@@ -960,9 +997,16 @@
         dmel_t = self._buf("d_mel_t", rows_o * M, T_)
         ops.copy3d(dmel, dmel_t, 1, rows_o, M, (0, M), (0, M))
         ko = self._o("decoder_postnet/dense/kernel")
-        ops.gemm(self._post_in[-1], dmel_t, g, Cp, M, rows_o, Cp, M, M, a_mode=1, b_mode=1, c_off=ko, accumulate=2,
-                 split_k=self._splitk(rows_o, Cp, M))
-        ops.colsum(dmel_t, M, rows_o, M, g, out_off=self._o("decoder_postnet/dense/bias"))
+        post_h = self._post_in[-1]
+
+        def postdense_wgrad():
+            ops.gemm(post_h, dmel_t, g, Cp, M, rows_o, Cp, M, M, a_mode=1, b_mode=1, c_off=ko, accumulate=2,
+                     split_k=self._splitk(rows_o, Cp, M))
+            ops.colsum(dmel_t, M, rows_o, M, g, out_off=self._o("decoder_postnet/dense/bias"))
+        if self._on_main("postdense"):
+            postdense_wgrad()
+        else:
+            self._defer("postnet", postdense_wgrad, eager=True)
         cur, nxt = dx, dx2
         ops.gemm(dmel_t, self._W(self.T), cur, rows_o, Cp, M, M, M, Cp, a_mode=0, b_mode=0, b_off=ko,
                  row_mask=(Po, self.padl, self.padl + To, 0), **self._dy_stats_kw("post%d" % (hp.postnet_conv_layers - 1)))
diff --git a/nspeech_amd/ops.py b/nspeech_amd/ops.py
--- a/nspeech_amd/ops.py
+++ b/nspeech_amd/ops.py
@@ -34,7 +34,7 @@
          bias=None, bias_off=0, act=0, alpha=1.0, accumulate=0, row_mask=None, col_sum=None,
          col_sumsq=None, split_k=1, b_seg=None, addend=None, addend_off=0, ld_add=0, f32_passes=None,
          gate=None, gate_off=0, ld_gate=0, a_lo=None, b_lo=None, batch=1, batch_strides=(0, 0, 0),
-         stat_z=None, ld_stat_z=0, stat_mean=None, stat_istd=None, stat_z_off=0):
+         stat_z=None, ld_stat_z=0, stat_mean=None, stat_istd=None, stat_z_off=0, bn=None):
     assert A.dtype == B.dtype
     p = L.GemmParams()
     p.dtype = dt(A)
@@ -57,6 +57,11 @@
     if stat_z is not None:
         p.stat_z, p.ld_stat_z, p.stat_z_dtype = ptr(stat_z, stat_z_off), ld_stat_z, dt(stat_z)
         p.stat_mean, p.stat_istd = ptr(stat_mean), ptr(stat_istd)
+    if bn is not None:
+        _fill(p.bn, count=float(bn["count"]), eps=bn.get("eps", 1e-3), momentum=bn.get("momentum", 0.99),
+              training=int(bn["training"]), moving_mean=ptr(bn.get("moving_mean"), bn.get("mm_off", 0)),
+              moving_var=ptr(bn.get("moving_var"), bn.get("mv_off", 0)), mean_out=ptr(bn["mean_out"]),
+              istd_out=ptr(bn["istd_out"]))
     p.split_k = split_k
     if addend is not None:
         p.addend, p.ld_add, p.addend_dtype = ptr(addend, addend_off), ld_add, dt(addend)
@@ -141,8 +146,9 @@
 
 def bn_fwd(z, y, rows, C, col_sum, col_sumsq, count, gamma, beta, moving_mean, moving_var, mean_out, istd_out,
            training, row_mask=None, eps=1e-3, momentum=0.99, gamma_off=0, beta_off=0, mm_off=0, mv_off=0,
-           y_hi=None, y_lo=None, y_off=0, ld_y=0):
+           y_hi=None, y_lo=None, y_off=0, ld_y=0, stats_final=False):
     p = L.struct("ns_bn_fwd_params")
+    p.stats_final = int(stats_final)
     if y_hi is not None:
         p.y_hi, p.y_lo = ptr(y_hi), ptr(y_lo)
     p.ld_y = ld_y
@@ -156,9 +162,10 @@
 
 
 def bn_bwd(dy, z, dpre, rows, C, mean, istd, gamma, dgamma, dbeta, dbias, work, count, act, row_mask=None,
-           gamma_off=0, dgamma_off=0, dbeta_off=0, dbias_off=0, sums=None, dy_off=0, ld_dy=0):
+           gamma_off=0, dgamma_off=0, dbeta_off=0, dbias_off=0, sums=None, dy_off=0, ld_dy=0, no_finalize=False):
     p = L.struct("ns_bn_bwd_params")
     p.ld_dy = ld_dy
+    p.no_finalize = int(no_finalize)
     if sums is not None:
         p.sum_dy, p.sum_dyxh = ptr(sums[0]), ptr(sums[1])
     assert work.numel() >= 200 * C, "ns_bn_bwd: work needs 200 * C floats"
@@ -170,6 +177,11 @@
     if row_mask is not None:
         p.row_period, p.row_lo, p.row_hi = row_mask
     L.call("ns_bn_bwd", p, stream())
+    return p if no_finalize else None
+
+
+def bn_bwd_finalize(p):
+    L.call("ns_bn_bwd_finalize", p, stream())
 
 
 _COLSUM_WORK = {}
```
